# 0Setsuna0/SoftbodyUnity

Hardware: AMD Instinct MI355X
Metric: particle-substeps/sec (higher is better)
Workload: dtype f32

## Files before the change

include/softbody_debug.h:

```cpp
#ifndef SOFTBODY_MI355X_DEBUG_H
#define SOFTBODY_MI355X_DEBUG_H

#include "softbody.h"

#ifdef __cplusplus
extern "C" {
#endif

#define SB_DEBUG_NO_COMM  1u
#define SB_DEBUG_LOOPBACK 2u

#define SB_TUNE_NO_MASS_PALETTE   (1u << 0)
#define SB_TUNE_NO_UNIFORM_MASS   (1u << 1)
#define SB_TUNE_NO_PALETTE        (1u << 2)
#define SB_TUNE_NO_WAVE_ITEMS     (1u << 3)
#define SB_TUNE_NO_LANE_PACK      (1u << 4)
#define SB_TUNE_NO_COST_ORDER     (1u << 5)
#define SB_TUNE_NO_FUSED_UNPACK   (1u << 6)
#define SB_TUNE_PEER_COARSE       (1u << 7)
#define SB_TUNE_NO_LAZY_TICK      (1u << 8)
#define SB_TUNE_NO_PACK           (1u << 9)
#define SB_TUNE_NO_PEEK           (1u << 10)
#define SB_TUNE_NO_KIN_FUSE       (1u << 11)
#define SB_TUNE_NO_WIDE_SLOTS     (1u << 12)
#define SB_TUNE_AUTO_PREFER_OVERLAP (1u << 13)
#define SB_TUNE_NO_AUTO_CALIBRATION (1u << 14)
#define SB_TUNE_NO_SHARED_PROGRAMS (1u << 15)
typedef struct {
    uint32_t flags;
    int32_t tile_lanes;
    int32_t quad_lanes;
    int32_t narrow_min_tiles;
    int32_t store_through_max_tiles;
    int32_t store_through_large;
    int32_t peek_min_tiles;
    int32_t lds_pad_bytes;
    int32_t win_dwords;
    int32_t prev_offset_bytes;
    int32_t reserved[6];
} sb_tuning;
void sb_tuning_default(sb_tuning *t);
int sb_set_tuning(sb_solver *s, const sb_tuning *t);

int sb_profile_begin(sb_solver *s);
int sb_profile_end(sb_solver *s, float *elapsed_ms_out);
int sb_step_profiled(sb_solver *s, float dt, int32_t substeps, float *slot_ms_out, int32_t *slot_launches_out,
                     int32_t n_slots);
typedef struct {
    int64_t exchanges;
    double pack_ms, transport_ms, total_ms;
    double exposed_wait_ms;
} sb_exchange_timing;
int sb_debug_exchange_timing(sb_solver *s, int32_t enabled);
int sb_debug_exchange_timing_read(sb_solver *s, sb_exchange_timing *out);

int sb_debug_launch(sb_solver *s, float dt, int32_t substeps, int32_t it, int32_t gcolour);
int sb_debug_halo_pack(sb_solver *s, int32_t slot, float *host_out, int64_t capacity_floats, int64_t *count_floats_out);
int sb_debug_halo_unpack(sb_solver *s, int32_t slot, const float *host_in, int64_t count_floats);

typedef struct {
    int64_t tiles_checked, groups_checked, constraints_checked;
    int64_t errors[6];
    int32_t first_stage;
    int32_t first_tile, first_group, first_kind;
} sb_validate_report;
int sb_debug_validate(sb_solver *s, int32_t inject_fault, sb_validate_report *out);

int sb_debug_last_words(int32_t fd, const char *text, int64_t len, int32_t exit_code);

#ifdef __cplusplus
}
#endif
#endif
```

softbodyunity_amd/csrc/abi.hip:

```cpp
#include "solver_internal.hpp"

using namespace sbi;

extern "C" {

void sb_desc_default(sb_desc *d) {
    if (!d) return;
    std::memset(d, 0, sizeof(*d));
    d->world = 1;
    d->gravity[1] = -9.81f;
    d->tile_particles = 0;
    d->use_graph = 1;
}

int sb_create(const sb_desc *desc, sb_solver **out) {
    if (!desc || !out) return fail(SB_ERR_INVALID_ARG, "sb_create: null argument");
    *out = nullptr;
    return guarded([&]() -> int {
        sb_desc d = *desc;
        if (d.world <= 0) d.world = 1;
        if (d.rank < 0 || d.rank >= d.world) return fail(SB_ERR_INVALID_ARG, "sb_create: rank out of range");
        if (!(d.damping >= 0.0f)) return fail(SB_ERR_INVALID_ARG, "sb_create: damping must be >= 0");
        if (d.tile_particles > sbp::kMaxTileLocal) return fail(SB_ERR_INVALID_ARG, "sb_create: tile_particles too large");
        if (d.partition < SB_PARTITION_AUTO || d.partition > SB_PARTITION_RCB) return fail(SB_ERR_INVALID_ARG, "sb_create: partition must be SB_PARTITION_AUTO, _BLOCKS or _RCB");
        if (d.plan_flags & ~kPlanFlagsAll) return fail(SB_ERR_INVALID_ARG, "sb_create: unknown bit in plan_flags");
        if (d.halo_transport != SB_TRANSPORT_RCCL && d.halo_transport != SB_TRANSPORT_PEER) return fail(SB_ERR_INVALID_ARG, "sb_create: halo_transport must be SB_TRANSPORT_RCCL or _PEER");
        if (d.halo_schedule < SB_SCHEDULE_AUTO || d.halo_schedule > SB_SCHEDULE_OVERLAP_GRAPH) return fail(SB_ERR_INVALID_ARG, "sb_create: halo_schedule must be one of SB_SCHEDULE_*");
        if (d.debug_flags & ~(SB_DEBUG_NO_COMM | SB_DEBUG_LOOPBACK)) return fail(SB_ERR_INVALID_ARG, "sb_create: unknown bit in debug_flags");
        if (d.reserved[0] || d.reserved[1] || d.reserved[2]) return fail(SB_ERR_INVALID_ARG, "sb_create: reserved fields must be 0 (zero-initialise sb_desc or call sb_desc_default)");
        int ndev = 0;
        hipError_t e = hipGetDeviceCount(&ndev);
        if (e != hipSuccess || ndev <= 0)
            return fail(SB_ERR_NO_DEVICE, "sb_create: no HIP device (this plugin has no CPU path)");
        if (d.device < 0 || d.device >= ndev) return fail(SB_ERR_NO_DEVICE, "sb_create: device ordinal out of range");
        hipDeviceProp_t prop;
        HIP_CHECK(hipGetDeviceProperties(&prop, d.device));
        if (std::strncmp(prop.gcnArchName, "gfx950", 6) != 0)
            return fail(SB_ERR_NO_DEVICE, std::string("sb_create: device is ") + prop.gcnArchName + ", kernels are built for gfx950 only");
        HIP_CHECK(hipSetDevice(d.device));
        auto s = std::make_unique<sb_solver>();
        s->desc = d;
        s->peer.enabled = d.world > 1 && d.halo_transport == SB_TRANSPORT_PEER;
        s->loopback = d.world > 1 && (d.debug_flags & SB_DEBUG_LOOPBACK) != 0;
        HIP_CHECK(hipStreamCreateWithFlags(&s->stream, hipStreamNonBlocking));
        HIP_CHECK(hipEventCreate(&s->ev0));
        HIP_CHECK(hipEventCreate(&s->ev1));
        *out = s.release();
        return SB_OK;
    });
}

void sb_tuning_default(sb_tuning *t) {
    if (!t) return;
    std::memset(t, 0, sizeof(*t));
    t->store_through_max_tiles = -1;
    t->peek_min_tiles = -1;
}

int sb_set_tuning(sb_solver *s, const sb_tuning *t) {
    if (!s || !t) return fail(SB_ERR_INVALID_ARG, "sb_set_tuning: null argument");
    if (s->finalized) return fail(SB_ERR_STATE, "sb_set_tuning after sb_finalize");
    constexpr uint32_t kAll = (SB_TUNE_NO_SHARED_PROGRAMS << 1) - 1u;
    if (t->flags & ~kAll) return fail(SB_ERR_INVALID_ARG, "sb_set_tuning: unknown bit in flags");
    for (int32_t r : t->reserved) if (r) return fail(SB_ERR_INVALID_ARG, "sb_set_tuning: reserved fields must be 0 (sb_tuning_default)");
    if (t->tile_lanes != 0 && t->tile_lanes != 128 && t->tile_lanes != 256 && t->tile_lanes != 512) return fail(SB_ERR_INVALID_ARG, "sb_set_tuning: tile_lanes must be 0, 128, 256 or 512");
    if (t->quad_lanes != 0 && t->quad_lanes != 256 && t->quad_lanes != 512) return fail(SB_ERR_INVALID_ARG, "sb_set_tuning: quad_lanes must be 0, 256 or 512");
    if (t->prev_offset_bytes < 0 || (t->prev_offset_bytes & 15)) return fail(SB_ERR_INVALID_ARG, "sb_set_tuning: prev_offset_bytes must be a non-negative multiple of 16");
    if (t->narrow_min_tiles < 0 || t->store_through_max_tiles < -1 || t->peek_min_tiles < -1 || t->lds_pad_bytes < 0 || t->win_dwords < 0 || (t->store_through_large & ~3))
        return fail(SB_ERR_INVALID_ARG, "sb_set_tuning: value out of range");
    s->tune_flags = t->flags;
    s->lazy_tick = !(t->flags & SB_TUNE_NO_LAZY_TICK);
    s->pack_tiles = !(t->flags & SB_TUNE_NO_PACK);
    s->peek_enabled = !(t->flags & SB_TUNE_NO_PEEK);
    s->kin_fuse = !(t->flags & SB_TUNE_NO_KIN_FUSE);
    s->tile_lanes = t->tile_lanes;
    s->quad_lanes = t->quad_lanes ? t->quad_lanes : 512;
    if (t->narrow_min_tiles > 0) s->narrow_min_tiles = t->narrow_min_tiles;
    if (t->store_through_max_tiles >= 0) s->store_through_max_tiles = t->store_through_max_tiles;
    s->store_through_large = t->store_through_large;
    if (t->peek_min_tiles >= 0) s->peek_min_tiles = t->peek_min_tiles;
    s->lds_pad = (size_t)t->lds_pad_bytes;
    s->win_dwords_cap = t->win_dwords;
    s->prev_offset_bytes = t->prev_offset_bytes;
    return SB_OK;
}

int sb_destroy(sb_solver *s) {
    if (!s) return fail(SB_ERR_INVALID_ARG, "sb_destroy: null handle");
    (void)hipSetDevice(s->desc.device);
    delete s;
    return SB_OK;
}

int sb_set_particles(sb_solver *s, const float *pos, const float *vel, const float *inv_mass, int32_t n) {
    if (!s || !pos || !inv_mass || n <= 0) return fail(SB_ERR_INVALID_ARG, "sb_set_particles: bad argument");
    if (s->finalized) return fail(SB_ERR_STATE, "sb_set_particles after sb_finalize");
    return guarded([&]() -> int {
        for (int32_t p = 0; p < n; ++p) if (!(inv_mass[p] >= 0.0f)) return fail(SB_ERR_INVALID_ARG, "sb_set_particles: inverse mass must be >= 0");
        s->n = n;
        s->pos.assign(pos, pos + 3 * (size_t)n);
        if (vel) s->vel.assign(vel, vel + 3 * (size_t)n); else s->vel.assign(3 * (size_t)n, 0.0f);
        s->invm.assign(inv_mass, inv_mass + n);
        return SB_OK;
    });
}

int sb_set_rest_positions(sb_solver *s, const float *rest, int32_t n) {
    if (!s || !rest) return fail(SB_ERR_INVALID_ARG, "sb_set_rest_positions: bad argument");
    if (s->finalized) return fail(SB_ERR_STATE, "sb_set_rest_positions after sb_finalize");
    if (n != s->n) return fail(SB_ERR_INVALID_ARG, "sb_set_rest_positions: n differs from sb_set_particles");
    return guarded([&]() -> int { s->rest.assign(rest, rest + 3 * (size_t)n); return SB_OK; });
}

static int set_cons(sb_solver *s, const char *who, const int32_t *idx, const float *rest, int32_t m, float compliance,
                    int type, int nv, int nrest) {
    if (!s || m < 0 || (m > 0 && (!idx || !rest))) return fail(SB_ERR_INVALID_ARG, std::string(who) + ": bad argument");
    if (s->finalized) return fail(SB_ERR_STATE, std::string(who) + " after sb_finalize");
    if (s->n <= 0) return fail(SB_ERR_STATE, std::string(who) + " before sb_set_particles");
    if (!(compliance >= 0.0f)) return fail(SB_ERR_INVALID_ARG, std::string(who) + ": compliance must be >= 0");
    return guarded([&]() -> int {
        std::atomic<bool> bad{false};
        sbp::parallel_for_chunks((int64_t)m * nv, 1 << 22, [&](int64_t, int64_t kb, int64_t ke) {
            for (int64_t k = kb; k < ke; ++k) if (idx[k] < 0 || idx[k] >= s->n) { bad = true; return; }
        });
        if (bad) return fail(SB_ERR_INVALID_ARG, std::string(who) + ": particle index out of range");
        std::vector<int32_t> &I = type == 0 ? s->dist_ij : (type == 1 ? s->vol_ijkl : s->bend_ijkl);
        std::vector<float> &R = type == 0 ? s->dist_rest : (type == 1 ? s->vol_rest : s->bend_rest);
        I.assign(idx, idx + (size_t)m * nv);
        R.assign(rest, rest + (size_t)m * nrest);
        s->compliance[type] = compliance;
        return SB_OK;
    });
}

int sb_set_distance_constraints(sb_solver *s, const int32_t *ij, const float *rest_len, int32_t m, float compliance) {
    return set_cons(s, "sb_set_distance_constraints", ij, rest_len, m, compliance, 0, 2, 1);
}
int sb_set_volume_constraints(sb_solver *s, const int32_t *ijkl, const float *rest_vol, int32_t m, float compliance) {
    return set_cons(s, "sb_set_volume_constraints", ijkl, rest_vol, m, compliance, 1, 4, 1);
}
int sb_set_bending_constraints(sb_solver *s, const int32_t *ijkl, const float *rest_cs, int32_t m, float compliance) {
    return set_cons(s, "sb_set_bending_constraints", ijkl, rest_cs, m, compliance, 2, 4, 2);
}

int sb_set_ground_plane(sb_solver *s, float nx, float ny, float nz, float d, int32_t enabled) {
    if (!s) return fail(SB_ERR_INVALID_ARG, "sb_set_ground_plane: null handle");
    if (!(nx == nx) || !(ny == ny) || !(nz == nz) || !(d == d)) return fail(SB_ERR_INVALID_ARG, "sb_set_ground_plane: NaN");
    s->plane[0] = nx; s->plane[1] = ny; s->plane[2] = nz; s->plane[3] = d;
    s->plane_on = enabled ? 1 : 0;
    return SB_OK;
}

int sb_comm_unique_id(uint8_t out_id[SB_UNIQUE_ID_BYTES]) {
    if (!out_id) return fail(SB_ERR_INVALID_ARG, "sb_comm_unique_id: null");
    static_assert(sizeof(ncclUniqueId) <= SB_UNIQUE_ID_BYTES, "unique id size");
    return guarded([&]() -> int {
        ncclUniqueId id;
        NCCL_CHECK(rccl().GetUniqueId(&id));
        std::memset(out_id, 0, SB_UNIQUE_ID_BYTES);
        std::memcpy(out_id, &id, sizeof(id));
        return SB_OK;
    });
}

int sb_comm_init(sb_solver *s, const uint8_t id_bytes[SB_UNIQUE_ID_BYTES]) {
    if (!s || !id_bytes) return fail(SB_ERR_INVALID_ARG, "sb_comm_init: null");
    if (s->finalized) return fail(SB_ERR_STATE, "sb_comm_init after sb_finalize");
    if (s->comm) return fail(SB_ERR_STATE, "sb_comm_init called twice");
    return guarded([&]() -> int {
        int rc = set_device(s); if (rc) return rc;
        ncclUniqueId id;
        std::memcpy(&id, id_bytes, sizeof(id));
        if (s->loopback) {
            NCCL_CHECK(rccl().CommInitRank(&s->comm, 1, id, 0));
        } else {
            NCCL_CHECK(rccl().CommInitRank(&s->comm, s->desc.world, id, s->desc.rank));
        }
        return SB_OK;
    });
}

int sb_peer_mailbox_handle(sb_solver *s, uint8_t out_handle[SB_IPC_HANDLE_BYTES]) {
    if (!s || !out_handle) return fail(SB_ERR_INVALID_ARG, "sb_peer_mailbox_handle: null argument");
    if (!s->finalized || !s->peer.mailbox) return fail(SB_ERR_STATE, "sb_peer_mailbox_handle: needs a finalized world > 1 solver with SB_HALO_TRANSPORT=peer");
    static_assert(sizeof(hipIpcMemHandle_t) <= SB_IPC_HANDLE_BYTES, "ipc handle size");
    return guarded([&]() -> int {
        int rc = set_device(s); if (rc) return rc;
        hipIpcMemHandle_t h;
        HIP_CHECK(hipIpcGetMemHandle(&h, s->peer.mailbox));
        std::memset(out_handle, 0, SB_IPC_HANDLE_BYTES);
        std::memcpy(out_handle, &h, sizeof(h));
        return SB_OK;
    });
}

int sb_peer_connect(sb_solver *s, int32_t rank, const uint8_t handle[SB_IPC_HANDLE_BYTES], sb_solver *same_process_peer) {
    if (!s || (!handle && !same_process_peer)) return fail(SB_ERR_INVALID_ARG, "sb_peer_connect: null argument");
    if (!s->finalized || !s->peer.mailbox) return fail(SB_ERR_STATE, "sb_peer_connect: needs a finalized world > 1 solver with SB_HALO_TRANSPORT=peer");
    if (rank < 0 || rank >= s->desc.world || rank == s->desc.rank) return fail(SB_ERR_INVALID_ARG, "sb_peer_connect: bad rank");
    if (s->peer.remote[(size_t)rank]) return fail(SB_ERR_STATE, "sb_peer_connect: rank already connected");
    return guarded([&]() -> int {
        int rc = set_device(s); if (rc) return rc;
        if (same_process_peer) {
            if (!same_process_peer->peer.mailbox || same_process_peer->desc.rank != rank) return fail(SB_ERR_INVALID_ARG, "sb_peer_connect: the given solver is not that rank");
            s->peer.remote[(size_t)rank] = same_process_peer->peer.mailbox;
        } else {
            hipIpcMemHandle_t h;
            std::memcpy(&h, handle, sizeof(h));
            void *p = nullptr;
            HIP_CHECK(hipIpcOpenMemHandle(&p, h, hipIpcMemLazyEnablePeerAccess));
            s->peer.remote[(size_t)rank] = (uint32_t *)p; s->peer.opened[(size_t)rank] = 1;
        }
        s->peer.linked = false;
        return SB_OK;
    });
// ... 174 lines not shown
    return SB_OK;
}

int finalize_agree(sb_solver *s, int local_rc) {
    const int W = s->desc.world;
    const size_t rec = (size_t)W + 2;
    const std::string my_error = local_rc ? std::string(last_error_text()) : std::string();
    std::vector<uint64_t> mine = agreement_record(s, local_rc != SB_OK);
    std::vector<uint64_t> all((size_t)W * rec);
    const int rc = guarded([&]() -> int {
        int r0 = set_device(s); if (r0) return r0;
        DevBuf<uint64_t> d_all; int64_t acct = 0;
        d_all.alloc((size_t)W * rec, acct);
        HIP_CHECK(hipMemcpy(d_all.p + (size_t)s->desc.rank * rec, mine.data(), rec * sizeof(uint64_t), hipMemcpyHostToDevice));
        NCCL_CHECK(rccl().AllGather(d_all.p + (size_t)s->desc.rank * rec, d_all.p, rec * sizeof(uint64_t), ncclUint8, s->comm, s->stream));
        HIP_CHECK(hipStreamSynchronize(s->stream));
        HIP_CHECK(hipMemcpy(all.data(), d_all.p, all.size() * sizeof(uint64_t), hipMemcpyDeviceToHost));
        return SB_OK;
    });
    if (local_rc) return fail(local_rc, my_error);
    if (rc) return rc;
    return check_agreement(all, W, s->desc.rank);
}

int finalize_link(sb_solver *s) {
    return guarded([&]() -> int {
        int rc = set_device(s); if (rc) return rc;
        if (s->peer.enabled && s->desc.world > 1) {
            if (s->loopback) {
                peer_link(s);
            } else if (s->comm) {
                const int W = s->desc.world;
                hipIpcMemHandle_t mine;
                HIP_CHECK(hipIpcGetMemHandle(&mine, s->peer.mailbox));
                DevBuf<uint8_t> d_all; int64_t acct = 0;
                d_all.alloc((size_t)W * sizeof(mine), acct);
                HIP_CHECK(hipMemcpy(d_all.p + (size_t)s->desc.rank * sizeof(mine), &mine, sizeof(mine), hipMemcpyHostToDevice));
                NCCL_CHECK(rccl().AllGather(d_all.p + (size_t)s->desc.rank * sizeof(mine), d_all.p, sizeof(mine), ncclUint8, s->comm, s->stream));
                HIP_CHECK(hipStreamSynchronize(s->stream));
                std::vector<hipIpcMemHandle_t> all((size_t)W);
                HIP_CHECK(hipMemcpy(all.data(), d_all.p, (size_t)W * sizeof(mine), hipMemcpyDeviceToHost));
                for (int r = 0; r < W; ++r) {
                    if (r == s->desc.rank) continue;
                    bool needed = false;
                    for (const auto &H : s->halos) for (int pr : H->peers) needed |= pr == r;
                    if (!needed) continue;
                    void *p = nullptr;
                    HIP_CHECK(hipIpcOpenMemHandle(&p, all[(size_t)r], hipIpcMemLazyEnablePeerAccess));
                    s->peer.remote[(size_t)r] = (uint32_t *)p; s->peer.opened[(size_t)r] = 1;
                }
                peer_link(s);
            }
        }
        if (std::getenv("SB_PRINT_ALLOC")) {
            std::fprintf(stderr, "[alloc] pos3 %p prev %p vel %p wf %p w8 %p T0.stream %p T1.stream %p T0.tiles %p T1.tiles %p\n", (void *)s->d_pos3.p, (void *)s->d_prev.p,
                         (void *)s->d_vel.p, (void *)s->d_wf.p, (void *)s->d_w8.p, (void *)s->tiling[0].stream.p, (void *)s->tiling[1].stream.p,
                         (void *)s->tiling[0].tiles.p, (void *)s->tiling[1].tiles.p);
            for (int tl = 0; tl < 3; ++tl) {
                const DevTiling &D = s->tiling[tl];
                if (D.n_tiles)
                    std::fprintf(stderr, "[alloc] T%d: %d tiles, %lld distinct programs, stream %lld B read by the tiles, %lld B uploaded\n", tl, D.n_tiles,
                                 (long long)D.n_programs, (long long)D.stream_bytes, (long long)(D.stream.count * sizeof(uint32_t)));
            }
        }
        HIP_CHECK(hipDeviceSynchronize());
        std::vector<float>().swap(s->pos); std::vector<float>().swap(s->vel); std::vector<float>().swap(s->rest);
        std::vector<int32_t>().swap(s->dist_ij); std::vector<int32_t>().swap(s->vol_ijkl); std::vector<int32_t>().swap(s->bend_ijkl);
        std::vector<float>().swap(s->dist_rest); std::vector<float>().swap(s->vol_rest); std::vector<float>().swap(s->bend_rest);
        s->finalized = true;
        return SB_OK;
    });
}

}

extern "C" {

int sb_finalize(sb_solver *s) {
    if (!s) return fail(SB_ERR_INVALID_ARG, "sb_finalize: null handle");
    if (s->finalized) return fail(SB_ERR_STATE, "sb_finalize called twice");
    if (s->n <= 0) return fail(SB_ERR_STATE, "sb_finalize before sb_set_particles");
    const bool no_comm = (s->desc.debug_flags & SB_DEBUG_NO_COMM) != 0;
    if (s->desc.world > 1 && !s->comm && !s->peer.enabled && !no_comm)
        return fail(SB_ERR_STATE, "sb_finalize: world > 1 needs sb_comm_init first (or halo_transport = SB_TRANSPORT_PEER with sb_peer_connect)");
    int rc = guarded([&]() -> int { return finalize_local(s); });
    if (s->desc.world > 1 && s->comm && !s->loopback) rc = finalize_agree(s, rc);
    if (rc) return rc;
    return finalize_link(s);
}

int sb_synchronize(sb_solver *s) {
    if (!s) return fail(SB_ERR_INVALID_ARG, "sb_synchronize: null handle");
    return guarded([&]() -> int {
        int rc = set_device(s); if (rc) return rc;
        flush_deferred(s);
        HIP_CHECK(hipStreamSynchronize(s->stream));
        check_peer_error(s);
        return SB_OK;
    });
}

int sb_get_owner(sb_solver *s, int32_t *owner, int32_t n) {
    if (!s || !owner) return fail(SB_ERR_INVALID_ARG, "sb_get_owner: null argument");
    if (!s->finalized) return fail(SB_ERR_STATE, "sb_get_owner before sb_finalize");
    if (n != s->n) return fail(SB_ERR_INVALID_ARG, "sb_get_owner: n mismatch");
    std::memcpy(owner, s->plan->plan.owner_of_old.data(), (size_t)n * sizeof(int32_t));
    return SB_OK;
}

int sb_profile_begin(sb_solver *s) {
    if (!s) return fail(SB_ERR_INVALID_ARG, "sb_profile_begin: null handle");
    return guarded([&]() -> int {
        int rc = set_device(s); if (rc) return rc;
        HIP_CHECK(hipEventRecord(s->ev0, s->stream));
        return SB_OK;
    });
}
int sb_profile_end(sb_solver *s, float *ms) {
    if (!s || !ms) return fail(SB_ERR_INVALID_ARG, "sb_profile_end: null argument");
    return guarded([&]() -> int {
        int rc = set_device(s); if (rc) return rc;
        HIP_CHECK(hipEventRecord(s->ev1, s->stream));
        HIP_CHECK(hipEventSynchronize(s->ev1));
        HIP_CHECK(hipEventElapsedTime(ms, s->ev0, s->ev1));
        return SB_OK;
    });
}

int sb_get_stats(sb_solver *s, sb_stats *out) {
    if (!s || !out) return fail(SB_ERR_INVALID_ARG, "sb_get_stats: null argument");
    if (!s->finalized) return fail(SB_ERR_STATE, "sb_get_stats before sb_finalize");
    std::memset(out, 0, sizeof(*out));
    const sbp::Plan &P = s->plan->plan;
    const sbp::LocalPlan &L = s->plan->local;
    out->n_particles_owned = s->n_owned;
    out->n_particles_local = s->n_local;
    for (size_t k = 0; k < L.order_mask[0].size(); ++k) if (L.order_mask[0][k]) ++out->n_constraints_local[P.order_type[0][k]];
    out->n_tilings = P.tiling ? 2 : 1;
    out->n_global_colours = (int32_t)P.gcolours.size();
    for (int tl = 0; tl < 2; ++tl) { out->n_tiles[tl] = s->tiling[tl].n_tiles; out->tile_constraints[tl] = s->tiling[tl].n_slots; }
    out->n_t2_layers = (int64_t)s->t2_layer_range.size();
    out->n_t2_tiles = s->tiling[2].n_tiles;
    out->t2_constraints = s->tiling[2].n_slots;
    out->constraints_in_tiles = P.cons_in_tiles;
    out->constraints_in_global = P.cons_in_global;
    for (size_t slot = 0; slot < s->halos.size(); ++slot) {
        const int64_t cnt = s->halos[slot]->send_off.back();
        if (slot == 1) out->halo_particles_t1 = cnt; else out->halo_particles_global += cnt;
    }
    out->device_bytes = s->dev_bytes;
    {
        const int64_t mb = s->w_uniform ? 0 : (s->w_palette ? 1 : 4);
        auto tables = [&](const DevTiling &D) { return D.stream_bytes + (int64_t)D.n_tiles * (int64_t)sizeof(sbk::TileDesc) + (int64_t)D.runs_overflow.count * 8; };
        for (int tl = 0; tl < 2; ++tl) {
            const DevTiling &D = s->tiling[tl];
            if (!D.n_tiles) continue;
            out->launch_bytes[tl] = D.staged_particles * (12 + mb + 12 + 12 + 12) + tables(D);
        }
        const DevTiling &D0 = s->tiling[0];
        if (D0.n_tiles) {
            out->launch_bytes[2] = D0.staged_particles * (12 + mb + 12 + 12 + 12) + tables(D0);
            out->launch_bytes[3] = D0.staged_particles * (12 + mb + 12 + 12 + 12) + tables(D0);
        }
        const DevTiling &D2 = s->tiling[2];
        if (D2.n_tiles) out->launch_bytes[4] = D2.staged_particles * (4 + 12 + mb + 12) + tables(D2);
    }
    out->partition = P.partition;
    out->halo_schedule = s->schedule;
    out->halo_unpack_fused = s->fused_unpack ? 1 : 0;
    out->halo_auto_state = s->calib.state;
    out->halo_auto_ticks = s->calib.n[0] + s->calib.n[1];
    out->halo_auto_ms[0] = s->calib.decided_ms[0]; out->halo_auto_ms[1] = s->calib.decided_ms[1];
    out->readback_peeks = s->n_peeks;
    out->readback_peek_tiles = s->n_peek_tiles;
    out->ticks_fused = s->n_fused;
    out->ticks_fused_kinematic = s->n_kin_fused;
    for (int tl = 0; tl < 2; ++tl) out->lane_packed_tiles[tl] = s->tiling[tl].n_packed_tiles;
    out->plan_hash = s->plan_hash;
    if (!P.rank_cost.empty()) {
        out->partition_cost = P.rank_cost[(size_t)s->desc.rank];
        for (int64_t c : P.rank_cost) { out->partition_cost_total += c; out->partition_cost_max = std::max(out->partition_cost_max, c); }
    }
    {
        std::vector<uint8_t> is_peer((size_t)s->desc.world, 0);
        for (const auto &H : s->halos) {
            for (int pr : H->peers) is_peer[(size_t)pr] = 1;
            out->halo_particles_recv += H->recv_off.back();
        }
        for (uint8_t b : is_peer) out->halo_peers += b;
    }
    return SB_OK;
}

}
```

softbodyunity_amd/csrc/device_math.hip.hpp:

```cpp
#pragma once
#include "kernel_types.hpp"

namespace sbk {

__device__ __forceinline__ float4 pv_load(const PosView &P, int g) {
    const size_t o = 3 * (size_t)g;
    return make_float4(P.xyz[o], P.xyz[o + 1], P.xyz[o + 2], P.w[g]);
}
__device__ __forceinline__ void pv_store(const PosView &P, int g, const float4 &v) {
    const size_t o = 3 * (size_t)g;
    P.xyz[o] = v.x; P.xyz[o + 1] = v.y; P.xyz[o + 2] = v.z;
}

__device__ __forceinline__ void store3_through(float *p, float x, float y, float z) {
    f32x3_t v = {x, y, z};
    asm volatile("global_store_dwordx3 %0, %1, off sc0 sc1" ::"v"(p), "v"(v) : "memory");
}

struct V3 { float x, y, z; };
__device__ __forceinline__ V3 sub3(V3 a, V3 b) { return {a.x - b.x, a.y - b.y, a.z - b.z}; }
__device__ __forceinline__ V3 cross3(V3 a, V3 b) {
    float t0 = a.y * b.z, t1 = a.z * b.y, t2 = a.z * b.x, t3 = a.x * b.z, t4 = a.x * b.y, t5 = a.y * b.x;
    return {t0 - t1, t2 - t3, t4 - t5};
}
__device__ __forceinline__ float dot3(V3 a, V3 b) {
    float xx = a.x * b.x, yy = a.y * b.y, zz = a.z * b.z;
    return (xx + yy) + zz;
}
__device__ __forceinline__ V3 addscaled3(V3 x, float s, V3 g) {
    float a = s * g.x, b = s * g.y, c = s * g.z;
    return {x.x + a, x.y + b, x.z + c};
}
__device__ __forceinline__ V3 xyz(float4 p) { return {p.x, p.y, p.z}; }

__device__ __forceinline__ float sqrt_rn_normal(float x) {
#ifdef SB_LIBM_SQRT
    return sqrtf(x);
#endif
    float s = __builtin_amdgcn_sqrtf(x);
    float sd = __int_as_float(__float_as_int(s) - 1), su = __int_as_float(__float_as_int(s) + 1);
    float rd = __builtin_fmaf(-sd, s, x), ru = __builtin_fmaf(-su, s, x);
    s = rd <= 0.0f ? sd : s;
    return ru > 0.0f ? su : s;
}

__device__ __forceinline__ bool project_distance(float4 &a, float4 &b, float L0, float at) {
    float dx = a.x - b.x, dy = a.y - b.y, dz = a.z - b.z;
    float xx = dx * dx, yy = dy * dy, zz = dz * dz;
    float L2 = (xx + yy) + zz;
    float ws = (a.w + b.w) + at;
    if (!(L2 >= 0x1p-96f) || !(ws > 0.0f)) return false;
    float L = sqrt_rn_normal(L2);
    float C = L - L0;
    float wl = ws * L;
    float s = (-C) / wl;
    float si = a.w * s, sj = b.w * s;
    float ax = si * dx, ay = si * dy, az = si * dz;
    float bx = sj * dx, by = sj * dy, bz = sj * dz;
    a.x = a.x + ax; a.y = a.y + ay; a.z = a.z + az;
    b.x = b.x - bx; b.y = b.y - by; b.z = b.z - bz;
    return true;
}

__device__ __forceinline__ bool project_distance_nobranch(float4 &a, float4 &b, float L0, float at) {
    float dx = a.x - b.x, dy = a.y - b.y, dz = a.z - b.z;
    float xx = dx * dx, yy = dy * dy, zz = dz * dz;
    float L2 = (xx + yy) + zz;
    float ws = (a.w + b.w) + at;
    const bool ok = (L2 >= 0x1p-96f) && (ws > 0.0f);
    float L = sqrt_rn_normal(L2);
    float C = L - L0;
    float wl = ws * L;
    float s = (-C) / wl;
    float si = a.w * s, sj = b.w * s;
    float ax = si * dx, ay = si * dy, az = si * dz;
    float bx = sj * dx, by = sj * dy, bz = sj * dz;
    a.x = a.x + ax; a.y = a.y + ay; a.z = a.z + az;
    b.x = b.x - bx; b.y = b.y - by; b.z = b.z - bz;
    return ok;
}

__device__ __forceinline__ bool project_volume(float4 &p0, float4 &p1, float4 &p2, float4 &p3, float R6, float at_v) {
    V3 x0 = xyz(p0), x1 = xyz(p1), x2 = xyz(p2), x3 = xyz(p3);
    V3 e1 = sub3(x1, x0), e2 = sub3(x2, x0), e3 = sub3(x3, x0);
    V3 g1 = cross3(e2, e3), g2 = cross3(e3, e1), g3 = cross3(e1, e2);
    V3 g0;
    { float t = g1.x + g2.x; t = t + g3.x; g0.x = -t; }
    { float t = g1.y + g2.y; t = t + g3.y; g0.y = -t; }
    { float t = g1.z + g2.z; t = t + g3.z; g0.z = -t; }
    float C6 = dot3(e1, g1) - R6;
    float a0 = p0.w * dot3(g0, g0), a1 = p1.w * dot3(g1, g1), a2 = p2.w * dot3(g2, g2), a3 = p3.w * dot3(g3, g3);
    float den = (((a0 + a1) + a2) + a3) + at_v;
    if (!(den > 0.0f)) return false;
    float s = (-C6) / den;
    x0 = addscaled3(x0, p0.w * s, g0); x1 = addscaled3(x1, p1.w * s, g1);
    x2 = addscaled3(x2, p2.w * s, g2); x3 = addscaled3(x3, p3.w * s, g3);
    p0.x = x0.x; p0.y = x0.y; p0.z = x0.z; p1.x = x1.x; p1.y = x1.y; p1.z = x1.z;
    p2.x = x2.x; p2.y = x2.y; p2.z = x2.z; p3.x = x3.x; p3.y = x3.y; p3.z = x3.z;
    return true;
}

__device__ __forceinline__ bool project_bending(float4 &pa, float4 &pb, float4 &pc, float4 &pd, float2 rest, float at_b) {
    V3 xa = xyz(pa), xb = xyz(pb), xc = xyz(pc), xd = xyz(pd);
    V3 e = sub3(xb, xa);
    float el2 = dot3(e, e);
    float el = sqrtf(el2);
    V3 ac = sub3(xa, xc), bc = sub3(xb, xc), bd = sub3(xb, xd), ad = sub3(xa, xd);
    V3 n1 = cross3(ac, bc), n2 = cross3(bd, ad);
    float q1 = dot3(n1, n1), q2 = dot3(n2, n2);
    if (!(el > 0.0f) || !(q1 > 0.0f) || !(q2 > 0.0f)) return false;
    V3 m1 = {n1.x / q1, n1.y / q1, n1.z / q1}, m2 = {n2.x / q2, n2.y / q2, n2.z / q2};
    V3 gc = {el * m1.x, el * m1.y, el * m1.z}, gd = {el * m2.x, el * m2.y, el * m2.z};
    V3 cb = sub3(xc, xb), db = sub3(xd, xb);
    float ta1 = dot3(cb, e) / el, ta2 = dot3(db, e) / el;
    float tb1 = dot3(ac, e) / el, tb2 = dot3(ad, e) / el;
    V3 ga, gb;
    { float p = ta1 * m1.x, q = ta2 * m2.x; ga.x = p + q; float r = tb1 * m1.x, t = tb2 * m2.x; gb.x = r + t; }
    { float p = ta1 * m1.y, q = ta2 * m2.y; ga.y = p + q; float r = tb1 * m1.y, t = tb2 * m2.y; gb.y = r + t; }
    { float p = ta1 * m1.z, q = ta2 * m2.z; ga.z = p + q; float r = tb1 * m1.z, t = tb2 * m2.z; gb.z = r + t; }
    float s1 = sqrtf(q1), s2 = sqrtf(q2);
    V3 u1 = {n1.x / s1, n1.y / s1, n1.z / s1}, u2 = {n2.x / s2, n2.y / s2, n2.z / s2};
    float cs = dot3(u1, u2);
    V3 cr = cross3(u1, u2);
    float sn = -(dot3(cr, e) / el);
    float t0 = sn * rest.x, t1 = cs * rest.y;
    float C = t0 - t1;
    float a0 = pa.w * dot3(ga, ga), a1 = pb.w * dot3(gb, gb), a2 = pc.w * dot3(gc, gc), a3 = pd.w * dot3(gd, gd);
    float den = (((a0 + a1) + a2) + a3) + at_b;
    if (!(den > 0.0f)) return false;
    float s = (-C) / den;
    xa = addscaled3(xa, pa.w * s, ga); xb = addscaled3(xb, pb.w * s, gb);
    xc = addscaled3(xc, pc.w * s, gc); xd = addscaled3(xd, pd.w * s, gd);
    pa.x = xa.x; pa.y = xa.y; pa.z = xa.z; pb.x = xb.x; pb.y = xb.y; pb.z = xb.z;
    pc.x = xc.x; pc.y = xc.y; pc.z = xc.z; pd.x = xd.x; pd.y = xd.y; pd.z = xd.z;
    return true;
}

constexpr int qp_ctrl(int a, int b, int c, int d) { return a | (b << 2) | (c << 4) | (d << 6); }
template <int CTRL>
__device__ __forceinline__ float qperm(float v) {
    return __int_as_float(__builtin_amdgcn_mov_dpp(__float_as_int(v), CTRL, 0xf, 0xf, true));
}
__device__ __forceinline__ float qb0(float v) { return qperm<qp_ctrl(0, 0, 0, 0)>(v); }
__device__ __forceinline__ float qb1(float v) { return qperm<qp_ctrl(1, 1, 1, 1)>(v); }
__device__ __forceinline__ float qb2(float v) { return qperm<qp_ctrl(2, 2, 2, 2)>(v); }
__device__ __forceinline__ float qb3(float v) { return qperm<qp_ctrl(3, 3, 3, 3)>(v); }
__device__ __forceinline__ float qrot1(float v) { return qperm<qp_ctrl(1, 2, 0, 3)>(v); }
__device__ __forceinline__ float qrot2(float v) { return qperm<qp_ctrl(2, 0, 1, 3)>(v); }
__device__ __forceinline__ float qdot(float a, float b) {
    const float t = a * b;
    const float xx = qb0(t), yy = qb1(t), zz = qb2(t);
    return (xx + yy) + zz;
}
__device__ __forceinline__ float qcross(float a, float b) {
    const float t0 = qrot1(a) * qrot2(b), t1 = qrot2(a) * qrot1(b);
    return t0 - t1;
}

__device__ __forceinline__ bool project_volume_quad(float (&P)[4], float R6, float at_v) {
    const float W0 = qb3(P[0]), W1 = qb3(P[1]), W2 = qb3(P[2]), W3 = qb3(P[3]);
    const float e1 = P[1] - P[0], e2 = P[2] - P[0], e3 = P[3] - P[0];
    const float g1 = qcross(e2, e3), g2 = qcross(e3, e1), g3 = qcross(e1, e2);
    float t = g1 + g2; t = t + g3;
    const float g0 = -t;
    const float C6 = qdot(e1, g1) - R6;
    const float a0 = W0 * qdot(g0, g0), a1 = W1 * qdot(g1, g1), a2 = W2 * qdot(g2, g2), a3 = W3 * qdot(g3, g3);
    const float den = (((a0 + a1) + a2) + a3) + at_v;
    if (!(den > 0.0f)) return false;
    const float s = (-C6) / den;
// ... 100 lines not shown
```

softbodyunity_amd/csrc/kernel_types.hpp:

```cpp
#pragma once
#include <hip/hip_runtime.h>
#include <stdint.h>

namespace sbk {

struct TickParams {
    float h, inv_h, hgx, hgy, hgz, kd, at_d, at_v, at_b;
    float pnx, pny, pnz, pd;
    int32_t plane_on;
    float pad[2];
};

struct TileDesc {
    int32_t n_local, run_count, n_rounds;
    int32_t gather_begin;
    uint32_t s_begin;
    uint32_t s_hdr;
    uint32_t s_len;
    uint32_t packed_lanes;
    int32_t run_overflow;
    int32_t n_pal;
    int32_t n_steps;
    uint32_t s_items;
    int2 runs[10];
};
constexpr int kInlineRuns = 10;
constexpr int kLanePackLanes = 128, kLanePackRounds = 3, kLanePackFieldBits = 21, kLanePackMaxPalette = 8;
constexpr uint32_t kLanePackDwordsCompact = 4 * kLanePackLanes, kLanePackDwordsFull = 10 * kLanePackLanes;
constexpr int kWidePackLanes = 256;
constexpr uint32_t kWidePackDwords = 2 * kWidePackLanes;
constexpr int kWide8MaxTiles = 768;
#ifndef SB_REG_ROUNDS
#define SB_REG_ROUNDS 4
#endif
#ifndef SB_REG_ROUNDS_NARROW
#define SB_REG_ROUNDS_NARROW 3
#endif
constexpr int kRegRoundsWide = SB_REG_ROUNDS, kRegRoundsNarrow = SB_REG_ROUNDS_NARROW;
#ifdef SB_REG_COMPACT_ONLY
constexpr bool kRegFullSlots = false;
#else
constexpr bool kRegFullSlots = true;
#endif
constexpr bool kLanePackDecodable = kRegRoundsNarrow >= kLanePackRounds;
constexpr int kItemWaves = 4;
constexpr uint32_t kItemIdle = 0, kItemDistCompact = 1, kItemDistFull = 2, kItemVolume = 3, kItemBending = 4;
constexpr int kItemCountShift = 3, kItemBarrierBit = 10, kItemOffsetShift = 11;
constexpr int kMaxRoundsLds = 128;
constexpr int kMaxPalette = 256;

typedef float f32x3_t __attribute__((ext_vector_type(3)));
struct PosView {
    float *xyz;
    const float *w;
};

constexpr int kMaxMassPalette = 64;

struct TileArgs {
    PosView pos;
    const uint8_t *w8;
    const float *wpal;
    float *prev;
    float *vel;
    const TileDesc *tiles;
    const int2 *runs_overflow;
    const uint32_t *stream;
    const TickParams *tp;
    const int32_t *gather;
    int32_t max_local;
    int32_t rounds_dwords;
    int32_t pal_dwords;
    int32_t win_dwords;
    int32_t tile_base;
    int32_t w_uniform;
    int32_t item_waves;
    int32_t store_through;
    const float *ghost_src;
    int32_t n_owned;
    float *peek_out;
    const int32_t *kin_map;
    float *kin_target;
};
constexpr int kHaloNone = 0, kHaloGhosts = 1;

constexpr int kNarrowTileThreads = 128;
constexpr int kQuadTileThreads = 512;
constexpr int kWideTileThreads = 256;
constexpr int kRoundSlots = 256;
constexpr int kSmallTile = 512, kLargeTile = 1024;
typedef float f32x3 __attribute__((ext_vector_type(3)));

typedef float f32x4 __attribute__((ext_vector_type(4)));
typedef uint32_t u32x4 __attribute__((ext_vector_type(4)));

constexpr int kMaxPeers = 8;
struct PeerSlot {
    int32_t n_send, n_recv;
    int32_t send_off[kMaxPeers + 1];
    int32_t send_cap[kMaxPeers];
    float *remote_data[kMaxPeers];
    int32_t remote_stride[kMaxPeers];
    int32_t my_stride[kMaxPeers];
    int32_t recv_off[kMaxPeers + 1];
    int32_t recv_cnt[kMaxPeers];
    const float *my_data[kMaxPeers];
    uint32_t *remote_data_flag[kMaxPeers];
    uint32_t *my_ack_flag[kMaxPeers];
    uint32_t *my_data_flag[kMaxPeers];
    uint32_t *remote_ack_flag[kMaxPeers];
    uint32_t *local;
    uint32_t *error;
};
constexpr int kPeerSpinLimit = 1 << 24;

struct ValidateCounters {
    unsigned long long tiles, groups, constraints;
    unsigned int errors[6];
    int first[4];
};
constexpr int kValidateThreads = 256;

}
```

softbodyunity_amd/csrc/schedule.hip:

```cpp
#include "solver_internal.hpp"
#include "tile_kernel.hip.hpp"
#include "aux_kernels.hip.hpp"

namespace sbi {

sbk::TickParams tick_params(const sb_solver *s, float dt, int substeps) {
    sbk::TickParams t{};
    volatile float S = (float)substeps;
    volatile float h = dt / S;
    t.h = h;
    volatile float inv_h = 1.0f / h;
    t.inv_h = inv_h;
    volatile float hx = h * s->desc.gravity[0], hy = h * s->desc.gravity[1], hz = h * s->desc.gravity[2];
    t.hgx = hx; t.hgy = hy; t.hgz = hz;
    volatile float td = s->desc.damping * h;
    volatile float kd = 1.0f - td;
    t.kd = kd < 0.0f ? 0.0f : (float)kd;
    volatile float h2 = h * h;
    volatile float ad = s->compliance[0] / h2;
    volatile float av = s->compliance[1] / h2;
    volatile float av36 = 36.0f * av;
    volatile float ab = s->compliance[2] / h2;
    t.at_d = ad; t.at_v = av36; t.at_b = ab;
    t.pnx = s->plane[0]; t.pny = s->plane[1]; t.pnz = s->plane[2]; t.pd = s->plane[3]; t.plane_on = s->plane_on;
// ... 23 lines not shown
                const uint64_t their_plan = (uint64_t)hw[0] | ((uint64_t)hw[1] << 32);
                const uint64_t their_pair = (uint64_t)hw[4 + 2 * (size_t)me] | ((uint64_t)hw[5 + 2 * (size_t)me] << 32);
                const uint64_t my_pair = s->plan->local.pair_hash[(size_t)r];
                char msg[320];
                if (hw[3] != plan_shape(s)) {
                    std::snprintf(msg, sizeof msg, "peer transport: ranks %d and %d planned tick programs of different shape (leftover layers / global colours: %x vs %x): "
                                  "a window that does not reproduce the whole-mesh plan, or different meshes on the ranks", me, r, plan_shape(s), hw[3]);
                    throw HipError(SB_ERR_STATE, msg);
                }
                if (!s->sharded && !hw[2] && their_plan != s->plan_hash) {
                    std::snprintf(msg, sizeof msg, "peer transport: rank %d planned a different schedule than rank %d (plan hash %016llx vs %016llx): every rank "
                                  "must pass the same mesh, tile_particles, partition and plan_flags", r, me, (unsigned long long)their_plan, (unsigned long long)s->plan_hash);
                    throw HipError(SB_ERR_STATE, msg);
                }
                if (their_pair != my_pair) {
                    std::snprintf(msg, sizeof msg, "peer transport: ranks %d and %d disagree on what they share (ghost lists / programs of the tiles both run: pair hash "
                                  "%016llx vs %016llx)", me, r, (unsigned long long)my_pair, (unsigned long long)their_pair);
                    throw HipError(SB_ERR_STATE, msg);
                }
            }
            if (cs) {
                if (P.n_send >= sbk::kMaxPeers) throw std::runtime_error("peer transport: too many neighbours");
                uint32_t off = 0;
                if (s->loopback) off = PS.my_off[(size_t)slot][(size_t)D.peers[k]];
                else HIP_CHECK(hipMemcpy(&off, rm + PS.off_table + (size_t)slot * W + (size_t)me, 4, hipMemcpyDeviceToHost));
                if (off == 0) throw std::runtime_error("peer transport: a neighbour's mailbox has no segment for this rank");
                P.send_off[P.n_send] = D.send_off[k];
                P.send_cap[P.n_send] = s->loopback ? std::min(cs, cr) : cs;
                P.remote_data[P.n_send] = reinterpret_cast<float *>(rm + off);
                P.remote_stride[P.n_send] = (int32_t)((fl * (size_t)(s->loopback ? cr : cs) + 3) & ~(size_t)3);
                P.remote_data_flag[P.n_send] = rm + base + (size_t)(s->loopback ? D.peers[k] : me);
                P.my_ack_flag[P.n_send] = PS.mailbox + base + (size_t)W + (size_t)D.peers[k];
                ++P.n_send;
                P.send_off[P.n_send] = D.send_off[k + 1];
            }
            if (cr) {
                P.recv_off[P.n_recv] = D.recv_off[k];
                P.recv_off[P.n_recv + 1] = D.recv_off[k + 1];
                P.recv_cnt[P.n_recv] = cr;
                P.my_data[P.n_recv] = reinterpret_cast<const float *>(PS.mailbox + PS.my_off[(size_t)slot][(size_t)D.peers[k]]);
                P.my_stride[P.n_recv] = (int32_t)((fl * (size_t)cr + 3) & ~(size_t)3);
                P.my_data_flag[P.n_recv] = PS.mailbox + base + (size_t)D.peers[k];
                P.remote_ack_flag[P.n_recv] = rm + base + (size_t)W + (size_t)(s->loopback ? D.peers[k] : me);
                ++P.n_recv;
            }
        }
        for (int q = P.n_send + 1; q <= sbk::kMaxPeers; ++q) P.send_off[q] = INT32_MAX;
        for (int q = P.n_recv + 1; q <= sbk::kMaxPeers; ++q) P.recv_off[q] = INT32_MAX;
    }
    PS.linked = true;
}

bool halo_slot_active(const sb_solver *s, int slot) { return slot >= 0 && slot < (int)s->halos.size() && s->halos[(size_t)slot]->active(); }

void halo_exchange_pre(sb_solver *s, int slot, hipStream_t st) {
    if (!halo_slot_active(s, slot)) return;
    DevHalo &D = *s->halos[slot];
    const bool with_prev = slot == 1;
    const int ns = D.send_off.back(), nr = D.recv_off.back();
    if (s->peer.enabled) {
        if (!s->peer.linked) peer_link(s);
        const sbk::PeerSlot &P = s->peer.slots[(size_t)slot];
        const int push_chunks = ns, unpack_chunks = nr;
        constexpr int kPeerGrid = 128;
        if (with_prev) {
            hipLaunchKernelGGL(sbk::peer_push_kernel<true>, dim3(std::min(kPeerGrid, std::max(1, (push_chunks + 255) / 256))), dim3(256), 0, st, s->pos_view(), s->d_prev.p, D.send_idx.p, push_chunks, P);
            hipLaunchKernelGGL(sbk::peer_unpack_kernel<true>, dim3(std::min(kPeerGrid, std::max(1, (unpack_chunks + 255) / 256))), dim3(256), 0, st, s->pos_view(), s->d_prev.p, D.recv_idx.p, unpack_chunks, P);
        } else {
            hipLaunchKernelGGL(sbk::peer_push_kernel<false>, dim3(std::min(kPeerGrid, std::max(1, (push_chunks + 255) / 256))), dim3(256), 0, st, s->pos_view(), s->d_prev.p, D.send_idx.p, push_chunks, P);
            hipLaunchKernelGGL(sbk::peer_unpack_kernel<false>, dim3(std::min(kPeerGrid, std::max(1, (unpack_chunks + 255) / 256))), dim3(256), 0, st, s->pos_view(), s->d_prev.p, D.recv_idx.p, unpack_chunks, P);
        }
        return;
    }
    if (!s->comm) throw HipError(SB_ERR_STATE, "world > 1 needs sb_comm_init before sb_finalize");
    if (ns) {
        if (with_prev)
            hipLaunchKernelGGL(sbk::halo_pack_kernel<true>, dim3((ns + 255) / 256), dim3(256), 0, st, s->pos_view(),
                               s->d_prev.p, D.send_idx.p, s->d_sendbuf.p, ns);
        else
            hipLaunchKernelGGL(sbk::halo_pack_kernel<false>, dim3((ns + 255) / 256), dim3(256), 0, st, s->pos_view(),
                               s->d_prev.p, D.send_idx.p, s->d_sendbuf.p, ns);
    }
}

void halo_exchange_calls(sb_solver *s, int slot, hipStream_t st) {
    if (!halo_slot_active(s, slot) || s->peer.enabled) return;
    DevHalo &D = *s->halos[slot];
    const bool with_prev = slot == 1;
    for (size_t k = 0; k < D.peers.size(); ++k) {
        int cs = D.send_off[k + 1] - D.send_off[k], cr = D.recv_off[k + 1] - D.recv_off[k];
        if (s->loopback) cs = cr = std::min(cs, cr);
        const size_t fl = with_prev ? 6 : 3;
        if (cs) NCCL_CHECK(rccl().Send(s->d_sendbuf.p + fl * D.send_off[k], fl * (size_t)cs, ncclFloat, s->loopback ? 0 : D.peers[k], s->comm, st));
        if (cr) NCCL_CHECK(rccl().Recv(s->d_recvbuf.p + fl * D.recv_off[k], fl * (size_t)cr, ncclFloat, s->loopback ? 0 : D.peers[k], s->comm, st));
    }
}

void halo_exchange_post(sb_solver *s, int slot, hipStream_t st) {
    if (!halo_slot_active(s, slot) || s->peer.enabled) return;
    DevHalo &D = *s->halos[slot];
    const bool with_prev = slot == 1;
    const int nr = D.recv_off.back();
    if (nr && !(with_prev && s->fused_unpack)) {
        if (with_prev)
            hipLaunchKernelGGL(sbk::halo_unpack_kernel<true>, dim3((nr + 255) / 256), dim3(256), 0, st, s->pos_view(),
                               s->d_prev.p, D.recv_idx.p, s->d_recvbuf.p, nr);
        else
            hipLaunchKernelGGL(sbk::halo_unpack_kernel<false>, dim3((nr + 255) / 256), dim3(256), 0, st, s->pos_view(),
                               s->d_prev.p, D.recv_idx.p, s->d_recvbuf.p, nr);
    }
}

void ExchangeTimer::mark(hipStream_t st, bool join) {
    hipEvent_t e;
    if (free_list.empty()) HIP_CHECK(hipEventCreate(&e)); else { e = free_list.back(); free_list.pop_back(); }
    HIP_CHECK(hipEventRecord(e, st));
    (join ? join_pending : pending).push_back(e);
}
ExchangeTimer::~ExchangeTimer() {
    for (auto e : pending) (void)hipEventDestroy(e);
    for (auto e : join_pending) (void)hipEventDestroy(e);
    for (auto e : free_list) (void)hipEventDestroy(e);
}

void halo_exchange(sb_solver *s, int slot, hipStream_t st) {
    if (!st) st = s->stream;
    if (!halo_slot_active(s, slot)) return;
    const bool timed = s->xtimer.enabled && !s->capturing;
    if (timed) s->xtimer.mark(st);
    if (!s->peer.enabled) halo_exchange_pre(s, slot, st);
    if (timed) s->xtimer.mark(st);
    if (s->peer.enabled) halo_exchange_pre(s, slot, st);
    if (!s->peer.enabled) {
        NCCL_CHECK(rccl().GroupStart());
        try {
            halo_exchange_calls(s, slot, st);
        } catch (...) {
            (void)rccl().GroupEnd();
            throw;
        }
        NCCL_CHECK(rccl().GroupEnd());
    }
    halo_exchange_post(s, slot, st);
    if (timed) s->xtimer.mark(st);
}

template <int KIND>
void launch_tile(sb_solver *s, DevTiling &D, int tile_begin = 0, int tile_end = -1, int halo = sbk::kHaloNone, const sbk::TileDesc *table = nullptr) {
    const bool ghosts = halo == sbk::kHaloGhosts;
    if (tile_end < 0) tile_end = D.n_tiles;
    if (tile_end <= tile_begin) return;
    sbk::TileArgs A{};
    A.pos = s->pos_view(); A.w8 = s->d_w8.p; A.wpal = s->d_wpal.p; A.prev = s->d_prev.p; A.vel = s->d_vel.p;
    A.tiles = D.tiles.p; A.runs_overflow = D.runs_overflow.p; A.stream = D.stream.p;
    A.tp = s->d_tp.p;
    A.gather = D.gather.p;
    A.w_uniform = s->w_uniform ? 1 : 0;
    A.item_waves = D.item_waves;
    A.store_through = tile_end - tile_begin <= s->store_through_max_tiles ? 3 : s->store_through_large;
    A.ghost_src = ghosts ? s->d_recvbuf.p : nullptr; A.n_owned = (int32_t)s->n_owned;
    A.peek_out = KIND == 4 ? s->d_peek.p : nullptr;
    A.kin_map = KIND == 5 ? s->d_kin_map.p : nullptr; A.kin_target = KIND == 5 ? s->d_kin_target.p : nullptr;
    A.max_local = D.max_local; A.win_dwords = D.win_dwords; A.tile_base = tile_begin; A.pal_dwords = D.pal_dwords; A.rounds_dwords = D.rounds_dwords;
    const sbk::TileDesc *tiles_at_base = table ? table : D.tiles.p + tile_begin;
    const int n_wg = tile_end - tile_begin;
    const bool small = D.max_local <= sbk::kSmallTile;
    const bool narrow = small && (D.packed_lanes ? D.packed_lanes == sbk::kLanePackLanes : (s->tile_lanes ? s->tile_lanes == sbk::kNarrowTileThreads : tile_end - tile_begin >= s->narrow_min_tiles));
    const bool quad8 = D.has_quads && s->quad_lanes == sbk::kQuadTileThreads;
    constexpr int kWide8MaxTiles = sbk::kWide8MaxTiles;
    const bool wide8 = small && !D.has_quads && !D.packed_lanes && (s->tile_lanes ? s->tile_lanes == 512 : tile_end - tile_begin <= kWide8MaxTiles);
    const dim3 grid(tile_end - tile_begin), block(quad8 || wide8 ? sbk::kQuadTileThreads : (narrow ? sbk::kNarrowTileThreads : sbk::kWideTileThreads));
#define SB_LAUNCH_TILE(Q, W, G)                                                                                               \
    do {                                                                                                                      \
        if (Q && quad8) {                                                                                                     \
            if (small) hipLaunchKernelGGL((sbk::tile_kernel<KIND, true, sbk::kQuadTileThreads, sbk::kSmallTile / sbk::kQuadTileThreads, W, sbk::kHaloNone>), \
                                          grid, block, D.lds_bytes + s->lds_pad, s->stream, tiles_at_base, n_wg, A);                                           \
            else hipLaunchKernelGGL((sbk::tile_kernel<KIND, true, sbk::kQuadTileThreads, sbk::kLargeTile / sbk::kQuadTileThreads, W, sbk::kHaloNone>), \
                                    grid, block, D.lds_bytes + s->lds_pad, s->stream, tiles_at_base, n_wg, A);                                                 \
        } else if (wide8) hipLaunchKernelGGL((sbk::tile_kernel<KIND, false, sbk::kQuadTileThreads, sbk::kSmallTile / sbk::kQuadTileThreads, W, G>), \
                                       grid, block, D.lds_bytes + s->lds_pad, s->stream, tiles_at_base, n_wg, A);                                              \
        else if (narrow) hipLaunchKernelGGL((sbk::tile_kernel<KIND, Q, sbk::kNarrowTileThreads, sbk::kSmallTile / sbk::kNarrowTileThreads, W, G>), \
                                       grid, block, D.lds_bytes + s->lds_pad, s->stream, tiles_at_base, n_wg, A);                                              \
        else if (small) hipLaunchKernelGGL((sbk::tile_kernel<KIND, Q, sbk::kWideTileThreads, sbk::kSmallTile / sbk::kWideTileThreads, W, G>), \
                                           grid, block, D.lds_bytes + s->lds_pad, s->stream, tiles_at_base, n_wg, A);                                          \
        else hipLaunchKernelGGL((sbk::tile_kernel<KIND, Q, sbk::kWideTileThreads, sbk::kLargeTile / sbk::kWideTileThreads, W, G>), \
                                grid, block, D.lds_bytes + s->lds_pad, s->stream, tiles_at_base, n_wg, A);                                                     \
    } while (0)
    constexpr bool kCanGhost = KIND == 1 || KIND == 2;
    if (ghosts && !(kCanGhost && !D.has_quads)) throw std::runtime_error("internal: ghost-reading tile kernel requested for a launch that has none");
    if (kCanGhost && ghosts) {
        if (s->w_palette) SB_LAUNCH_TILE(false, true, (kCanGhost ? sbk::kHaloGhosts : sbk::kHaloNone)); else SB_LAUNCH_TILE(false, false, (kCanGhost ? sbk::kHaloGhosts : sbk::kHaloNone));
    } else
    if (s->w_palette) { if (D.has_quads) SB_LAUNCH_TILE(true, true, sbk::kHaloNone); else SB_LAUNCH_TILE(false, true, sbk::kHaloNone); }
    else { if (D.has_quads) SB_LAUNCH_TILE(true, false, sbk::kHaloNone); else SB_LAUNCH_TILE(false, false, sbk::kHaloNone); }
#undef SB_LAUNCH_TILE
}

struct LaunchTimer {
    std::vector<hipEvent_t> ev;
    std::vector<int> slot;
    hipStream_t stream;
    void begin(int which) {
        hipEvent_t a, b;
        HIP_CHECK(hipEventCreate(&a)); HIP_CHECK(hipEventCreate(&b));
        ev.push_back(a); ev.push_back(b); slot.push_back(which);
        HIP_CHECK(hipEventRecord(a, stream));
    }
    void end() { HIP_CHECK(hipEventRecord(ev.back(), stream)); }
    ~LaunchTimer() { for (auto e : ev) (void)hipEventDestroy(e); }
};

void launch_tick_kernel(sb_solver *s, int it, int substeps, LaunchTimer *lt, int tile_begin = 0, int tile_end = -1, bool kin = false) {
    const int tl = s->plan->plan.tiling ? (it & 1) : 0;
    DevTiling &D = s->tiling[tl];
    if (lt && D.n_tiles) lt->begin(it == 0 ? 2 + (int)s->gcolours.size() : (it == substeps ? 3 + (int)s->gcolours.size() : tl));
    const int halo_in = s->fused_unpack && tl == 1 ? sbk::kHaloGhosts : sbk::kHaloNone;
    if (it == 0) launch_tile<0>(s, D, tile_begin, tile_end);
    else if (it < substeps && kin) launch_tile<5>(s, D, tile_begin, tile_end);
    else if (it < substeps) launch_tile<1>(s, D, tile_begin, tile_end, halo_in);
    else launch_tile<2>(s, D, tile_begin, tile_end, halo_in);
    if (lt && D.n_tiles) lt->end();
}

void launch_t2_layer(sb_solver *s, int layer, LaunchTimer *lt, bool with_halo = true) {
    const auto rg = s->t2_layer_range[layer];
    if (with_halo) halo_exchange(s, 2 + (int)s->gcolours.size() + layer);
    if (rg.second <= rg.first) return;
    if (lt) lt->begin(4 + (int)s->gcolours.size());
    launch_tile<3>(s, s->tiling[2], rg.first, rg.second);
    if (lt) lt->end();
}

void launch_gcolour(sb_solver *s, int gc, LaunchTimer *lt) {
    DevGColour &G = *s->gcolours[gc];
    if (G.count == 0) return;
    if (lt) lt->begin(2 + gc);
    dim3 grid((G.count + 255) / 256);
    if (G.type == 0)
        hipLaunchKernelGGL(sbk::global_distance_kernel, grid, dim3(256), 0, s->stream, s->pos_view(), G.ij.p, G.rest.p, G.count,
                           s->d_tp.p);
    else
        hipLaunchKernelGGL(sbk::global_quad_kernel, grid, dim3(256), 0, s->stream, s->pos_view(), G.quad.p, G.rest2.p, G.count,
                           G.type, s->d_tp.p);
    if (lt) lt->end();
}

std::vector<TickStep> tick_program(const sb_solver *s, int substeps, bool fused_first, bool defer_last, bool kin) {
    std::vector<TickStep> P;
    const bool two = s->plan->plan.tiling;
    auto tile = [&](int it, TileRange rg, bool k = false) {
        const bool ff = it == 0 && fused_first;
        P.push_back(TickStep{StepKind::Tile, rg, k && ff, ff ? 2 : it, ff ? 4 : substeps, 0});
    };
    if (s->overlap_halo) {
        for (int it = 0; it <= substeps; ++it) {
            if (it == substeps && defer_last) break;
            if (it & 1) {
                tile(it, TileRange::T1Interior);
                P.push_back(TickStep{StepKind::JoinExchange, TileRange::All, false, it, substeps, 1});
                tile(it, TileRange::T1Boundary);
            } else {
                tile(it, TileRange::T0Boundary);
                if (it < substeps) P.push_back(TickStep{StepKind::ForkExchange, TileRange::All, false, it, substeps, 1});
                tile(it, TileRange::T0Interior);
            }
        }
        return P;
    }
    for (int it = 0; it <= substeps; ++it) {
        if (it == substeps && defer_last) break;
        if (two && (it & 1)) P.push_back(TickStep{StepKind::Exchange, TileRange::All, false, it, substeps, 1});
        tile(it, TileRange::All, kin);
        if (it == substeps) break;
        for (size_t ly = 0; ly < s->t2_layer_range.size(); ++ly) {
            P.push_back(TickStep{StepKind::Exchange, TileRange::All, false, it, substeps, 2 + (int)s->gcolours.size() + (int)ly});
            P.push_back(TickStep{StepKind::T2Layer, TileRange::All, false, it, substeps, (int)ly});
        }
        for (size_t gc = 0; gc < s->gcolours.size(); ++gc) {
            P.push_back(TickStep{StepKind::Exchange, TileRange::All, false, it, substeps, 2 + (int)gc});
            P.push_back(TickStep{StepKind::GColour, TileRange::All, false, it, substeps, (int)gc});
        }
    }
    return P;
}

void run_step(sb_solver *s, const TickStep &st, LaunchTimer *lt) {
    switch (st.kind) {
    case StepKind::Tile: {
        DevTiling &T0 = s->tiling[0], &T1 = s->tiling[1];
        int b = 0, e = -1;
        if (st.range == TileRange::T0Boundary) { b = 0; e = T0.n_boundary; }
        else if (st.range == TileRange::T0Interior) { b = T0.n_boundary; e = T0.n_tiles; }
        else if (st.range == TileRange::T1Interior) { b = 0; e = T1.n_tiles - T1.n_boundary; }
        else if (st.range == TileRange::T1Boundary) { b = T1.n_tiles - T1.n_boundary; e = T1.n_tiles; }
        launch_tick_kernel(s, st.it, st.substeps, lt, b, e, st.kin);
        break;
    }
    case StepKind::T2Layer: launch_t2_layer(s, st.index, lt, false); break;
    case StepKind::GColour: launch_gcolour(s, st.index, lt); break;
    case StepKind::Exchange: halo_exchange(s, st.index); break;
    case StepKind::ForkExchange:
        HIP_CHECK(hipEventRecord(s->ev_boundary, s->stream));
        HIP_CHECK(hipStreamWaitEvent(s->comm_stream, s->ev_boundary, 0));
        halo_exchange(s, st.index, s->comm_stream);
        HIP_CHECK(hipEventRecord(s->ev_halo, s->comm_stream));
        break;
    case StepKind::JoinExchange: {
        const bool timed = s->xtimer.enabled && !s->capturing;
        if (timed) s->xtimer.mark(s->stream, true);
        HIP_CHECK(hipStreamWaitEvent(s->stream, s->ev_halo, 0));
        if (timed) s->xtimer.mark(s->stream, true);
        break;
    }
    }
}

void enqueue_substeps(sb_solver *s, int substeps, LaunchTimer *lt = nullptr, bool fused_first = false, bool defer_last = false, bool kin = false) {
    for (const TickStep &st : tick_program(s, substeps, fused_first, defer_last, kin)) run_step(s, st, lt);
    HIP_CHECK(hipGetLastError());
}

void scatter_kinematic(sb_solver *s, float *dst) {
    const int q = s->kin_pending, count = s->kin_pending_count;
    hipLaunchKernelGGL(sbk::kinematic_scatter_kernel, dim3((unsigned)((count + 255) / 256)), dim3(256), 0, s->stream, dst, s->d_kin_idx[q], s->d_kin_pos[q], count);
    HIP_CHECK(hipGetLastError());
}
void retire_kinematic(sb_solver *s) {
    HIP_CHECK(hipEventRecord(s->ev_kin[s->kin_pending], s->stream));
    s->kin_pending = -1; s->kin_pending_count = 0;
}

void flush_deferred(sb_solver *s) {
    if (s->deferred) {
        const int S = s->deferred_substeps;
        s->deferred = false;
        if (s->plan->plan.tiling && (S & 1)) halo_exchange(s, 1);
        launch_tick_kernel(s, S, S, nullptr);
        HIP_CHECK(hipGetLastError());
    }
    if (s->kin_pending >= 0) {
        scatter_kinematic(s, s->d_pos3.p);
        retire_kinematic(s);
    }
}

void stage_kinematic_for_fusion(sb_solver *s) {
    if (!s->d_kin_map.p) {
// ... 341 lines not shown
```

softbodyunity_amd/csrc/solver_internal.hpp:

```cpp
#pragma once
#include <hip/hip_runtime.h>
#include <rccl/rccl.h>
#include <dlfcn.h>

#include <algorithm>
#include <array>
#include <atomic>
#include <chrono>
#include <climits>
#include <cmath>
#include <cstdio>
#include <cstdlib>
#include <cstring>
#include <limits>
#include <map>
#include <memory>
#include <mutex>
#include <type_traits>
#include <stdexcept>
#include <string>
#include <utility>
#include <vector>

#include "../../include/softbody.h"
// ... 8 lines not shown

int fail(int code, const std::string &msg);
const char *last_error_text();

struct HipError : std::runtime_error {
    int code;
    HipError(int c, const std::string &m) : std::runtime_error(m), code(c) {}
};
#define HIP_CHECK(expr)                                                                                   \
    do {                                                                                                  \
        hipError_t e_ = (expr);                                                                           \
        if (e_ != hipSuccess)                                                                             \
            throw HipError(SB_ERR_HIP, std::string(#expr) + ": " + hipGetErrorString(e_));                \
    } while (0)
struct RcclApi {
    void *handle = nullptr;
    bool was_resident = false;
    int version = 0;
    std::string path, error;
    decltype(&ncclGetVersion) GetVersion = nullptr;
    decltype(&ncclGetUniqueId) GetUniqueId = nullptr;
    decltype(&ncclCommInitRank) CommInitRank = nullptr;
    decltype(&ncclCommDestroy) CommDestroy = nullptr;
    decltype(&ncclGetErrorString) GetErrorString = nullptr;
    decltype(&ncclGroupStart) GroupStart = nullptr;
    decltype(&ncclGroupEnd) GroupEnd = nullptr;
    decltype(&ncclSend) Send = nullptr;
    decltype(&ncclRecv) Recv = nullptr;
    decltype(&ncclAllGather) AllGather = nullptr;
    bool ok() const { return handle != nullptr; }
};
RcclApi &rccl(bool required = true);
#define NCCL_CHECK(expr)                                                                                  \
    do {                                                                                                  \
        ncclResult_t r_ = (expr);                                                                         \
        if (r_ != ncclSuccess)                                                                            \
            throw HipError(SB_ERR_RCCL, std::string(#expr) + ": " + rccl().GetErrorString(r_));          \
    } while (0)

int hip_runtime_version();
bool capture_overlap_ok();

template <class T>
struct DevBuf {
    T *p = nullptr;
    T *base = nullptr;
    size_t count = 0;
    DevBuf() = default;
    DevBuf(const DevBuf &) = delete;
    DevBuf &operator=(const DevBuf &) = delete;
    DevBuf(DevBuf &&o) noexcept : p(o.p), base(o.base), count(o.count) { o.p = o.base = nullptr; o.count = 0; }
    DevBuf &operator=(DevBuf &&o) noexcept { if (this != &o) { free(); p = o.p; base = o.base; count = o.count; o.p = o.base = nullptr; o.count = 0; } return *this; }
    void alloc(size_t n, int64_t &acct, size_t lead_elems = 0) {
        free();
        count = n;
        if (n) { HIP_CHECK(hipMalloc((void **)&base, (n + lead_elems) * sizeof(T))); p = base + lead_elems; acct += (int64_t)((n + lead_elems) * sizeof(T)); }
    }
    void upload(const std::vector<T> &h, int64_t &acct) {
        alloc(h.size(), acct);
        if (!h.empty()) HIP_CHECK(hipMemcpy(p, h.data(), h.size() * sizeof(T), hipMemcpyHostToDevice));
    }
    void free() { if (base) { (void)hipFree(base); } base = nullptr; p = nullptr; count = 0; }
    ~DevBuf() { free(); }
};

struct DevHalo {
    std::vector<int> peers;
    std::vector<int32_t> send_off, recv_off;
    DevBuf<int32_t> send_idx, recv_idx;
    bool active() const { return !peers.empty(); }
};

struct DevTiling : sbt::TilingScalars {
    DevBuf<sbk::TileDesc> tiles;
    DevBuf<int2> runs_overflow;
    DevBuf<uint32_t> stream;
    DevBuf<int32_t> gather;
};

struct DevGColour {
    int type = 0;
    int32_t count = 0;
    DevBuf<int2> ij;
    DevBuf<int4> quad;
    DevBuf<float> rest;
    DevBuf<float2> rest2;
};

}

namespace sbi {

enum class StepKind : uint8_t { Tile, T2Layer, GColour, Exchange, ForkExchange, JoinExchange };
enum class TileRange : uint8_t { All, T0Boundary, T0Interior, T1Interior, T1Boundary };
struct TickStep {
    StepKind kind;
    TileRange range;
    bool kin;
    int it, substeps;
    int index;
};
struct TickShape { int substeps; bool fuse, defer_last, kin; };

struct ExchangeTimer {
    bool enabled = false;
    std::vector<hipEvent_t> pending, join_pending, free_list;
    void mark(hipStream_t st, bool join = false);
    ~ExchangeTimer();
};

}

using sbi::DevBuf; using sbi::DevGColour; using sbi::DevHalo; using sbi::DevTiling;

struct sb_plan {
    sbp::Plan plan;
    sbp::LocalPlan local;
    bool owns_local = true;
};

struct sb_solver {
    sb_desc desc;
    bool finalized = false;
    hipStream_t stream = nullptr;
    hipEvent_t ev0 = nullptr, ev1 = nullptr;
    ncclComm_t comm = nullptr;
    bool loopback = false;
    int schedule = SB_SCHEDULE_SERIAL_EAGER;
    uint64_t plan_hash = 0;
    hipStream_t comm_stream = nullptr;
    hipEvent_t ev_boundary = nullptr, ev_halo = nullptr;
    bool overlap_halo = false;
    int32_t n = 0;
    std::vector<float> pos, vel, invm, rest;
    bool sharded = false;
    sb_domain domain{};
    std::vector<int32_t> global_id;
    std::vector<int32_t> dist_ij, vol_ijkl, bend_ijkl;
    std::vector<float> dist_rest, vol_rest, bend_rest;
    float compliance[3] = {0, 0, 0};
    float plane[4] = {0, 1, 0, 0};
    int32_t plane_on = 0;
    std::unique_ptr<sb_plan> plan;
    int64_t dev_bytes = 0;
    int64_t n_owned = 0, n_local = 0;
    DevBuf<float> d_pos3;
    DevBuf<float> d_wf;
    DevBuf<uint8_t> d_w8;
    DevBuf<float> d_wpal;
    bool w_palette = false;
    bool w_uniform = false;
    sbk::PosView pos_view() const { return sbk::PosView{d_pos3.p, d_wf.p}; }
    DevBuf<float> d_prev, d_vel;
    DevBuf<sbk::TickParams> d_tp;
    DevBuf<float> d_sendbuf, d_recvbuf;
    DevTiling tiling[3];
    std::vector<std::pair<int32_t, int32_t>> t2_layer_range;
    std::vector<std::unique_ptr<DevGColour>> gcolours;
    std::vector<std::unique_ptr<DevHalo>> halos;
    sbk::TickParams tp_host{};
    bool tp_valid = false;
    struct CachedGraph { hipGraphExec_t exec; uint64_t last_use; };
    std::map<int, CachedGraph> graphs;
    uint64_t graph_clock = 0;
    static constexpr size_t kMaxGraphs = 8;
    bool deferred = false;
    int deferred_substeps = 0;
    uint32_t tune_flags = 0;
    int win_dwords_cap = 0;
    int prev_offset_bytes = 0;
    bool lazy_tick = true;
    int tile_lanes = 0;
    int quad_lanes = 512;
    int store_through_max_tiles = 6144;
    int store_through_large = 0;
    int narrow_min_tiles = 10240;
    size_t lds_pad = 0;
    bool pack_tiles = true;
    bool fused_unpack = false;
    bool graph_rccl = false;
    std::vector<float> h_stage;
    struct AutoSchedule {
        int state = 0;
        int tick = 0;
        hipEvent_t ev[8] = {nullptr, nullptr, nullptr, nullptr, nullptr, nullptr, nullptr, nullptr};
        int n[2] = {0, 0};
        double decided_ms[2] = {0, 0};
    } calib;
    bool group_walk = false;
    bool capturing = false;
    sbi::ExchangeTimer xtimer;
    struct PeerState {
        bool enabled = false, linked = false, fine_grained = false;
        uint32_t *mailbox = nullptr;
        size_t bytes = 0, data_off_words = 0, off_table = 0;
        int n_slots = 0;
        std::vector<uint32_t *> remote;
        std::vector<uint8_t> opened;
        std::vector<std::vector<uint32_t>> my_off;
        std::vector<sbk::PeerSlot> slots;
        uint32_t *local = nullptr;
        uint32_t *h_error = nullptr;
        size_t slot_base(int slot, int world) const { return sbt::mailbox_slot_base(slot, world); }
    } peer;
    hipStream_t copy_stream = nullptr;
    DevBuf<int32_t> d_local_to_old;
    DevBuf<float> d_get_scratch;
    static constexpr int kSnapSlots = 3;
    DevBuf<float> d_snap[kSnapSlots];
    float *h_snap[kSnapSlots] = {nullptr, nullptr, nullptr};
    hipEvent_t ev_snap[kSnapSlots] = {nullptr, nullptr, nullptr}, ev_copied[kSnapSlots] = {nullptr, nullptr, nullptr};
    int snap_head = 0, snap_pending = 0;
    std::vector<int32_t> render_tri;
    bool render_dirty = false;
    DevBuf<int32_t> d_tri, d_adj_off, d_adj_tri, d_render_set, d_render_local;
    std::vector<int32_t> render_set;
    bool render_set_only = false;
    DevBuf<float> d_cpos[kSnapSlots];
    float *h_cpos[kSnapSlots] = {nullptr, nullptr, nullptr};
    bool snap_compact[kSnapSlots] = {false, false, false};
    DevBuf<float> d_nrm[kSnapSlots];
    float *h_nrm[kSnapSlots] = {nullptr, nullptr, nullptr};
    bool snap_has_normals[kSnapSlots] = {false, false, false};
    bool snap_has_render_set[kSnapSlots] = {false, false, false};
    std::vector<int32_t> render_local;
    int snap_last_ended = -1;
    struct Embedding {
        int32_t m = 0;
        std::vector<int32_t> cage, tri;
        std::vector<float> w;
        bool dirty = false;
        std::vector<int32_t> wanted_local;
        DevBuf<int4> d_cage;
        DevBuf<float4> d_w;
        DevBuf<int32_t> d_tri, d_adj_off, d_adj_tri;
        DevBuf<float> d_pos[kSnapSlots], d_nrm[kSnapSlots];
        float *h_pos[kSnapSlots] = {nullptr, nullptr, nullptr}, *h_nrm[kSnapSlots] = {nullptr, nullptr, nullptr};
        void release() {
            d_cage.free(); d_w.free(); d_tri.free(); d_adj_off.free(); d_adj_tri.free();
            for (int k = 0; k < kSnapSlots; ++k) {
                d_pos[k].free(); d_nrm[k].free();
                if (h_pos[k]) (void)hipHostFree(h_pos[k]);
                if (h_nrm[k]) (void)hipHostFree(h_nrm[k]);
                h_pos[k] = h_nrm[k] = nullptr;
            }
        }
    } emb;
    bool snap_embedded[kSnapSlots] = {false, false, false};
    static constexpr int kKinSlots = 4;
    int32_t *h_kin_idx[kKinSlots] = {nullptr, nullptr, nullptr, nullptr};
    float *h_kin_pos[kKinSlots] = {nullptr, nullptr, nullptr, nullptr};
    int32_t *d_kin_idx[kKinSlots] = {nullptr, nullptr, nullptr, nullptr};
    float *d_kin_pos[kKinSlots] = {nullptr, nullptr, nullptr, nullptr};
    std::vector<uint32_t> kin_seen; uint32_t kin_stamp = 0;
    std::vector<int32_t> local_of_old;
    size_t kin_cap[kKinSlots] = {0, 0, 0, 0};
    hipEvent_t ev_kin[kKinSlots] = {nullptr, nullptr, nullptr, nullptr};
    int kin_next = 0;
    int kin_pending = -1, kin_pending_count = 0;
    DevBuf<int32_t> d_kin_map;
    DevBuf<float> d_kin_target;
    int64_t n_kin_fused = 0;
    bool kin_fuse = true;
    DevBuf<float> d_peek;
    DevBuf<sbk::TileDesc> peek_tiles;
    int32_t n_peek_tiles = -1;
    bool peek_enabled = true;
    int peek_min_tiles = 2048;
    int64_t n_peeks = 0;
    int64_t n_fused = 0;

    ~sb_solver() {
        if (stream) (void)hipStreamSynchronize(stream);
        if (comm_stream) (void)hipStreamSynchronize(comm_stream);
        if (copy_stream) (void)hipStreamSynchronize(copy_stream);
        for (auto &g : graphs) (void)hipGraphExecDestroy(g.second.exec);
        graphs.clear();
        if (comm) (void)sbi::rccl(false).CommDestroy(comm);
        for (size_t r = 0; r < peer.remote.size(); ++r) if (peer.opened[r] && peer.remote[r]) (void)hipIpcCloseMemHandle(peer.remote[r]);
        if (peer.mailbox) (void)hipFree(peer.mailbox);
        if (peer.local) (void)hipFree(peer.local);
        if (peer.h_error) (void)hipHostFree(peer.h_error);
        for (hipEvent_t e : calib.ev) if (e) (void)hipEventDestroy(e);
        if (ev_boundary) (void)hipEventDestroy(ev_boundary);
        if (ev_halo) (void)hipEventDestroy(ev_halo);
        if (comm_stream) (void)hipStreamDestroy(comm_stream);
        gcolours.clear(); halos.clear();
        for (int k = 0; k < kSnapSlots; ++k) {
            if (h_snap[k]) (void)hipHostFree(h_snap[k]);
            if (h_nrm[k]) (void)hipHostFree(h_nrm[k]);
            if (h_cpos[k]) (void)hipHostFree(h_cpos[k]);
            if (ev_snap[k]) (void)hipEventDestroy(ev_snap[k]);
            if (ev_copied[k]) (void)hipEventDestroy(ev_copied[k]);
        }
        emb.release();
        if (copy_stream) (void)hipStreamDestroy(copy_stream);
        for (int k = 0; k < kKinSlots; ++k) {
            if (h_kin_idx[k]) (void)hipHostFree(h_kin_idx[k]);
            if (h_kin_pos[k]) (void)hipHostFree(h_kin_pos[k]);
            if (ev_kin[k]) (void)hipEventDestroy(ev_kin[k]);
        }
        if (ev0) (void)hipEventDestroy(ev0);
        if (ev1) (void)hipEventDestroy(ev1);
        if (stream) (void)hipStreamDestroy(stream);
    }
};
// ... 70 lines not shown
```

softbodyunity_amd/csrc/tables.hip:

```cpp
#include "solver_internal.hpp"

namespace sbi {

sbp::Input make_input(const float *rest, int32_t n, const int32_t *d, int64_t md, const int32_t *v, int64_t mv,
                      const int32_t *b, int64_t mb) {
    sbp::Input in;
    in.rest = rest; in.n = n; in.dist_ij = d; in.m_d = md; in.vol = v; in.m_v = mv; in.bend = b; in.m_b = mb;
    return in;
}

sbp::Domain to_domain(const sb_domain &d) {
    sbp::Domain D;
    D.set = true; D.n_global = d.n_global; D.ell = d.spacing; D.fill = d.fill > 0 && d.fill <= 1 ? d.fill : 1.0;
    for (int a = 0; a < 3; ++a) { D.lo[a] = d.lo[a]; D.hi[a] = d.hi[a]; }
    return D;
}
sbp::Opts plan_opts(int rank, int world, const int32_t dims[3], int32_t tile_particles, int32_t partition, uint32_t plan_flags,
                    int64_t m_v, int64_t m_b, const sb_domain *domain) {
    sbp::Opts o;
    if (domain) {
        o.domain = to_domain(*domain);
        if (domain->four_vertex_constraints) m_v += 1;
    }
    o.rank = rank; o.world = world <= 0 ? 1 : world;
    for (int a = 0; a < 3; ++a) o.dims[a] = dims ? dims[a] : 0;
    o.tile_particles = tile_particles != 0 ? tile_particles : (m_v + m_b > 0 ? 256 : 512);
    o.partition = partition;
    o.third_tiling = !(plan_flags & SB_PLAN_NO_T2);
    o.third_list = !(plan_flags & SB_PLAN_NO_THIRD_LIST);
    o.cluster_layers = !(plan_flags & SB_PLAN_NO_CLUSTER_LAYERS);
    o.mixed_groups = !(plan_flags & SB_PLAN_NO_MIXED_GROUPS);
    o.bank_aware_lanes = !(plan_flags & SB_PLAN_NO_BANK_ORDER);
    o.merge_tiles = !(plan_flags & SB_PLAN_NO_TILE_MERGE);
    if ((plan_flags >> 8) & 3u) o.balanced_lists = (int)((plan_flags >> 8) & 3u);
    return o;
}

uint64_t hash_plan(const sbp::Plan &P) {
    uint64_t h = sbt::kFnvBasis;
    auto mix = [&](const void *p, size_t bytes) {
        const uint8_t *b = static_cast<const uint8_t *>(p);
        size_t k = 0;
        for (; k + 8 <= bytes; k += 8) { uint64_t w; std::memcpy(&w, b + k, 8); h = sbt::fnv1a(h, w); }
        for (; k < bytes; ++k) h = sbt::fnv1a(h, b[k]);
    };
    const int32_t head[8] = {P.n, P.opts.world, P.opts.tile_particles, P.partition,
                             (int32_t)((P.opts.third_tiling ? 0 : 1) | (P.opts.third_list ? 0 : 2) | (P.opts.cluster_layers ? 0 : 4) |
                                       (P.opts.mixed_groups ? 0 : 8) | (P.opts.bank_aware_lanes ? 0 : 16) | (P.opts.merge_tiles ? 0 : 32) | (P.opts.balanced_lists << 8)),
                             P.dims[0], P.dims[1], P.dims[2]};
    mix(head, sizeof(head));
    mix(P.m, sizeof(P.m));
    for (int p = 0; p < 2; ++p) {
        mix(P.order_type[p].data(), P.order_type[p].size());
        mix(P.order_id[p].data(), P.order_id[p].size() * sizeof(int32_t));
        for (const sbp::Phase &ph : P.phases[p]) {
            const int64_t rec[6] = {ph.kind, ph.tiling, ph.halo_slot, ph.layer, ph.order_begin, ph.order_end};
            mix(rec, sizeof(rec));
        }
    }
    mix(P.owner_of_old.data(), P.owner_of_old.size() * sizeof(int32_t));
    return h;
}

static void alloc_mailbox(sb_solver *s, sbt::HostMailbox &M) {
    auto &PS = s->peer;
    const int W = s->plan->local.world;
    PS.n_slots = M.n_slots; PS.off_table = M.off_table; PS.data_off_words = M.data_off_words; PS.bytes = M.bytes;
    PS.my_off = std::move(M.my_off);
    void *mb = nullptr;
    if (!(s->tune_flags & SB_TUNE_PEER_COARSE) && hipExtMallocWithFlags(&mb, PS.bytes, hipDeviceMallocFinegrained) == hipSuccess) PS.fine_grained = true;
    else { (void)hipGetLastError(); HIP_CHECK(hipMalloc(&mb, PS.bytes)); }
    PS.mailbox = (uint32_t *)mb;
    s->dev_bytes += (int64_t)PS.bytes;
    HIP_CHECK(hipMemset(PS.mailbox, 0, PS.bytes));
    HIP_CHECK(hipMemcpy(PS.mailbox, M.header.data(), M.header.size() * 4, hipMemcpyHostToDevice));
    HIP_CHECK(hipMalloc((void **)&PS.local, (size_t)PS.n_slots * 8 * sizeof(uint32_t)));
    HIP_CHECK(hipMemset(PS.local, 0, (size_t)PS.n_slots * 8 * sizeof(uint32_t)));
    HIP_CHECK(hipHostMalloc((void **)&PS.h_error, sizeof(uint32_t), hipHostMallocMapped));
    *PS.h_error = 0;
    PS.remote.assign((size_t)W, nullptr);
    PS.opened.assign((size_t)W, 0);
    PS.remote[(size_t)s->plan->local.rank] = PS.mailbox;
}

void build_device(sb_solver *s) {
    const sbp::LocalPlan &L = s->plan->local;
    const sbt::TableInput in{&s->plan->plan, &L, s->pos.data(), s->vel.data(), s->invm.data(), s->dist_rest.data(), s->vol_rest.data(),
                             s->bend_rest.data(), (int64_t)s->vol_rest.size(), (int64_t)s->bend_rest.size()};
    sbt::TableOptions opt;
    opt.tune_flags = s->tune_flags; opt.tile_lanes = s->tile_lanes; opt.quad_lanes = s->quad_lanes; opt.narrow_min_tiles = s->narrow_min_tiles;
    opt.pack_tiles = s->pack_tiles; opt.win_dwords_cap = s->win_dwords_cap;
    opt.split_launches = s->overlap_halo || s->calib.state == 1;
    opt.peer_enabled = s->peer.enabled; opt.sharded = s->sharded; opt.plan_hash = s->plan_hash;
    opt.plan_shape = opt.peer_enabled && L.world > 1 ? plan_shape(s) : 0u;
    sbt::HostTables H;
    sbt::build_state(in, opt, H);
    s->n_owned = H.n_owned; s->n_local = H.n_local;
    s->w_palette = H.w_palette; s->w_uniform = H.w_uniform;
    s->d_pos3.upload(H.pos3, s->dev_bytes);
    s->d_wf.upload(H.wf, s->dev_bytes);
    if (H.w_palette) s->d_w8.upload(H.w8, s->dev_bytes);
    s->d_wpal.upload(H.wpal, s->dev_bytes);
    s->d_vel.upload(H.vel, s->dev_bytes);
    for (std::vector<float> *v : {&H.pos3, &H.wf, &H.vel}) std::vector<float>().swap(*v);
    std::vector<uint8_t>().swap(H.w8);
    s->d_prev.alloc((size_t)s->n_local * 3, s->dev_bytes, (size_t)s->prev_offset_bytes / sizeof(float));
    HIP_CHECK(hipMemset(s->d_prev.p, 0, (size_t)s->n_local * 3 * sizeof(float)));
    s->d_tp.alloc(1, s->dev_bytes);
    for (int tl = 0; tl < 3; ++tl) {
        sbt::build_tiling(in, opt, tl, H);
        sbt::HostTiling &T = H.T[tl];
        DevTiling &D = s->tiling[tl];
        static_cast<sbt::TilingScalars &>(D) = T;
        D.tiles.upload(T.tiles, s->dev_bytes); D.runs_overflow.upload(T.runs_overflow, s->dev_bytes);
        D.stream.upload(T.stream, s->dev_bytes);
        D.gather.upload(T.gather, s->dev_bytes);
        T.release_arrays();
    }
    s->t2_layer_range = H.t2_layer_range;
    sbt::build_gcolours(in, H);
    for (const sbt::HostGColour &G : H.gcolours) {
        auto D = std::make_unique<DevGColour>();
        D->type = G.type; D->count = G.count;
        if (G.type == 0) { D->ij.upload(G.ij, s->dev_bytes); D->rest.upload(G.rest, s->dev_bytes); }
        else { D->quad.upload(G.quad, s->dev_bytes); D->rest2.upload(G.rest2, s->dev_bytes); }
        s->gcolours.push_back(std::move(D));
    }
    sbt::build_halos(in, opt, H);
    for (sbt::HostHalo &G : H.halos) {
        auto D = std::make_unique<DevHalo>();
        D->send_idx.upload(G.send_idx, s->dev_bytes); D->recv_idx.upload(G.recv_idx, s->dev_bytes);
        D->peers = std::move(G.peers); D->send_off = std::move(G.send_off); D->recv_off = std::move(G.recv_off);
        s->halos.push_back(std::move(D));
    }
    s->d_sendbuf.alloc(H.send_floats, s->dev_bytes);
    s->d_recvbuf.alloc(H.recv_floats, s->dev_bytes);
    if (H.recv_floats) HIP_CHECK(hipMemset(s->d_recvbuf.p, 0, H.recv_floats * sizeof(float)));
    s->fused_unpack = H.fused_unpack;
    if (s->peer.enabled && L.world > 1) alloc_mailbox(s, H.mailbox);
}

}
```

softbodyunity_amd/csrc/tile_kernel.hip.hpp:

```cpp
#pragma once
#include "device_math.hip.hpp"

namespace sbk {

__device__ __forceinline__ void lds_barrier() { asm volatile("s_waitcnt lgkmcnt(0)\n\ts_barrier" ::: "memory"); }

template <bool QUADS, int THREADS> constexpr int kWavesPerSimd = QUADS ? (THREADS == 64 ? 3 : (THREADS == 512 ? 2 : 4)) : (THREADS == 256 ? 8 : (THREADS == 128 ? 6 : 4));
template <int KIND_, bool QUADS, int THREADS, int PPT, bool WPAL, int HALO = kHaloNone>
__global__ __launch_bounds__(THREADS, (kWavesPerSimd<QUADS, THREADS> - (KIND_ == 5 && !QUADS ? 1 : 0))) void tile_kernel(const TileDesc *tiles_at_base, int n_workgroups, TileArgs A) {
    constexpr int KIND = KIND_ == 5 ? 1 : KIND_;
    constexpr bool KIN = KIND_ == 5;
    constexpr bool GHOSTS = HALO == kHaloGhosts;
    constexpr int kTileThreads = THREADS;
    constexpr int kCPL = THREADS >= kRoundSlots ? 1 : kRoundSlots / THREADS;
    extern __shared__ uint4 lds_raw[];
    float4 *lds_pos = reinterpret_cast<float4 *>(lds_raw);
    uint32_t *s_rounds = reinterpret_cast<uint32_t *>(lds_pos + A.max_local);
    float *s_pal = reinterpret_cast<float *>(s_rounds + A.rounds_dwords);
    uint32_t *cbuf = s_rounds + A.rounds_dwords + A.pal_dwords;
    f32x3 *lds_spare = reinterpret_cast<f32x3 *>(cbuf + A.win_dwords);
    typedef const TileDesc __attribute__((address_space(4))) *ConstTileDescPtr;
#ifndef SB_NO_XCD_REMAP
    const int nwg = n_workgroups, wg = (int)blockIdx.x;
    const int xq = nwg >> 3, xr = nwg & 7, xcd = wg & 7;
    const int tile_index = (xcd < xr ? xcd * (xq + 1) : xr * (xq + 1) + (xcd - xr) * xq) + (wg >> 3);
#else
    const int tile_index = (int)blockIdx.x;
#endif
    const TileDesc __attribute__((address_space(4))) &td = *((ConstTileDescPtr)(uintptr_t)tiles_at_base + tile_index);
    const int n_rounds_all = td.n_rounds;
    const int tid = threadIdx.x;
    const int n_local = td.n_local;
    const int run_count = td.run_count;
    const TickParams tp = *A.tp;
    const uint32_t *tstream = A.stream + td.s_begin;
#if defined(SB_ABLATE) && SB_ABLATE == 4
    if (n_local >= 0) { if (n_rounds_all == 0x7fffffff) A.vel[0] = tp.h; return; }
#endif

    int g[PPT];
    if (KIND == 3) {
#pragma unroll
        for (int m = 0; m < PPT; ++m) {
            const int l = tid + m * kTileThreads;
            g[m] = l < n_local ? A.gather[td.gather_begin + l] : -1;
        }
    } else {
        int run_d[kInlineRuns], run_y[kInlineRuns];
#pragma unroll
        for (int r = 0; r < kInlineRuns; ++r) { run_y[r] = td.runs[r].y; run_d[r] = td.runs[r].x - td.runs[r].y; }
#pragma unroll
        for (int m = 0; m < PPT; ++m) {
            const int l = tid + m * kTileThreads;
            int d = run_d[0];
#pragma unroll
            for (int r = 1; r < kInlineRuns; ++r) d = l >= run_y[r] ? run_d[r] : d;
            int gi = l + d;
            if (run_count > kInlineRuns)
                for (int r = kInlineRuns; r < run_count; ++r) {
                    const int2 rn = A.runs_overflow[td.run_overflow + r - kInlineRuns];
                    if (rn.y <= l) gi = rn.x + (l - rn.y);
                }
            g[m] = l < n_local ? gi : -1;
        }
    }
    const int R = n_rounds_all;
    const int v_begin = KIND == 0 ? R : 0;
    const int v_end = KIND == 3 ? R : (KIND == 2 || KIND == 4 ? R + 1 : 2 * R + 1);
    const uint32_t d_lo = td.s_hdr;
    const uint32_t d_hi = td.s_len;
    const uint32_t win = (uint32_t)A.win_dwords;
    uint32_t win_lo = d_lo;
    auto load_window = [&](uint32_t lo) {
        const uint32_t n4 = (min(lo + win, d_hi) - lo) >> 2;
        const uint4 *src = reinterpret_cast<const uint4 *>(tstream + lo);
        uint4 *dst = reinterpret_cast<uint4 *>(cbuf);
        uint32_t t0 = (uint32_t)tid;
        asm volatile("" : "+v"(t0));
        for (uint32_t i = t0; i < n4; i += 4 * kTileThreads) {
            uint4 v0 = src[i], v1, v2, v3;
            const bool b1 = i + kTileThreads < n4, b2 = i + 2 * kTileThreads < n4, b3 = i + 3 * kTileThreads < n4;
            if (b1) v1 = src[i + kTileThreads];
            if (b2) v2 = src[i + 2 * kTileThreads];
            if (b3) v3 = src[i + 3 * kTileThreads];
            dst[i] = v0;
            if (b1) dst[i + kTileThreads] = v1;
            if (b2) dst[i + 2 * kTileThreads] = v2;
            if (b3) dst[i + 3 * kTileThreads] = v3;
        }
    };
    f32x4 X[PPT];
    float pvx[PPT], pvy[PPT], pvz[PPT];
    uint32_t wi[PPT];
    const int mypal = WPAL ? __float_as_int(A.wpal[tid & (kMaxMassPalette - 1)]) : 0;
#pragma unroll
    for (int m = 0; m < PPT; ++m) {
        const int gc = max(g[m], 0);
        const bool ghost = GHOSTS && gc >= A.n_owned;
        const float *px = ghost ? A.ghost_src + 6 * (size_t)(gc - A.n_owned) : A.pos.xyz + 3 * (size_t)gc;
        X[m].x = px[0]; X[m].y = px[1]; X[m].z = px[2];
        if (WPAL) { wi[m] = A.w8[A.w_uniform ? 0 : gc]; X[m].w = 0.0f; } else { wi[m] = 0; X[m].w = A.pos.w[gc]; }
        pvx[m] = pvy[m] = pvz[m] = 0.0f;
        if (KIND != 0 && KIND != 3 && KIND != 4) {
            const float *pp = ghost ? px + 3 : A.prev + 3 * (size_t)gc;
            pvx[m] = pp[0]; pvy[m] = pp[1]; pvz[m] = pp[2];
        }
    }
    const bool rounds_in_lds = n_rounds_all <= A.rounds_dwords;
    const uint32_t rw = tstream[max(min(tid, n_rounds_all - 1), 0)];
    const bool rounds_in_lanes = n_rounds_all <= 64;
    const uint32_t rwl = tstream[max(min(tid & 63, n_rounds_all - 1), 0)];
    uint32_t itreg = 0;
    if (QUADS && kTileThreads == 64 * A.item_waves) {
        const int ns = td.n_steps;
        itreg = tstream[ns > 0 ? td.s_items + (uint32_t)((tid >> 6) * ns + min(tid & 63, ns - 1)) : 0u];
    }
    const int n_pal = td.n_pal;
    const uint32_t palw = tstream[tid < n_pal ? ((n_rounds_all + 3) & ~3) + tid : 0];
#ifndef SB_KW
#define SB_KW (QUADS ? 4 : 2)
#endif
    constexpr int kW = SB_KW;
    const bool lane_packed = !QUADS && kTileThreads == kLanePackLanes && td.packed_lanes == (uint32_t)kLanePackLanes;
    const bool lane_packed_full = !WPAL && lane_packed && td.n_pal == 0;
    const bool wide_packed = !QUADS && kTileThreads == kWidePackLanes && td.packed_lanes == (uint32_t)kWidePackLanes;
    const bool any_packed = lane_packed || wide_packed;
    const uint32_t n4_first = wide_packed ? 0u : lane_packed ? (lane_packed_full ? 2u * (uint32_t)kLanePackLanes : (uint32_t)kLanePackLanes)
                                          : (min(win_lo + win, d_hi) - win_lo) >> 2;
    const u32x4 *wsrc = reinterpret_cast<const u32x4 *>(tstream + win_lo);
    u32x4 wv[kW];
#pragma unroll
    for (int q = 0; q < kW; ++q) {
        const uint32_t i = tid + q * kTileThreads;
        wv[q] = i < n4_first ? wsrc[i] : *reinterpret_cast<const u32x4 *>(tstream);
    }
    typedef uint32_t u32x2 __attribute__((ext_vector_type(2)));
    u32x2 wc = {0u, 0u};
    u32x2 wp = {0u, 0u};
    if (!QUADS && kTileThreads == kWidePackLanes)
        wp = *reinterpret_cast<const u32x2 *>(wide_packed ? tstream + win_lo + 2u * (uint32_t)tid : tstream);
#pragma unroll
    for (int m = 0; m < PPT; ++m) asm volatile("" ::"v"(X[m].x), "v"(pvx[m]), "v"(wi[m]), "v"(X[m].w));
    asm volatile("" ::"v"(mypal));
    if (WPAL) {
#pragma unroll
        for (int m = 0; m < PPT; ++m) X[m].w = __int_as_float(__builtin_amdgcn_ds_bpermute((int)(wi[m] << 2), mypal));
    }
#pragma unroll
    for (int q = 0; q < kW; ++q) asm volatile("" ::"v"(wv[q].x));
    asm volatile("" ::"v"(rw), "v"(palw), "v"(rwl), "v"(itreg));
    if (!QUADS && kTileThreads == kWidePackLanes) asm volatile("" ::"v"(wp.x));
#pragma unroll
    for (int m = 0; m < PPT; ++m)
        if (g[m] >= 0) *reinterpret_cast<f32x4 *>(lds_pos + tid + m * kTileThreads) = X[m];
    if (rounds_in_lds && tid < n_rounds_all) s_rounds[tid] = rw;
    if (tid < n_pal) s_pal[tid] = __uint_as_float(palw);
    if (kTileThreads < kMaxRoundsLds && rounds_in_lds)
        for (int q = tid + kTileThreads; q < n_rounds_all; q += kTileThreads) s_rounds[q] = tstream[q];
    if (kTileThreads < kMaxPalette)
        for (int q = tid + kTileThreads; q < n_pal; q += kTileThreads) s_pal[q] = __uint_as_float(tstream[((n_rounds_all + 3) & ~3) + q]);
    {
        u32x4 *dst = reinterpret_cast<u32x4 *>(cbuf);
#pragma unroll
        for (int q = 0; q < kW; ++q) {
            const uint32_t i = tid + q * kTileThreads;
            if (i < n4_first && !any_packed) dst[i] = wv[q];
        }
        if (!any_packed)
            for (uint32_t i = tid + kW * kTileThreads; i < n4_first; i += kTileThreads) dst[i] = wsrc[i];
    }
    __syncthreads();
    if (!WPAL && !QUADS && kTileThreads == kLanePackLanes && lane_packed_full)
        wc = *reinterpret_cast<const u32x2 *>(tstream + win_lo + 8u * (uint32_t)kLanePackLanes + 2u * (uint32_t)tid);
#if defined(SB_ABLATE) && SB_ABLATE == 5
    if (n_local >= 0) { if (lds_pos[tid].x == 1.2345e-30f && cbuf[tid] == 0x12345678u) A.vel[0] = tp.h; return; }
#endif

    auto mark_step = [&]() {
#pragma unroll
        for (int m = 0; m < PPT; ++m)
            if (g[m] >= 0) {
                const int l = tid + m * kTileThreads;
                float4 P = lds_pos[l];
                if (KIND != 0 && tp.plane_on && P.w > 0.0f) {
                    float a = tp.pnx * P.x, b = tp.pny * P.y, c = tp.pnz * P.z;
                    float pen = ((a + b) + c) - tp.pd;
                    if (pen < 0.0f) {
                        float dx = pen * tp.pnx, dy = pen * tp.pny, dz = pen * tp.pnz;
                        P.x = P.x - dx; P.y = P.y - dy; P.z = P.z - dz;
                        if (KIND == 2 || KIND == 4) lds_pos[l] = P;
                    }
                }
                if (KIND == 4) continue;
                float vx, vy, vz;
                const size_t o = 3 * (size_t)g[m];
                if (KIND == 0) {
                    vx = A.vel[o + 0]; vy = A.vel[o + 1]; vz = A.vel[o + 2];
                } else {
                    float dx = P.x - pvx[m], dy = P.y - pvy[m], dz = P.z - pvz[m];
                    float qx = dx * tp.inv_h, qy = dy * tp.inv_h, qz = dz * tp.inv_h;
                    vx = qx * tp.kd; vy = qy * tp.kd; vz = qz * tp.kd;
                }
                bool moved = false;
                if (KIN && P.w == 0.0f) {
                    const int ks = A.kin_map[g[m]];
                    if (ks >= 0) {
                        float *t = A.kin_target + 3 * (size_t)ks;
                        const float tx = t[0], ty = t[1], tz = t[2];
                        if (tx == tx) { P.x = tx; P.y = ty; P.z = tz; moved = true; t[0] = __int_as_float(0x7fc00000); }
                    }
                }
                if (KIND == 2) {
                    A.vel[o + 0] = vx; A.vel[o + 1] = vy; A.vel[o + 2] = vz;
                } else {
                    if (A.store_through & 1) store3_through(A.prev + o, P.x, P.y, P.z);
                    else { A.prev[o + 0] = P.x; A.prev[o + 1] = P.y; A.prev[o + 2] = P.z; }
                    if (P.w > 0.0f) {
                        vx = vx + tp.hgx; vy = vy + tp.hgy; vz = vz + tp.hgz;
                        float hx = tp.h * vx, hy = tp.h * vy, hz = tp.h * vz;
                        P.x = P.x + hx; P.y = P.y + hy; P.z = P.z + hz;
                        lds_pos[l] = P;
                    } else if (KIN && moved) lds_pos[l] = P;
                }
            }
    };

    constexpr int kRegRounds = THREADS >= 256 ? kRegRoundsWide : kRegRoundsNarrow;
    if (kRegRounds > 0 && !QUADS && n_rounds_all <= kRegRounds && n_rounds_all > 0 && (kRegFullSlots || n_pal > 0) && (any_packed || d_hi - d_lo <= win)) {
        const bool tile_compact = n_pal > 0;
        uint32_t rs[kRegRounds > 0 ? kRegRounds : 1][kCPL];
        float rl[kRegRounds > 0 ? kRegRounds : 1][kCPL];
        int rcnt[kRegRounds > 0 ? kRegRounds : 1];
        {
            uint32_t o = 0;
#pragma unroll
            for (int r = 0; r < kRegRounds; ++r) {
                rcnt[r] = 0;
                if (r < n_rounds_all) {
                    rcnt[r] = (int)((uint32_t)__builtin_amdgcn_readlane((int)rwl, r) & 1023u);
                    if (kCPL == 2 && lane_packed) {
#pragma unroll
                        for (int u = 0; u < kCPL; ++u) {
                            const int bit = kLanePackFieldBits * (2 * r + u), w0 = bit >> 5, sh = bit & 31;
                            const uint32_t lo = wv[0][w0] >> sh;
                            const uint32_t hi = (sh + kLanePackFieldBits > 32) ? (wv[0][w0 + 1 < 4 ? w0 + 1 : 3] << ((32 - sh) & 31)) : 0u;
                            const uint32_t f = (lo | hi) & ((1u << kLanePackFieldBits) - 1u);
                            rs[r][u] = (f & 511u) | (((f >> 9) & 511u) << 12) | ((f >> 18) << 24);
                            if (!WPAL) {
                                const int fld = 2 * r + u;
                                rl[r][u] = __uint_as_float(fld < 4 ? wv[1][fld < 4 ? fld : 0] : wc[fld >= 4 ? fld - 4 : 0]);
                            }
                        }
                    } else if (kCPL == 1 && wide_packed) {
                        const uint64_t two = (uint64_t)wp.x | ((uint64_t)wp.y << 32);
                        const uint32_t f = (uint32_t)(two >> (kLanePackFieldBits * (r < kLanePackRounds ? r : 0))) & ((1u << kLanePackFieldBits) - 1u);
                        rs[r][0] = (f & 511u) | (((f >> 9) & 511u) << 12) | ((f >> 18) << 24);
                    } else if (tile_compact) {
#pragma unroll
                        for (int u = 0; u < kCPL; ++u) {
                            const int c = tid + u * kTileThreads;
                            rs[r][u] = cbuf[o + (c < rcnt[r] ? c : 0)];
                        }
                        o += ((uint32_t)rcnt[r] + 3u) & ~3u;
                    } else {
#pragma unroll
                        for (int u = 0; u < kCPL; ++u) {
                            const int c = tid + u * kTileThreads;
                            const uint2 e = *reinterpret_cast<const uint2 *>(cbuf + o + 2 * (c < rcnt[r] ? c : 0));
                            rs[r][u] = (e.x & 0xfffu) | ((e.x >> 16) << 12);
                            rl[r][u] = __uint_as_float(e.y);
                        }
                        o += (2u * (uint32_t)rcnt[r] + 3u) & ~3u;
                    }
                } else {
#pragma unroll
                    for (int u = 0; u < kCPL; ++u) { rs[r][u] = 0; rl[r][u] = 0.0f; }
                }
            }
            if (tile_compact) {
#pragma unroll
                for (int r = 0; r < kRegRounds; ++r)
#pragma unroll
                    for (int u = 0; u < kCPL; ++u) rl[r][u] = s_pal[rs[r][u] >> 24];
            }
        }
        auto reg_round = [&](const uint32_t (&e)[kCPL], const float (&L0)[kCPL], int cnt) {
            if (kCPL == 1) {
                if (tid < cnt) {
                    const int i = e[0] & 0xfffu, k = (e[0] >> 12) & 0xfffu;
                    float4 a = lds_pos[i], b = lds_pos[k];
                    if (project_distance(a, b, L0[0], tp.at_d)) { lds_pos[i] = a; lds_pos[k] = b; }
                }
            } else {
                int ci[kCPL], ck[kCPL];
                bool con[kCPL];
                f32x4 ca[kCPL], cb[kCPL];
#pragma unroll
                for (int u = 0; u < kCPL; ++u) {
                    con[u] = tid + u * kTileThreads < cnt;
                    ci[u] = e[u] & 0xfffu; ck[u] = (e[u] >> 12) & 0xfffu;
                    ca[u] = *reinterpret_cast<const f32x4 *>(lds_pos + ci[u]);
                    cb[u] = *reinterpret_cast<const f32x4 *>(lds_pos + ck[u]);
                }
#pragma unroll
                for (int u = 0; u < kCPL; ++u) {
                    float4 a = make_float4(ca[u].x, ca[u].y, ca[u].z, ca[u].w), b = make_float4(cb[u].x, cb[u].y, cb[u].z, cb[u].w);
                    con[u] = project_distance_nobranch(a, b, L0[u], tp.at_d) && con[u];
                    ca[u].x = a.x; ca[u].y = a.y; ca[u].z = a.z; cb[u].x = b.x; cb[u].y = b.y; cb[u].z = b.z;
                }
#pragma unroll
                for (int u = 0; u < kCPL; ++u) {
                    f32x3 *da = con[u] ? reinterpret_cast<f32x3 *>(lds_pos + ci[u]) : lds_spare;
                    f32x3 *db = con[u] ? reinterpret_cast<f32x3 *>(lds_pos + ck[u]) : lds_spare;
                    *da = (f32x3){ca[u].x, ca[u].y, ca[u].z};
                    *db = (f32x3){cb[u].x, cb[u].y, cb[u].z};
                }
            }
            lds_barrier();
        };
#if defined(SB_ABLATE) && SB_ABLATE == 1
        constexpr bool kRunRounds = false;
#else
        constexpr bool kRunRounds = true;
#endif
        if (KIND != 0 && kRunRounds) {
#pragma unroll
            for (int r = 0; r < kRegRounds; ++r) if (r < n_rounds_all) reg_round(rs[r], rl[r], rcnt[r]);
        }
        if (KIND != 3) { mark_step(); lds_barrier(); }
        if ((KIND == 0 || KIND == 1) && kRunRounds) {
#pragma unroll
            for (int r = 0; r < kRegRounds; ++r) if (r < n_rounds_all) reg_round(rs[r], rl[r], rcnt[r]);
        }
    } else if (QUADS && kTileThreads == 64 * A.item_waves && td.n_steps > 0 && d_hi - d_lo <= win) {
        const int n_steps = td.n_steps;
        const int wave = __builtin_amdgcn_readfirstlane(tid >> 6), lane = tid & 63;
        const uint32_t *items = tstream + td.s_items + (uint32_t)(wave * n_steps);
        float *lds_f = reinterpret_cast<float *>(lds_pos);
        const int q = tid & 3;
        auto run_pass = [&]() {
            if (n_steps > 64) itreg = items[min(lane, n_steps - 1)];
#if defined(SB_ABLATE) && SB_ABLATE == 1
            if (n_steps >= 0) return;
#endif
#pragma unroll 1
            for (int st = 0; st < n_steps; ++st) {
                if ((st & 63) == 0 && st > 0) itreg = items[min(st + lane, n_steps - 1)];
                const uint32_t it = (uint32_t)__builtin_amdgcn_readlane((int)itreg, st & 63);
                const uint32_t type = it & 7u;
                const int cnt = (int)((it >> kItemCountShift) & 127u);
                const uint32_t *slots = cbuf + (it >> kItemOffsetShift);
                if (type == kItemBending) {
                    const int c = lane >> 4;
                    if (c < cnt) {
                        const uint4 e = *reinterpret_cast<const uint4 *>(slots + 4 * c);
                        const int k = (lane >> 2) & 3;
                        const int o0 = 4 * (int)(e.x & 0xffffu) + q, o1 = 4 * (int)(e.x >> 16) + q;
                        const int o2 = 4 * (int)(e.y & 0xffffu) + q, o3 = 4 * (int)(e.y >> 16) + q;
                        const float P[4] = {lds_f[o0], lds_f[o1], lds_f[o2], lds_f[o3]};
                        float Xk = k == 0 ? P[0] : (k == 1 ? P[1] : (k == 2 ? P[2] : P[3]));
                        const int ok_off = k == 0 ? o0 : (k == 1 ? o1 : (k == 2 ? o2 : o3));
#if defined(SB_ABLATE) && SB_ABLATE == 2
                        const bool ok = true; Xk += __uint_as_float(e.z) * P[1];
#else
                        const bool ok = project_bending_row(P, __uint_as_float(e.z), __uint_as_float(e.w), tp.at_b, k, (lane & 48) << 2, Xk);
#endif
                        if (ok && q < 3) lds_f[ok_off] = Xk;
                    }
// ... 26 lines not shown
#if defined(SB_ABLATE) && SB_ABLATE == 2
                        a.x += L0; b.x -= tp.at_d; lds_pos[i] = a; lds_pos[k] = b;
#else
                        if (project_distance(a, b, L0, tp.at_d)) { lds_pos[i] = a; lds_pos[k] = b; }
#endif
                    }
                }
                if (it & (1u << kItemBarrierBit)) lds_barrier();
            }
        };
        if (KIND != 0) run_pass();
        if (KIND != 3) { mark_step(); lds_barrier(); }
        if (KIND == 0 || KIND == 1) run_pass();
    } else {
    uint32_t off = d_lo;
#if defined(SB_ABLATE) && SB_ABLATE == 1
    for (int v = v_begin; v < v_end; v += 100000) {
#else
    for (int v = v_begin; v < v_end; ++v) {
#endif
        if (v == R) { mark_step(); lds_barrier(); continue; }
        const int r = v < R ? v : v - R - 1;
        if (v == R + 1) off = d_lo;
        uint32_t w;
        if (rounds_in_lanes) w = (uint32_t)__builtin_amdgcn_readlane((int)rwl, __builtin_amdgcn_readfirstlane(r));
        else if (rounds_in_lds) w = (uint32_t)__builtin_amdgcn_readfirstlane((int)s_rounds[r]);
        else w = (uint32_t)__builtin_amdgcn_readfirstlane((int)tstream[r]);
        const int cnt = w & 1023u, n_vol = (w >> 10) & 1023u, n_bend = (w >> 20) & 1023u;
        const bool compact = (w >> 30) & 1u;
        const uint32_t dsize = compact ? ((cnt + 3u) & ~3u) : ((2u * cnt + 3u) & ~3u);
        const uint32_t size = dsize + 4u * (uint32_t)(n_vol + n_bend);
        if (off + size > win_lo + win || off < win_lo) {
            lds_barrier();
            win_lo = off;
            load_window(win_lo);
            __syncthreads();
        }
        const uint32_t *base = cbuf + (off - win_lo);
        if (QUADS) {
            const int wave = __builtin_amdgcn_readfirstlane(tid >> 6), lane = tid & 63;
            const int n_wb = (n_bend + 15) >> 4, n_wv = (n_vol + 15) >> 4, n_wd = (cnt + 63) >> 6;
            const uint32_t *qbase = base + dsize;
            float *lds_f = reinterpret_cast<float *>(lds_pos);
            const int q = tid & 3;
            constexpr int kWavesPerTile = kTileThreads / 64;
            const int n_slots = n_wb + n_wv + n_wd;
#pragma unroll 1
            for (int row = 0; row * kWavesPerTile < n_slots; ++row) {
                const int sw = row * kWavesPerTile + ((row & 1) ? kWavesPerTile - 1 - wave : wave);
                if (sw >= n_slots) continue;
                if (sw < n_wb + n_wv) {
                    const bool bend = sw < n_wb;
                    const int c = (bend ? sw : sw - n_wb) * 16 + (lane >> 2);
                    if (c < (bend ? n_bend : n_vol)) {
                        const uint4 e = *reinterpret_cast<const uint4 *>(qbase + 4 * (bend ? n_vol + c : c));
                        const int o0 = 4 * (int)(e.x & 0xffffu) + q, o1 = 4 * (int)(e.x >> 16) + q;
                        const int o2 = 4 * (int)(e.y & 0xffffu) + q, o3 = 4 * (int)(e.y >> 16) + q;
                        float P[4] = {lds_f[o0], lds_f[o1], lds_f[o2], lds_f[o3]};
                        const bool ok = bend ? project_bending_quad(P, __uint_as_float(e.z), __uint_as_float(e.w), tp.at_b, q)
                                             : project_volume_quad(P, __uint_as_float(e.z), tp.at_v);
                        if (ok && q < 3) { lds_f[o0] = P[0]; lds_f[o1] = P[1]; lds_f[o2] = P[2]; lds_f[o3] = P[3]; }
                    }
                } else {
                    const int c = (sw - n_wb - n_wv) * 64 + lane;
                    if (c < cnt) {
                        int i, k;
                        float L0;
                        if (compact) {
                            const uint32_t e = base[c];
                            i = e & 0xfffu; k = (e >> 12) & 0xfffu; L0 = s_pal[e >> 24];
                        } else {
                            const uint2 e = *reinterpret_cast<const uint2 *>(base + 2 * c);
                            i = e.x & 0xffffu; k = e.x >> 16; L0 = __uint_as_float(e.y);
                        }
                        float4 a = lds_pos[i], b = lds_pos[k];
                        if (project_distance(a, b, L0, tp.at_d)) { lds_pos[i] = a; lds_pos[k] = b; }
                    }
                }
            }
        } else if (kCPL == 1) {
            if (tid < cnt) {
                int i, k;
                float L0;
                if (compact) {
                    const uint32_t e = base[tid];
                    i = e & 0xfffu; k = (e >> 12) & 0xfffu; L0 = s_pal[e >> 24];
                } else {
                    const uint2 e = *reinterpret_cast<const uint2 *>(base + 2 * tid);
                    i = e.x & 0xffffu; k = e.x >> 16; L0 = __uint_as_float(e.y);
                }
                float4 a = lds_pos[i], b = lds_pos[k];
#if defined(SB_ABLATE) && SB_ABLATE == 2
                a.x += L0; b.x -= tp.at_d;
                lds_pos[i] = a; lds_pos[k] = b;
#else
                if (project_distance(a, b, L0, tp.at_d)) { lds_pos[i] = a; lds_pos[k] = b; }
#endif
            }
        } else {
            int ci[kCPL], ck[kCPL];
            float cL0[kCPL];
            bool con[kCPL];
            f32x4 ca[kCPL], cb[kCPL];
            if (!compact) {
#pragma unroll
                for (int u = 0; u < kCPL; ++u) {
                    const int c = tid + u * kTileThreads;
                    con[u] = c < cnt;
                    const uint2 e = *reinterpret_cast<const uint2 *>(base + 2 * (con[u] ? c : 0));
                    ci[u] = e.x & 0xffffu; ck[u] = e.x >> 16; cL0[u] = __uint_as_float(e.y);
                }
            } else {
                uint32_t ce[kCPL];
#pragma unroll
                for (int u = 0; u < kCPL; ++u) {
                    const int c = tid + u * kTileThreads;
                    con[u] = c < cnt;
                    ce[u] = base[con[u] ? c : 0];
                }
#pragma unroll
                for (int u = 0; u < kCPL; ++u) { ci[u] = ce[u] & 0xfffu; ck[u] = (ce[u] >> 12) & 0xfffu; cL0[u] = s_pal[ce[u] >> 24]; }
            }
#pragma unroll
            for (int u = 0; u < kCPL; ++u) {
                ca[u] = *reinterpret_cast<const f32x4 *>(lds_pos + ci[u]);
                cb[u] = *reinterpret_cast<const f32x4 *>(lds_pos + ck[u]);
            }
#pragma unroll
            for (int u = 0; u < kCPL; ++u) {
                float4 a = make_float4(ca[u].x, ca[u].y, ca[u].z, ca[u].w), b = make_float4(cb[u].x, cb[u].y, cb[u].z, cb[u].w);
                con[u] = project_distance_nobranch(a, b, cL0[u], tp.at_d) && con[u];
                ca[u].x = a.x; ca[u].y = a.y; ca[u].z = a.z; cb[u].x = b.x; cb[u].y = b.y; cb[u].z = b.z;
            }
#pragma unroll
            for (int u = 0; u < kCPL; ++u) {
                f32x3 *da = con[u] ? reinterpret_cast<f32x3 *>(lds_pos + ci[u]) : lds_spare;
                f32x3 *db = con[u] ? reinterpret_cast<f32x3 *>(lds_pos + ck[u]) : lds_spare;
                *da = (f32x3){ca[u].x, ca[u].y, ca[u].z};
                *db = (f32x3){cb[u].x, cb[u].y, cb[u].z};
            }
        }
        off += size;
#if defined(SB_ABLATE) && SB_ABLATE == 3
        asm volatile("s_waitcnt lgkmcnt(0)" ::: "memory");
#else
        lds_barrier();
#endif
    }
    }
#pragma unroll
    for (int m = 0; m < PPT; ++m)
        if (g[m] >= 0) {
            const float4 P = lds_pos[tid + m * kTileThreads];
            if (KIND == 4) { float *o = A.peek_out + 3 * (size_t)g[m]; o[0] = P.x; o[1] = P.y; o[2] = P.z; }
            else if (A.store_through & 2) store3_through(A.pos.xyz + 3 * (size_t)g[m], P.x, P.y, P.z);
            else pv_store(A.pos, g[m], P);
        }
}


}
```

softbodyunity_amd/csrc/validate.hip:

```cpp
#include "solver_internal.hpp"
#include "validate_kernels.hip.hpp"

using namespace sbi;

extern "C" {

int sb_debug_validate(sb_solver *s, int32_t inject_fault, sb_validate_report *out) {
    if (!s || !out) return fail(SB_ERR_INVALID_ARG, "sb_debug_validate: null argument");
    if (!s->finalized) return fail(SB_ERR_STATE, "sb_debug_validate before sb_finalize");
    if (inject_fault < 0 || inject_fault > 2) return fail(SB_ERR_INVALID_ARG, "sb_debug_validate: inject_fault must be 0, 1 or 2");
    std::memset(out, 0, sizeof(*out));
    out->first_stage = out->first_tile = out->first_group = out->first_kind = -1;
    return guarded([&]() -> int {
        int rc = set_device(s); if (rc) return rc;
        int64_t acct = 0;
        DevBuf<int32_t> owner; owner.alloc((size_t)std::max<int64_t>(s->n_local, 1), acct);
        DevBuf<sbk::ValidateCounters> d_cnt; d_cnt.alloc(1, acct);
        sbk::ValidateCounters zero{}; zero.first[0] = zero.first[1] = zero.first[2] = zero.first[3] = -1;
        auto stage = [&](int which, auto &&launch) {
            HIP_CHECK(hipMemcpyAsync(d_cnt.p, &zero, sizeof(zero), hipMemcpyHostToDevice, s->stream));
            HIP_CHECK(hipMemsetAsync(owner.p, 0xff, owner.count * sizeof(int32_t), s->stream));
            launch();
            HIP_CHECK(hipGetLastError());
            sbk::ValidateCounters c{};
            HIP_CHECK(hipMemcpyAsync(&c, d_cnt.p, sizeof(c), hipMemcpyDeviceToHost, s->stream));
            HIP_CHECK(hipStreamSynchronize(s->stream));
            out->tiles_checked += (int64_t)c.tiles; out->groups_checked += (int64_t)c.groups; out->constraints_checked += (int64_t)c.constraints;
            bool any = false;
            for (int k = 0; k < 6; ++k) { out->errors[k] += c.errors[k]; any |= c.errors[k] != 0; }
            if (any && out->first_stage < 0) { out->first_stage = which; out->first_tile = c.first[0]; out->first_group = c.first[1]; out->first_kind = c.first[2]; }
        };
        auto tiles_launch = [&](DevTiling &D, int tl, int begin, int end, const sbk::TileDesc *tiles, const uint32_t *stream) {
            if (end <= begin) return;
            hipLaunchKernelGGL(sbk::validate_tiles_kernel, dim3((unsigned)(end - begin)), dim3(sbk::kValidateThreads), 0, s->stream, tiles, begin,
                               D.runs_overflow.p, stream, D.gather.p, tl == 2 ? 1 : 0, (int)s->n_local, (int)D.item_waves, owner.p, d_cnt.p);
        };
        if (inject_fault) {
            DevTiling &D = s->tiling[0];
            if (D.n_tiles < 2) return fail(SB_ERR_STATE, "sb_debug_validate: fault injection needs a tiling of at least two tiles");
            std::vector<sbk::TileDesc> tiles((size_t)D.n_tiles);
            HIP_CHECK(hipMemcpy(tiles.data(), D.tiles.p, tiles.size() * sizeof(sbk::TileDesc), hipMemcpyDeviceToHost));
            DevBuf<sbk::TileDesc> t_copy; DevBuf<uint32_t> s_copy;
            s_copy.alloc(D.stream.count, acct);
            HIP_CHECK(hipMemcpy(s_copy.p, D.stream.p, D.stream.count * sizeof(uint32_t), hipMemcpyDeviceToDevice));
            if (inject_fault == 2) tiles[1] = tiles[0];
            else {
                bool planted = false;
                for (size_t t = 0; t < tiles.size() && !planted; ++t) {
                    const sbk::TileDesc &td = tiles[t];
                    std::vector<uint32_t> words((size_t)std::max(td.n_rounds, 1));
                    HIP_CHECK(hipMemcpy(words.data(), D.stream.p + td.s_begin, words.size() * sizeof(uint32_t), hipMemcpyDeviceToHost));
                    uint32_t off = td.s_hdr;
                    if (td.packed_lanes && td.n_rounds > 0 && (words[0] & 1023u) >= 2) {
                        uint32_t *base = s_copy.p + td.s_begin + off;
                        const size_t lane_dwords = td.packed_lanes == (uint32_t)sbk::kWidePackLanes ? 2 : 4;
                        HIP_CHECK(hipMemcpy(base + lane_dwords, base, lane_dwords * sizeof(uint32_t), hipMemcpyDeviceToDevice));
                        planted = true;
                    }
                    for (int r = 0; r < td.n_rounds && !planted && !td.packed_lanes; ++r) {
                        const uint32_t w = words[(size_t)r], cnt = w & 1023u, nq = ((w >> 10) & 1023u) + ((w >> 20) & 1023u);
                        const bool compact = (w >> 30) & 1u;
                        const uint32_t dsize = compact ? ((cnt + 3u) & ~3u) : ((2u * cnt + 3u) & ~3u);
                        uint32_t *base = s_copy.p + td.s_begin + off;
                        if (cnt >= 2) { HIP_CHECK(hipMemcpy(base + (compact ? 1 : 2), base, (compact ? 1 : 2) * sizeof(uint32_t), hipMemcpyDeviceToDevice)); planted = true; }
                        else if (nq >= 2) { HIP_CHECK(hipMemcpy(base + dsize + 4, base + dsize, 4 * sizeof(uint32_t), hipMemcpyDeviceToDevice)); planted = true; }
                        off += dsize + 4u * nq;
                    }
                }
                if (!planted) return fail(SB_ERR_STATE, "sb_debug_validate: no group with two constraints of one type to plant the fault in");
            }
            t_copy.upload(tiles, acct);
            stage(0, [&] { tiles_launch(D, 0, 0, D.n_tiles, t_copy.p, s_copy.p); });
            return SB_OK;
        }
        for (int tl = 0; tl < 2; ++tl) {
            DevTiling &D = s->tiling[tl];
            if (D.n_tiles) stage(tl, [&] { tiles_launch(D, tl, 0, D.n_tiles, D.tiles.p, D.stream.p); });
        }
        for (const auto &rg : s->t2_layer_range) {
            DevTiling &D = s->tiling[2];
            stage(2, [&] { tiles_launch(D, 2, rg.first, rg.second, D.tiles.p, D.stream.p); });
        }
        for (size_t gc = 0; gc < s->gcolours.size(); ++gc) {
            DevGColour &G = *s->gcolours[gc];
            if (!G.count) continue;
            stage(3, [&] {
                const int per = G.type == 0 ? 2 : 4;
                const int32_t *idx = G.type == 0 ? reinterpret_cast<const int32_t *>(G.ij.p) : reinterpret_cast<const int32_t *>(G.quad.p);
                hipLaunchKernelGGL(sbk::validate_gcolour_kernel, dim3((unsigned)((G.count + 255) / 256)), dim3(256), 0, s->stream, idx, per, (int)G.count,
                                   (int)s->n_local, (int)gc, owner.p, d_cnt.p);
            });
        }
        return SB_OK;
    });
}

}
```

softbodyunity_amd/native.py:

```python
import ctypes as C
import os

import numpy as np

_HERE = os.path.dirname(os.path.abspath(__file__))
_VARIANT = os.environ.get("SB_LIB_VARIANT", "")
LIB_PATH = os.path.join(_HERE, f"libsoftbody_mi355x{'_' + _VARIANT if _VARIANT else ''}.so")

SB_UNIQUE_ID_BYTES = 128
SB_IPC_HANDLE_BYTES = 64
SB_OK = 0
SB_PARTITION_AUTO, SB_PARTITION_BLOCKS, SB_PARTITION_RCB = 0, 1, 2
SB_PLAN_NO_T2, SB_PLAN_NO_THIRD_LIST, SB_PLAN_NO_CLUSTER_LAYERS, SB_PLAN_NO_MIXED_GROUPS, SB_PLAN_NO_BANK_ORDER, SB_PLAN_NO_TILE_MERGE = 1, 2, 4, 8, 16, 32
SB_TRANSPORT_RCCL, SB_TRANSPORT_PEER = 0, 1
SB_SCHEDULE_AUTO, SB_SCHEDULE_SERIAL_EAGER, SB_SCHEDULE_SERIAL_GRAPH, SB_SCHEDULE_OVERLAP_EAGER, SB_SCHEDULE_OVERLAP_GRAPH = 0, 1, 2, 3, 4
SB_DEBUG_NO_COMM, SB_DEBUG_LOOPBACK = 1, 2
SB_GROUP_WALK = 1
SB_GROUP_WHOLE_MESH = 2
(SB_TUNE_NO_MASS_PALETTE, SB_TUNE_NO_UNIFORM_MASS, SB_TUNE_NO_PALETTE, SB_TUNE_NO_WAVE_ITEMS, SB_TUNE_NO_LANE_PACK, SB_TUNE_NO_COST_ORDER,
 SB_TUNE_NO_FUSED_UNPACK, SB_TUNE_PEER_COARSE, SB_TUNE_NO_LAZY_TICK, SB_TUNE_NO_PACK, SB_TUNE_NO_PEEK, SB_TUNE_NO_KIN_FUSE,
 SB_TUNE_NO_WIDE_SLOTS, SB_TUNE_AUTO_PREFER_OVERLAP, SB_TUNE_NO_AUTO_CALIBRATION, SB_TUNE_NO_SHARED_PROGRAMS) = (1 << k for k in range(16))
SB_ERR_INVALID_ARG, SB_ERR_STATE, SB_ERR_NO_DEVICE, SB_ERR_HIP, SB_ERR_RCCL, SB_ERR_NOMEM, SB_ERR_UNSUPPORTED = \
    -1, -2, -3, -4, -5, -6, -7


class SbDesc(C.Structure):
    _fields_ = [("device", C.c_int32), ("rank", C.c_int32), ("world", C.c_int32), ("part_dims", C.c_int32 * 3),
                ("gravity", C.c_float * 3), ("damping", C.c_float), ("tile_particles", C.c_int32),
                ("use_graph", C.c_int32), ("partition", C.c_int32), ("plan_flags", C.c_uint32),
                ("halo_transport", C.c_int32), ("halo_schedule", C.c_int32), ("debug_flags", C.c_uint32),
                ("reserved", C.c_int32 * 3)]


class SbTuning(C.Structure):
    _fields_ = [("flags", C.c_uint32), ("tile_lanes", C.c_int32), ("quad_lanes", C.c_int32), ("narrow_min_tiles", C.c_int32),
                ("store_through_max_tiles", C.c_int32), ("store_through_large", C.c_int32), ("peek_min_tiles", C.c_int32),
                ("lds_pad_bytes", C.c_int32), ("win_dwords", C.c_int32), ("prev_offset_bytes", C.c_int32), ("reserved", C.c_int32 * 6)]


class SbExchangeTiming(C.Structure):
    _fields_ = [("exchanges", C.c_int64), ("pack_ms", C.c_double), ("transport_ms", C.c_double), ("total_ms", C.c_double), ("exposed_wait_ms", C.c_double)]


class SbStats(C.Structure):
    _fields_ = [("n_particles_owned", C.c_int64), ("n_particles_local", C.c_int64),
                ("n_constraints_local", C.c_int64 * 3), ("n_tilings", C.c_int32), ("n_global_colours", C.c_int32),
                ("n_tiles", C.c_int64 * 2), ("tile_constraints", C.c_int64 * 2), ("constraints_in_tiles", C.c_int64),
                ("constraints_in_global", C.c_int64), ("halo_particles_t1", C.c_int64),
                ("halo_particles_global", C.c_int64), ("device_bytes", C.c_int64),
                ("n_t2_layers", C.c_int64), ("n_t2_tiles", C.c_int64), ("t2_constraints", C.c_int64),
                ("launch_bytes", C.c_int64 * 5), ("partition", C.c_int32), ("halo_peers", C.c_int32),
                ("partition_cost", C.c_int64), ("partition_cost_max", C.c_int64), ("partition_cost_total", C.c_int64),
                ("halo_particles_recv", C.c_int64), ("plan_hash", C.c_uint64), ("halo_schedule", C.c_int32),
                ("halo_unpack_fused", C.c_int32), ("readback_peeks", C.c_int64), ("readback_peek_tiles", C.c_int64), ("ticks_fused", C.c_int64), ("ticks_fused_kinematic", C.c_int64), ("lane_packed_tiles", C.c_int64 * 2),
                ("halo_auto_state", C.c_int32), ("halo_auto_ticks", C.c_int32), ("halo_auto_ms", C.c_double * 2)]

    def as_dict(self):
        out = {}
        for name, _ in self._fields_:
            v = getattr(self, name)
            out[name] = list(v) if hasattr(v, "__len__") else v
        return out


class SbValidateReport(C.Structure):
    _fields_ = [("tiles_checked", C.c_int64), ("groups_checked", C.c_int64), ("constraints_checked", C.c_int64), ("errors", C.c_int64 * 6),
                ("first_stage", C.c_int32), ("first_tile", C.c_int32), ("first_group", C.c_int32), ("first_kind", C.c_int32)]


class SbDomain(C.Structure):
    _fields_ = [("n_global", C.c_int64), ("lo", C.c_double * 3), ("hi", C.c_double * 3), ("spacing", C.c_double), ("fill", C.c_double),
                ("four_vertex_constraints", C.c_int32), ("reserved", C.c_int32)]


class SbPlanOpts(C.Structure):
    _fields_ = [("rank", C.c_int32), ("world", C.c_int32), ("part_dims", C.c_int32 * 3), ("tile_particles", C.c_int32),
                ("partition", C.c_int32), ("plan_flags", C.c_uint32), ("domain", C.POINTER(SbDomain)), ("global_id", C.c_void_p)]


class SbRuntimeInfo(C.Structure):
    _fields_ = [("hip_runtime_version", C.c_int32), ("hip_driver_version", C.c_int32), ("rccl_version", C.c_int32),
                ("rccl_header_version", C.c_int32), ("rccl_was_resident", C.c_int32), ("capture_serial_ok", C.c_int32),
                ("capture_overlap_ok", C.c_int32), ("reserved", C.c_int32), ("hip_library", C.c_char * 256),
                ("rccl_library", C.c_char * 256)]


class SbPhaseInfo(C.Structure):
    _fields_ = [("kind", C.c_int32), ("type", C.c_int32), ("tiling", C.c_int32), ("halo_slot", C.c_int32),
                ("order_begin", C.c_int64), ("order_end", C.c_int64), ("task_begin", C.c_int64), ("task_end", C.c_int64)]


_P = C.c_void_p
SIGNATURES = {
    "sb_desc_default": (None, [C.POINTER(SbDesc)]),
    "sb_create": (C.c_int, [C.POINTER(SbDesc), C.POINTER(_P)]),
    "sb_destroy": (C.c_int, [_P]),
    "sb_set_particles": (C.c_int, [_P, _P, _P, _P, C.c_int32]),
    "sb_set_rest_positions": (C.c_int, [_P, _P, C.c_int32]),
    "sb_set_distance_constraints": (C.c_int, [_P, _P, _P, C.c_int32, C.c_float]),
    "sb_set_volume_constraints": (C.c_int, [_P, _P, _P, C.c_int32, C.c_float]),
    "sb_set_bending_constraints": (C.c_int, [_P, _P, _P, C.c_int32, C.c_float]),
    "sb_set_ground_plane": (C.c_int, [_P, C.c_float, C.c_float, C.c_float, C.c_float, C.c_int32]),
    "sb_set_domain": (C.c_int, [_P, C.POINTER(SbDomain), _P, C.c_int32]),
    "sb_domain_from_mesh": (C.c_int, [_P, C.c_int32, _P, C.c_int32, _P, C.c_int32, _P, C.c_int32, C.POINTER(SbDomain)]),
    "sb_domain_window": (C.c_int, [C.POINTER(SbDomain), C.POINTER(SbPlanOpts), C.POINTER(C.c_double), C.POINTER(C.c_double)]),
    "sb_finalize": (C.c_int, [_P]),
    "sb_comm_unique_id": (C.c_int, [_P]),
    "sb_comm_init": (C.c_int, [_P, _P]),
    "sb_peer_mailbox_handle": (C.c_int, [_P, _P]),
    "sb_peer_connect": (C.c_int, [_P, C.c_int32, _P, _P]),
    "sb_step": (C.c_int, [_P, C.c_float, C.c_int32]),
    "sb_get_positions": (C.c_int, [_P, _P, C.c_int32]),
    "sb_get_velocities": (C.c_int, [_P, _P, C.c_int32]),
    "sb_set_kinematic_positions": (C.c_int, [_P, _P, _P, C.c_int32]),
    "sb_set_state": (C.c_int, [_P, _P, _P, C.c_int32]),
    "sb_readback_begin": (C.c_int, [_P]),
    "sb_readback_end": (C.c_int, [_P, C.POINTER(C.POINTER(C.c_float))]),
    "sb_set_render_triangles": (C.c_int, [_P, C.POINTER(C.c_int32), C.c_int32]),
    "sb_set_render_embedding": (C.c_int, [_P, C.POINTER(C.c_int32), C.POINTER(C.c_float), C.c_int32, C.POINTER(C.c_int32), C.c_int32]),
    "sb_readback_get_normals": (C.c_int, [_P, C.POINTER(C.POINTER(C.c_float))]),
    "sb_set_readback_render_set_only": (C.c_int, [_P, C.c_int32]),
    "sb_readback_get_render_set": (C.c_int, [_P, C.POINTER(C.POINTER(C.c_int32)), C.POINTER(C.c_int32)]),
    "sb_get_owner": (C.c_int, [_P, _P, C.c_int32]),
    "sb_profile_begin": (C.c_int, [_P]),
    "sb_profile_end": (C.c_int, [_P, C.POINTER(C.c_float)]),
    "sb_synchronize": (C.c_int, [_P]),
    "sb_step_profiled": (C.c_int, [_P, C.c_float, C.c_int32, _P, _P, C.c_int32]),
    "sb_debug_launch": (C.c_int, [_P, C.c_float, C.c_int32, C.c_int32, C.c_int32]),
    "sb_debug_halo_pack": (C.c_int, [_P, C.c_int32, _P, C.c_int64, C.POINTER(C.c_int64)]),
    "sb_debug_halo_unpack": (C.c_int, [_P, C.c_int32, _P, C.c_int64]),
    "sb_debug_validate": (C.c_int, [_P, C.c_int32, C.POINTER(SbValidateReport)]),
    "sb_get_stats": (C.c_int, [_P, C.POINTER(SbStats)]),
    "sb_plan_build": (C.c_int, [_P, C.c_int32, _P, C.c_int32, _P, C.c_int32, _P, C.c_int32, C.POINTER(SbPlanOpts),
                                C.POINTER(_P)]),
    "sb_plan_destroy": (C.c_int, [_P]),
    "sb_get_plan": (C.c_int, [_P, C.POINTER(_P)]),
    "sb_plan_order_count": (C.c_int64, [_P]),
    "sb_plan_get_order": (C.c_int, [_P, C.c_int32, _P, _P]),
    "sb_plan_phase_count": (C.c_int32, [_P, C.c_int32]),
    "sb_plan_get_phases": (C.c_int, [_P, C.c_int32, C.POINTER(SbPhaseInfo)]),
    "sb_plan_task_count": (C.c_int64, [_P, C.c_int32]),
    "sb_plan_get_tasks": (C.c_int, [_P, C.c_int32, _P]),
    "sb_plan_group_count": (C.c_int64, [_P, C.c_int32]),
    "sb_plan_get_groups": (C.c_int, [_P, C.c_int32, _P]),
    "sb_plan_get_owner": (C.c_int, [_P, _P]),
    "sb_plan_local_count": (C.c_int64, [_P, C.POINTER(C.c_int64)]),
    "sb_plan_get_local_particles": (C.c_int, [_P, _P]),
    "sb_plan_halo_slot_count": (C.c_int32, [_P]),
    "sb_plan_halo_counts": (C.c_int, [_P, C.c_int32, _P, _P]),
    "sb_plan_get_halo": (C.c_int, [_P, C.c_int32, C.c_int32, _P, _P]),
    "sb_plan_get_pair_hashes": (C.c_int, [_P, _P]),
    "sb_plan_get_local_order_mask": (C.c_int, [_P, C.c_int32, _P]),
    "sb_runtime_info": (C.c_int, [C.POINTER(SbRuntimeInfo)]),
    "sb_tuning_default": (None, [C.POINTER(SbTuning)]),
    "sb_set_tuning": (C.c_int, [_P, C.POINTER(SbTuning)]),
    "sb_debug_exchange_timing": (C.c_int, [_P, C.c_int32]),
    "sb_debug_exchange_timing_read": (C.c_int, [_P, C.POINTER(SbExchangeTiming)]),
    "sb_debug_last_words": (C.c_int, [C.c_int32, C.c_char_p, C.c_int64, C.c_int32]),
    "sb_group_create": (C.c_int, [C.POINTER(SbDesc), _P, C.c_int32, C.c_uint32, C.POINTER(_P)]),
    "sb_group_destroy": (C.c_int, [_P]),
    "sb_group_set_particles": (C.c_int, [_P, _P, _P, _P, C.c_int32]),
    "sb_group_set_rest_positions": (C.c_int, [_P, _P, C.c_int32]),
    "sb_group_set_distance_constraints": (C.c_int, [_P, _P, _P, C.c_int32, C.c_float]),
    "sb_group_set_volume_constraints": (C.c_int, [_P, _P, _P, C.c_int32, C.c_float]),
    "sb_group_set_bending_constraints": (C.c_int, [_P, _P, _P, C.c_int32, C.c_float]),
    "sb_group_set_ground_plane": (C.c_int, [_P, C.c_float, C.c_float, C.c_float, C.c_float, C.c_int32]),
    "sb_group_finalize": (C.c_int, [_P]),
    "sb_group_step": (C.c_int, [_P, C.c_float, C.c_int32]),
    "sb_group_get_positions": (C.c_int, [_P, _P, C.c_int32]),
    "sb_group_get_velocities": (C.c_int, [_P, _P, C.c_int32]),
    "sb_group_set_state": (C.c_int, [_P, _P, _P, C.c_int32]),
    "sb_group_set_kinematic_positions": (C.c_int, [_P, _P, _P, C.c_int32]),
    "sb_group_set_render_triangles": (C.c_int, [_P, C.POINTER(C.c_int32), C.c_int32]),
    "sb_group_set_render_embedding": (C.c_int, [_P, C.POINTER(C.c_int32), C.POINTER(C.c_float), C.c_int32, C.POINTER(C.c_int32), C.c_int32]),
    "sb_group_set_readback_render_set_only": (C.c_int, [_P, C.c_int32]),
    "sb_group_readback_begin": (C.c_int, [_P]),
    "sb_group_readback_end": (C.c_int, [_P, C.POINTER(C.POINTER(C.c_float))]),
    "sb_group_readback_get_normals": (C.c_int, [_P, C.POINTER(C.POINTER(C.c_float))]),
    "sb_group_readback_get_render_set": (C.c_int, [_P, C.POINTER(C.POINTER(C.c_int32)), C.POINTER(C.c_int32)]),
    "sb_group_synchronize": (C.c_int, [_P]),
    "sb_group_rank_count": (C.c_int32, [_P]),
    "sb_group_get_rank": (C.c_int, [_P, C.c_int32, C.POINTER(_P)]),
    "sb_last_error": (C.c_char_p, []),
    "sb_abi_version": (C.c_int, []),
}

_lib = None


class SoftbodyError(RuntimeError):
    def __init__(self, code, msg):
        super().__init__(f"softbody_mi355x error {code}: {msg}")
        self.code = code


def lib():
    global _lib
    if _lib is None:
        if not os.path.exists(LIB_PATH):
            raise FileNotFoundError(
                f"{LIB_PATH} is missing: build it with `python -c 'import __graft_entry__ as g; g.build()'` "
                "(softbodyunity_amd has no CPU fallback)")
        L = C.CDLL(LIB_PATH)
        for name, (res, args) in SIGNATURES.items():
            fn = getattr(L, name)
            fn.restype = res
            fn.argtypes = args
        _lib = L
    return _lib


def check(rc):
    if rc != SB_OK:
        raise SoftbodyError(rc, lib().sb_last_error().decode("utf-8", "replace"))


def ptr(a):
    return None if a is None else a.ctypes.data_as(C.c_void_p)


def f32(a, shape=None):
    a = np.ascontiguousarray(a, dtype=np.float32)
    return a if shape is None else a.reshape(shape)


def i32(a, shape=None):
    a = np.ascontiguousarray(a, dtype=np.int32)
    return a if shape is None else a.reshape(shape)


_PLAN_FLAG_ENV = (("SB_NO_T2", SB_PLAN_NO_T2), ("SB_NO_THIRD_LIST", SB_PLAN_NO_THIRD_LIST),
                  ("SB_NO_CLUSTER_LAYERS", SB_PLAN_NO_CLUSTER_LAYERS), ("SB_NO_MIXED_GROUPS", SB_PLAN_NO_MIXED_GROUPS),
                  ("SB_NO_BANK_ORDER", SB_PLAN_NO_BANK_ORDER), ("SB_NO_TILE_MERGE", SB_PLAN_NO_TILE_MERGE))


def plan_flags_from_env():
    lists = int(os.environ.get("SB_BALANCED_LISTS", "0") or 0) & 3
    return sum(bit for name, bit in _PLAN_FLAG_ENV if os.environ.get(name)) | (lists << 8)


def halo_transport_from_env():
    return SB_TRANSPORT_PEER if os.environ.get("SB_HALO_TRANSPORT") == "peer" else SB_TRANSPORT_RCCL


def halo_schedule_from_env():
    overlap, graph = bool(os.environ.get("SB_HALO_OVERLAP")), bool(os.environ.get("SB_GRAPH_RCCL"))
    if not overlap and not graph:
        return SB_SCHEDULE_AUTO
    return (SB_SCHEDULE_OVERLAP_GRAPH if graph else SB_SCHEDULE_OVERLAP_EAGER) if overlap else SB_SCHEDULE_SERIAL_GRAPH


def debug_flags_from_env():
    return (SB_DEBUG_NO_COMM if os.environ.get("SB_TEST_NO_COMM") else 0) | (SB_DEBUG_LOOPBACK if os.environ.get("SB_TEST_LOOPBACK") else 0)


_TUNE_FLAG_ENV = (("SB_NO_MASS_PALETTE", SB_TUNE_NO_MASS_PALETTE), ("SB_NO_UNIFORM_MASS", SB_TUNE_NO_UNIFORM_MASS), ("SB_NO_PALETTE", SB_TUNE_NO_PALETTE),
                  ("SB_NO_WAVE_ITEMS", SB_TUNE_NO_WAVE_ITEMS), ("SB_NO_LANE_PACK", SB_TUNE_NO_LANE_PACK), ("SB_NO_COST_ORDER", SB_TUNE_NO_COST_ORDER),
                  ("SB_NO_FUSED_UNPACK", SB_TUNE_NO_FUSED_UNPACK), ("SB_PEER_COARSE", SB_TUNE_PEER_COARSE), ("SB_NO_LAZY_TICK", SB_TUNE_NO_LAZY_TICK),
                  ("SB_NO_PACK", SB_TUNE_NO_PACK), ("SB_NO_PEEK", SB_TUNE_NO_PEEK), ("SB_NO_KIN_FUSE", SB_TUNE_NO_KIN_FUSE),
                  ("SB_NO_WIDE_SLOTS", SB_TUNE_NO_WIDE_SLOTS), ("SB_AUTO_PREFER_OVERLAP", SB_TUNE_AUTO_PREFER_OVERLAP),
                  ("SB_NO_AUTO_CALIBRATION", SB_TUNE_NO_AUTO_CALIBRATION), ("SB_NO_SHARED_PROGRAMS", SB_TUNE_NO_SHARED_PROGRAMS))
_TUNE_INT_ENV = (("SB_TILE_LANES", "tile_lanes"), ("SB_QUAD_LANES", "quad_lanes"), ("SB_NARROW_MIN_TILES", "narrow_min_tiles"),
                 ("SB_STORE_THROUGH_MAX_TILES", "store_through_max_tiles"), ("SB_STORE_THROUGH_LARGE", "store_through_large"),
                 ("SB_PEEK_MIN_TILES", "peek_min_tiles"), ("SB_LDS_PAD", "lds_pad_bytes"), ("SB_WIN_DWORDS", "win_dwords"),
                 ("SB_PREV_OFFSET", "prev_offset_bytes"))


def tuning_from_env():
    t = SbTuning()
    lib().sb_tuning_default(C.byref(t))
    any_set = False
    for name, bit in _TUNE_FLAG_ENV:
        if os.environ.get(name):
            t.flags |= bit; any_set = True
    for name, field in _TUNE_INT_ENV:
        v = os.environ.get(name)
        if v not in (None, ""):
            setattr(t, field, int(v)); any_set = True
    return t if any_set else None


def runtime_info():
    ri = SbRuntimeInfo()
    check(lib().sb_runtime_info(C.byref(ri)))
    return {"hip_runtime_version": ri.hip_runtime_version, "hip_driver_version": ri.hip_driver_version,
            "rccl_version": ri.rccl_version, "rccl_header_version": ri.rccl_header_version,
            "rccl_was_resident": bool(ri.rccl_was_resident), "capture_serial_ok": bool(ri.capture_serial_ok),
            "capture_overlap_ok": bool(ri.capture_overlap_ok), "hip_library": ri.hip_library.decode(),
            "rccl_library": ri.rccl_library.decode()}


def domain_from_mesh(rest_pos, dist_ij=None, vol_ijkl=None, bend_ijkl=None):
    rest = f32(rest_pos, (-1, 3))
    d = i32(dist_ij if dist_ij is not None else np.zeros((0, 2)), (-1, 2))
    v = i32(vol_ijkl if vol_ijkl is not None else np.zeros((0, 4)), (-1, 4))
    b = i32(bend_ijkl if bend_ijkl is not None else np.zeros((0, 4)), (-1, 4))
    out = SbDomain()
    check(lib().sb_domain_from_mesh(ptr(rest), rest.shape[0], ptr(d), d.shape[0], ptr(v), v.shape[0], ptr(b), b.shape[0], C.byref(out)))
    return out


def make_domain(n_global, lo, hi, spacing, four_vertex_constraints=False):
    d = SbDomain()
    d.n_global = int(n_global); d.lo[:] = [float(c) for c in lo]; d.hi[:] = [float(c) for c in hi]
    d.spacing = float(spacing); d.fill = 1.0; d.four_vertex_constraints = 1 if four_vertex_constraints else 0
    return d


def domain_window(domain, rank, world, part_dims=(0, 0, 0), tile_particles=0):
    o = SbPlanOpts(rank, world, (C.c_int32 * 3)(*part_dims), tile_particles, SB_PARTITION_BLOCKS, 0, None, None)
    lo = (C.c_double * 3)(); hi = (C.c_double * 3)()
    check(lib().sb_domain_window(C.byref(domain), C.byref(o), lo, hi))
    return np.array(lo[:]), np.array(hi[:])


class Plan:

    def __init__(self, handle, owned):
        self._h = C.c_void_p(handle)
        self._owned = owned

    @classmethod
    def build(cls, rest_pos, dist_ij=None, vol_ijkl=None, bend_ijkl=None, rank=0, world=1, part_dims=(0, 0, 0),
              tile_particles=0, partition=SB_PARTITION_AUTO, plan_flags=None, domain=None, global_id=None):
        L = lib()
        rest = f32(rest_pos, (-1, 3))
        d = i32(dist_ij if dist_ij is not None else np.zeros((0, 2)), (-1, 2))
        v = i32(vol_ijkl if vol_ijkl is not None else np.zeros((0, 4)), (-1, 4))
        b = i32(bend_ijkl if bend_ijkl is not None else np.zeros((0, 4)), (-1, 4))
        gid = None if global_id is None else i32(global_id, (-1,))
        o = SbPlanOpts(rank, world, (C.c_int32 * 3)(*part_dims), tile_particles, partition,
                       plan_flags_from_env() if plan_flags is None else plan_flags,
                       C.pointer(domain) if domain is not None else None, ptr(gid))
        h = C.c_void_p()
        check(L.sb_plan_build(ptr(rest), rest.shape[0], ptr(d), d.shape[0], ptr(v), v.shape[0], ptr(b), b.shape[0],
                              C.byref(o), C.byref(h)))
        p = cls(h.value, True)
        p.n = rest.shape[0]
        p.world = world
        return p

    def close(self):
        if self._owned and self._h:
            lib().sb_plan_destroy(self._h)
        self._h = None

    def __del__(self):
        try:
            self.close()
        except Exception:
            pass

    def order(self, parity=0):
        L = lib()
        m = L.sb_plan_order_count(self._h)
        t = np.zeros(m, np.uint8); ids = np.zeros(m, np.int32)
        check(L.sb_plan_get_order(self._h, parity, ptr(t), ptr(ids)))
        return t, ids

    def phases(self, parity=0):
        L = lib()
        k = L.sb_plan_phase_count(self._h, parity)
        arr = (SbPhaseInfo * k)()
        check(L.sb_plan_get_phases(self._h, parity, arr))
        return [dict(kind=a.kind, type=a.type, tiling=a.tiling, halo_slot=a.halo_slot, order_begin=a.order_begin,
                     order_end=a.order_end, task_begin=a.task_begin, task_end=a.task_end) for a in arr]

    def tasks(self, parity=0):
        L = lib()
        k = L.sb_plan_task_count(self._h, parity)
        out = np.zeros(k + 1, np.int64)
        check(L.sb_plan_get_tasks(self._h, parity, ptr(out)))
        return out

    def groups(self, parity=0):
        L = lib()
        k = L.sb_plan_group_count(self._h, parity)
        out = np.zeros(k + 1, np.int64)
        check(L.sb_plan_get_groups(self._h, parity, ptr(out)))
        return out

    def phase_task_offsets(self, parity=0):
        ph = self.phases(parity)
        if not ph:
            return np.zeros(1, np.int64)
        return np.array([p["task_begin"] for p in ph] + [ph[-1]["task_end"]], np.int64)

    def owner(self, n):
        out = np.zeros(n, np.int32)
        check(lib().sb_plan_get_owner(self._h, ptr(out)))
        return out

    def local_particles(self):
        L = lib()
        owned = C.c_int64()
        k = L.sb_plan_local_count(self._h, C.byref(owned))
        out = np.zeros(k, np.int32)
        check(L.sb_plan_get_local_particles(self._h, ptr(out)))
        return out, owned.value

    def halo_slot_count(self):
        return lib().sb_plan_halo_slot_count(self._h)

    def halo(self, slot, world):
        L = lib()
        sc = np.zeros(world, np.int32); rc = np.zeros(world, np.int32)
        check(L.sb_plan_halo_counts(self._h, slot, ptr(sc), ptr(rc)))
        out = {}
        for peer in range(world):
            if sc[peer] == 0 and rc[peer] == 0:
                continue
            s = np.zeros(sc[peer], np.int32); r = np.zeros(rc[peer], np.int32)
            check(L.sb_plan_get_halo(self._h, slot, peer, ptr(s), ptr(r)))
            out[peer] = (s, r)
# ... 14 lines not shown
```

softbodyunity_amd/softbody.py:

```python
import ctypes as C
import os

import numpy as np

from . import native
from .native import check, f32, i32, ptr


class Softbody:
    def __init__(self, mesh, substeps=20, fixed_delta_time=0.02, gravity=(0.0, -9.81, 0.0), damping=0.0,
                 distance_compliance=0.0, volume_compliance=0.0, bending_compliance=0.0, device=0, rank=0, world=1,
                 part_dims=(0, 0, 0), tile_particles=0, use_graph=True, unique_id=None, ground_plane=None, use_gpu=True,
                 partition=native.SB_PARTITION_AUTO, plan_flags=None, halo_transport=None, halo_schedule=None, debug_flags=None, tuning=None):
        self.mesh = mesh
        self.substeps = int(substeps)
        self.fixed_delta_time = float(fixed_delta_time)
        self.gravity = tuple(float(g) for g in gravity)
        self.damping = float(damping)
        self.compliance = (float(distance_compliance), float(volume_compliance), float(bending_compliance))
        self.device, self.rank, self.world = int(device), int(rank), int(world)
        self.part_dims = tuple(int(d) for d in part_dims)
        self.tile_particles = int(tile_particles)
        self.use_graph = bool(use_graph)
        self.partition = int(partition)
# ... 35 lines not shown
        check(L.sb_create(C.byref(d), C.byref(h)))
        self._h = h
        try:
            tune = native.tuning_from_env() if self.tuning is None else self.tuning
            if tune is not None:
                check(L.sb_set_tuning(h, C.byref(tune)))
            self._author(L, h)
        except Exception:
            self.OnDestroy()
            raise
        return self

    def _author(self, L, h):
        m = self.mesh
        pos = f32(m.pos, (-1, 3)); vel = f32(m.vel, (-1, 3)); w = f32(m.inv_mass, (-1,))
        self.n = pos.shape[0]
        check(L.sb_set_particles(h, ptr(pos), ptr(vel), ptr(w), self.n))
        if m.rest_pos is not None:
            rest = f32(m.rest_pos, (-1, 3))
            check(L.sb_set_rest_positions(h, ptr(rest), self.n))
        if len(m.dist_rest):
            ij = i32(m.dist_ij, (-1, 2)); r = f32(m.dist_rest, (-1,))
            check(L.sb_set_distance_constraints(h, ptr(ij), ptr(r), r.shape[0], self.compliance[0]))
        if len(m.vol_rest):
            q = i32(m.vol_ijkl, (-1, 4)); r = f32(m.vol_rest, (-1,))
            check(L.sb_set_volume_constraints(h, ptr(q), ptr(r), r.shape[0], self.compliance[1]))
        if len(m.bend_rest):
            q = i32(m.bend_ijkl, (-1, 4)); r = f32(m.bend_rest, (-1, 2))
            check(L.sb_set_bending_constraints(h, ptr(q), ptr(r), r.shape[0], self.compliance[2]))
        peer_only = self.halo_transport == native.SB_TRANSPORT_PEER and self.unique_id is None
        if self.world > 1 and not (self.debug_flags & native.SB_DEBUG_NO_COMM) and not peer_only:
            assert self.unique_id is not None and len(self.unique_id) == native.SB_UNIQUE_ID_BYTES
            buf = (C.c_uint8 * native.SB_UNIQUE_ID_BYTES)(*self.unique_id)
            check(L.sb_comm_init(h, buf))
        if self.ground_plane is not None:
            check(L.sb_set_ground_plane(h, *[float(c) for c in self.ground_plane], 1))
        if getattr(m, "domain", None) is not None:
            gid = i32(m.global_id, (-1,))
            check(L.sb_set_domain(h, C.byref(m.domain), ptr(gid), self.n))
        check(L.sb_finalize(h))
        self.vertices = pos.copy()

    def cpu_schedule(self):
        if self._cpu_plan is None:
            raise RuntimeError("cpu_schedule() needs use_gpu=False and Start()")
        return [self._cpu_plan.order(parity) for parity in (0, 1)]

    def FixedUpdate(self, readback=True):
        if not self.use_gpu:
            raise RuntimeError("softbodyunity_amd has no CPU execution path: the CPU tick is csharp/SoftbodyCpuSolver.cs "
                               "(tests drive the oracle with cpu_schedule())")
        check(native.lib().sb_step(self._h, self.fixed_delta_time, self.substeps))
        if readback:
            self.get_positions(self.vertices)
        return self.vertices

    def OnDestroy(self):
        if self._cpu_plan is not None:
            self._cpu_plan.close()
            self._cpu_plan = None
        if self._h is not None:
            native.lib().sb_destroy(self._h)
            self._h = None

    def __enter__(self):
        return self.Start()

    def __exit__(self, *a):
        self.OnDestroy()

    def step(self, dt=None, substeps=None):
        check(native.lib().sb_step(self._h, self.fixed_delta_time if dt is None else dt,
                                   self.substeps if substeps is None else substeps))

    def synchronize(self):
        check(native.lib().sb_synchronize(self._h))

    def peer_mailbox_handle(self):
        out = np.zeros(native.SB_IPC_HANDLE_BYTES, np.uint8)
        check(native.lib().sb_peer_mailbox_handle(self._h, ptr(out)))
        return out

    def peer_connect(self, rank, handle):
        h = np.ascontiguousarray(handle, np.uint8)
        assert h.shape == (native.SB_IPC_HANDLE_BYTES,)
        check(native.lib().sb_peer_connect(self._h, int(rank), ptr(h), None))

    def get_positions(self, out=None):
        out = np.zeros((self.n, 3), np.float32) if out is None else out
        check(native.lib().sb_get_positions(self._h, ptr(out), self.n))
        return out

    def get_velocities(self, out=None):
        out = np.zeros((self.n, 3), np.float32) if out is None else out
        check(native.lib().sb_get_velocities(self._h, ptr(out), self.n))
        return out

    def readback_begin(self):
        check(native.lib().sb_readback_begin(self._h))

    def readback_end(self, normals=False):
        p = C.POINTER(C.c_float)()
        check(native.lib().sb_readback_end(self._h, C.byref(p)))
        rows = self.n
        if self._embedded:
            rows = self._embedded
        elif self._render_set_only:
            rows = len(self.render_set())
        pos = np.ctypeslib.as_array(p, shape=(rows, 3))
        if not normals:
            return pos
        q = C.POINTER(C.c_float)()
        check(native.lib().sb_readback_get_normals(self._h, C.byref(q)))
        return pos, np.ctypeslib.as_array(q, shape=(rows, 3))

    def set_readback_render_set_only(self, on=True):
        check(native.lib().sb_set_readback_render_set_only(self._h, 1 if on else 0))
        self._render_set_only = bool(on)

    def render_set(self):
        ids = C.POINTER(C.c_int32)(); cnt = C.c_int32()
        check(native.lib().sb_readback_get_render_set(self._h, C.byref(ids), C.byref(cnt)))
        return np.ctypeslib.as_array(ids, shape=(cnt.value,)) if cnt.value else np.zeros(0, np.int32)

    def set_render_triangles(self, tri):
        tri = np.ascontiguousarray(tri, dtype=np.int32).reshape(-1, 3)
        check(native.lib().sb_set_render_triangles(self._h, tri.ctypes.data_as(C.POINTER(C.c_int32)), tri.shape[0]))

    def set_render_embedding(self, cage, weights, tri=None):
        cage, weights, tri, m = _embedding_args(cage, weights, tri)
        check(native.lib().sb_set_render_embedding(self._h, _ip(cage), _fp(weights), m, _ip(tri), 0 if tri is None else tri.shape[0]))
        self._embedded = m

    def set_kinematic_positions(self, ids, pos):
        ids = i32(ids); pos = f32(pos, (-1, 3))
        assert pos.shape[0] == ids.shape[0]
        check(native.lib().sb_set_kinematic_positions(self._h, ptr(ids), ptr(pos), int(ids.shape[0])))

    def set_state(self, pos, vel):
        pos = f32(pos, (-1, 3)); vel = f32(vel, (-1, 3))
        check(native.lib().sb_set_state(self._h, ptr(pos), ptr(vel), self.n))

    def owner(self):
        out = np.zeros(self.n, np.int32)
        check(native.lib().sb_get_owner(self._h, ptr(out), self.n))
        return out

    def validate(self, inject_fault=0):
        rep = native.SbValidateReport()
        check(native.lib().sb_debug_validate(self._h, int(inject_fault), C.byref(rep)))
        return {"tiles_checked": rep.tiles_checked, "groups_checked": rep.groups_checked, "constraints_checked": rep.constraints_checked,
                "errors": list(rep.errors), "first_stage": rep.first_stage, "first_tile": rep.first_tile, "first_group": rep.first_group,
                "first_kind": rep.first_kind}

    def stats(self):
        st = native.SbStats()
        check(native.lib().sb_get_stats(self._h, C.byref(st)))
        return st.as_dict()

    def plan(self):
        h = C.c_void_p()
        check(native.lib().sb_get_plan(self._h, C.byref(h)))
        p = native.Plan(h.value, False)
        p.n = self.n
        p.world = self.world
        return p

    def step_profiled(self, dt=None, substeps=None):
        k = self.stats()["n_global_colours"] + 5
        ms = np.zeros(k, np.float32); cnt = np.zeros(k, np.int32)
        check(native.lib().sb_step_profiled(self._h, self.fixed_delta_time if dt is None else dt,
                                            self.substeps if substeps is None else substeps, ptr(ms), ptr(cnt), k))
        return ms, cnt

    def profile_begin(self):
        check(native.lib().sb_profile_begin(self._h))

    def exchange_timing(self, enabled):
        check(native.lib().sb_debug_exchange_timing(self._h, 1 if enabled else 0))

    def exchange_timing_read(self):
        t = native.SbExchangeTiming()
        check(native.lib().sb_debug_exchange_timing_read(self._h, C.byref(t)))
        return {"exchanges": t.exchanges, "pack_ms": t.pack_ms, "transport_ms": t.transport_ms, "total_ms": t.total_ms, "exposed_wait_ms": t.exposed_wait_ms}

    def profile_end(self):
        ms = C.c_float()
        check(native.lib().sb_profile_end(self._h, C.byref(ms)))
        return ms.value


def _embedding_args(cage, weights, tri):
    if cage is None:
        return None, None, None, 0
    cage = np.ascontiguousarray(cage, dtype=np.int32).reshape(-1, 4)
    weights = np.ascontiguousarray(weights, dtype=np.float32).reshape(-1, 4)
    assert cage.shape == weights.shape, "one row of four weights per row of four cage particles"
    if tri is not None:
        tri = np.ascontiguousarray(tri, dtype=np.int32).reshape(-1, 3)
    return cage, weights, tri, cage.shape[0]


def _ip(a):
    return None if a is None else a.ctypes.data_as(C.POINTER(C.c_int32))


def _fp(a):
    return None if a is None else a.ctypes.data_as(C.POINTER(C.c_float))


def comm_unique_id():
    buf = (C.c_uint8 * native.SB_UNIQUE_ID_BYTES)()
    check(native.lib().sb_comm_unique_id(buf))
    return bytes(buf)


class SoftbodyGroup:

    def __init__(self, mesh, devices, substeps=20, fixed_delta_time=0.02, gravity=(0.0, -9.81, 0.0), damping=0.0,
                 distance_compliance=0.0, volume_compliance=0.0, bending_compliance=0.0, part_dims=(0, 0, 0), tile_particles=0,
                 use_graph=True, ground_plane=None, partition=native.SB_PARTITION_AUTO, plan_flags=None,
                 halo_transport=native.SB_TRANSPORT_RCCL, halo_schedule=native.SB_SCHEDULE_AUTO, debug_flags=0, walk=False, tuning=None, whole_mesh=False):
        self.mesh = mesh
        self.whole_mesh = bool(whole_mesh)
        self.devices = [int(d) for d in devices]
        self.substeps, self.fixed_delta_time = int(substeps), float(fixed_delta_time)
        self.gravity, self.damping = tuple(float(g) for g in gravity), float(damping)
        self.compliance = (float(distance_compliance), float(volume_compliance), float(bending_compliance))
        self.part_dims, self.tile_particles, self.use_graph = tuple(int(d) for d in part_dims), int(tile_particles), bool(use_graph)
        self.ground_plane = ground_plane
        self.partition = int(partition)
        self.plan_flags = native.plan_flags_from_env() if plan_flags is None else int(plan_flags)
        self.halo_transport, self.halo_schedule, self.debug_flags = int(halo_transport), int(halo_schedule), int(debug_flags)
        self.walk = bool(walk)
        self.tuning = tuning
        self._g = None
        self._render_set_only = False
        self._embedded = 0
        self.vertices = None

    def Start(self):
        L = native.lib()
        d = native.SbDesc()
        L.sb_desc_default(C.byref(d))
        d.part_dims[:] = self.part_dims
        d.gravity[:] = self.gravity
        d.damping, d.tile_particles, d.use_graph = self.damping, self.tile_particles, 1 if self.use_graph else 0
        d.partition, d.plan_flags = self.partition, self.plan_flags
        d.halo_transport, d.halo_schedule, d.debug_flags = self.halo_transport, self.halo_schedule, self.debug_flags
        devs = (C.c_int32 * len(self.devices))(*self.devices)
        g = C.c_void_p()
        check(L.sb_group_create(C.byref(d), devs, len(self.devices), (native.SB_GROUP_WALK if self.walk else 0) | (native.SB_GROUP_WHOLE_MESH if self.whole_mesh else 0), C.byref(g)))
        self._g = g
        try:
            tune = native.tuning_from_env() if self.tuning is None else self.tuning
            if tune is not None:
                for r in range(len(self.devices)):
                    check(L.sb_set_tuning(self._rank_handle(r), C.byref(tune)))
            m = self.mesh
            pos = f32(m.pos, (-1, 3)); vel = f32(m.vel, (-1, 3)); w = f32(m.inv_mass, (-1,))
            self.n = pos.shape[0]
            check(L.sb_group_set_particles(g, ptr(pos), ptr(vel), ptr(w), self.n))
            if m.rest_pos is not None:
                rest = f32(m.rest_pos, (-1, 3))
                check(L.sb_group_set_rest_positions(g, ptr(rest), self.n))
            if len(m.dist_rest):
                ij = i32(m.dist_ij, (-1, 2)); r = f32(m.dist_rest, (-1,))
                check(L.sb_group_set_distance_constraints(g, ptr(ij), ptr(r), r.shape[0], self.compliance[0]))
            if len(m.vol_rest):
                q = i32(m.vol_ijkl, (-1, 4)); r = f32(m.vol_rest, (-1,))
                check(L.sb_group_set_volume_constraints(g, ptr(q), ptr(r), r.shape[0], self.compliance[1]))
            if len(m.bend_rest):
                q = i32(m.bend_ijkl, (-1, 4)); r = f32(m.bend_rest, (-1, 2))
                check(L.sb_group_set_bending_constraints(g, ptr(q), ptr(r), r.shape[0], self.compliance[2]))
            if self.ground_plane is not None:
                check(L.sb_group_set_ground_plane(g, *[float(c) for c in self.ground_plane], 1))
            check(L.sb_group_finalize(g))
            self.vertices = pos.copy()
        except Exception:
            self.OnDestroy()
            raise
        return self

    def FixedUpdate(self, readback=True):
        check(native.lib().sb_group_step(self._g, self.fixed_delta_time, self.substeps))
        if readback:
            self.get_positions(self.vertices)
        return self.vertices

    def OnDestroy(self):
        if self._g is not None:
            native.lib().sb_group_destroy(self._g)
            self._g = None

    def __enter__(self):
        return self.Start()

    def __exit__(self, *a):
        self.OnDestroy()

    def step(self, dt=None, substeps=None):
        check(native.lib().sb_group_step(self._g, self.fixed_delta_time if dt is None else dt, self.substeps if substeps is None else substeps))

    def synchronize(self):
        check(native.lib().sb_group_synchronize(self._g))

# ... 66 lines not shown
```

Before: 115.2 billion.

## Store previous positions as lossless 64-bit deltas against current positions

Previous positions are now written as one 8-byte word per particle, holding three 21-bit integer deltas scaled to the ulp of the current position, in place of 12 bytes of floats. The codec checks that decoding reproduces the exact bits. Particles whose delta does not fit are marked as escaped and fall back to the float prev array. The aim is to cut memory traffic in the bandwidth-bound tile kernels, at the cost of extra encode/decode ALU work, escape-path loads and a new kernel template variant. It is enabled only for single-rank runs with no global colours, no third tiling and no tets or hinges.

```diff
diff --git a/include/softbody_debug.h b/include/softbody_debug.h
--- a/include/softbody_debug.h
+++ b/include/softbody_debug.h
@@ -26,6 +26,7 @@
 #define SB_TUNE_AUTO_PREFER_OVERLAP (1u << 13)
 #define SB_TUNE_NO_AUTO_CALIBRATION (1u << 14)
 #define SB_TUNE_NO_SHARED_PROGRAMS (1u << 15)
+#define SB_TUNE_NO_PACKED_PREV     (1u << 16)
 typedef struct {
     uint32_t flags;
     int32_t tile_lanes;
@@ -66,6 +67,8 @@
 } sb_validate_report;
 int sb_debug_validate(sb_solver *s, int32_t inject_fault, sb_validate_report *out);
 
+int sb_debug_prev_escapes(sb_solver *s, uint64_t *escaped, uint64_t *total);
+
 int sb_debug_last_words(int32_t fd, const char *text, int64_t len, int32_t exit_code);
 
 #ifdef __cplusplus
diff --git a/softbodyunity_amd/csrc/abi.hip b/softbodyunity_amd/csrc/abi.hip
--- a/softbodyunity_amd/csrc/abi.hip
+++ b/softbodyunity_amd/csrc/abi.hip
@@ -60,7 +60,7 @@
 int sb_set_tuning(sb_solver *s, const sb_tuning *t) {
     if (!s || !t) return fail(SB_ERR_INVALID_ARG, "sb_set_tuning: null argument");
     if (s->finalized) return fail(SB_ERR_STATE, "sb_set_tuning after sb_finalize");
-    constexpr uint32_t kAll = (SB_TUNE_NO_SHARED_PROGRAMS << 1) - 1u;
+    constexpr uint32_t kAll = (SB_TUNE_NO_PACKED_PREV << 1) - 1u;
     if (t->flags & ~kAll) return fail(SB_ERR_INVALID_ARG, "sb_set_tuning: unknown bit in flags");
     for (int32_t r : t->reserved) if (r) return fail(SB_ERR_INVALID_ARG, "sb_set_tuning: reserved fields must be 0 (sb_tuning_default)");
     if (t->tile_lanes != 0 && t->tile_lanes != 128 && t->tile_lanes != 256 && t->tile_lanes != 512) return fail(SB_ERR_INVALID_ARG, "sb_set_tuning: tile_lanes must be 0, 128, 256 or 512");
@@ -541,15 +541,16 @@
     {
         const int64_t mb = s->w_uniform ? 0 : (s->w_palette ? 1 : 4);
         auto tables = [&](const DevTiling &D) { return D.stream_bytes + (int64_t)D.n_tiles * (int64_t)sizeof(sbk::TileDesc) + (int64_t)D.runs_overflow.count * 8; };
+        const int64_t pb = s->packed_prev ? 8 : 12;
         for (int tl = 0; tl < 2; ++tl) {
             const DevTiling &D = s->tiling[tl];
             if (!D.n_tiles) continue;
-            out->launch_bytes[tl] = D.staged_particles * (12 + mb + 12 + 12 + 12) + tables(D);
+            out->launch_bytes[tl] = D.staged_particles * (12 + mb + pb + 12 + pb) + tables(D);
         }
         const DevTiling &D0 = s->tiling[0];
         if (D0.n_tiles) {
-            out->launch_bytes[2] = D0.staged_particles * (12 + mb + 12 + 12 + 12) + tables(D0);
-            out->launch_bytes[3] = D0.staged_particles * (12 + mb + 12 + 12 + 12) + tables(D0);
+            out->launch_bytes[2] = D0.staged_particles * (12 + mb + 12 + 12 + pb) + tables(D0);
+            out->launch_bytes[3] = D0.staged_particles * (12 + mb + pb + 12 + 12) + tables(D0);
         }
         const DevTiling &D2 = s->tiling[2];
         if (D2.n_tiles) out->launch_bytes[4] = D2.staged_particles * (4 + 12 + mb + 12) + tables(D2);
diff --git a/softbodyunity_amd/csrc/device_math.hip.hpp b/softbodyunity_amd/csrc/device_math.hip.hpp
--- a/softbodyunity_amd/csrc/device_math.hip.hpp
+++ b/softbodyunity_amd/csrc/device_math.hip.hpp
@@ -15,6 +15,11 @@
 __device__ __forceinline__ void store3_through(float *p, float x, float y, float z) {
     f32x3_t v = {x, y, z};
     asm volatile("global_store_dwordx3 %0, %1, off sc0 sc1" ::"v"(p), "v"(v) : "memory");
+}
+
+typedef uint32_t u32x2_t __attribute__((ext_vector_type(2)));
+__device__ __forceinline__ void store2_through(void *p, u32x2_t v) {
+    asm volatile("global_store_dwordx2 %0, %1, off sc0 sc1" ::"v"(p), "v"(v) : "memory");
 }
 
 struct V3 { float x, y, z; };
diff --git a/softbodyunity_amd/csrc/kernel_types.hpp b/softbodyunity_amd/csrc/kernel_types.hpp
--- a/softbodyunity_amd/csrc/kernel_types.hpp
+++ b/softbodyunity_amd/csrc/kernel_types.hpp
@@ -81,6 +81,7 @@
     float *peek_out;
     const int32_t *kin_map;
     float *kin_target;
+    uint64_t *prev_pk;
 };
 constexpr int kHaloNone = 0, kHaloGhosts = 1;
 
diff --git a/softbodyunity_amd/csrc/prev_codec.hpp b/softbodyunity_amd/csrc/prev_codec.hpp
--- /dev/null
+++ b/softbodyunity_amd/csrc/prev_codec.hpp
@@ -0,0 +1,62 @@
+#pragma once
+#include <stdint.h>
+#include <string.h>
+
+#if defined(__HIPCC__) || defined(__CUDACC__)
+#define SB_PREV_HD __host__ __device__ __forceinline__
+#else
+#define SB_PREV_HD inline
+#endif
+
+namespace sbk {
+
+#ifndef SB_PREV_UNIT_SHIFT
+#define SB_PREV_UNIT_SHIFT 0
+#endif
+constexpr int kPrevUnitShift = SB_PREV_UNIT_SHIFT;
+constexpr int kPrevFieldBits = 21;
+constexpr uint32_t kPrevEscapeHi = 0x80000000u;
+
+SB_PREV_HD uint32_t prev_f2u(float f) { uint32_t u; memcpy(&u, &f, 4); return u; }
+SB_PREV_HD float prev_u2f(uint32_t u) { float f; memcpy(&f, &u, 4); return f; }
+
+SB_PREV_HD float prev_unit(float x) { return prev_u2f((prev_f2u(x) & 0x7f800000u) - ((23u + (uint32_t)kPrevUnitShift) << 23)); }
+SB_PREV_HD float prev_inv_unit(float x) { return prev_u2f(((277u + (uint32_t)kPrevUnitShift) << 23) - (prev_f2u(x) & 0x7f800000u)); }
+
+SB_PREV_HD float prev_decode_c(float x, int32_t q) {
+    const float t = (float)q * prev_unit(x);
+    return x - t;
+}
+
+SB_PREV_HD bool prev_encode_c(float x, float p, int32_t &q) {
+    const float d = x - p;
+    const float qf = d * prev_inv_unit(x);
+    const bool fits = (qf < 1048576.0f) && (qf > -1048576.0f);
+    q = fits ? (int32_t)qf : 0;
+    return fits && prev_f2u(prev_decode_c(x, q)) == prev_f2u(p);
+}
+
+struct PrevWord { uint32_t lo, hi; };
+
+SB_PREV_HD PrevWord prev_encode(float x0, float x1, float x2, float p0, float p1, float p2) {
+    int32_t q0, q1, q2;
+    const bool ok0 = prev_encode_c(x0, p0, q0), ok1 = prev_encode_c(x1, p1, q1), ok2 = prev_encode_c(x2, p2, q2);
+    const uint32_t m = (1u << kPrevFieldBits) - 1u;
+    const uint32_t a = (uint32_t)q0 & m, b = (uint32_t)q1 & m, c = (uint32_t)q2 & m;
+    PrevWord w;
+    w.lo = a | (b << 21);
+    w.hi = (b >> 11) | (c << 10);
+    if (!(ok0 && ok1 && ok2)) { w.lo = 0u; w.hi = kPrevEscapeHi; }
+    return w;
+}
+
+SB_PREV_HD bool prev_escaped(PrevWord w) { return (w.hi & kPrevEscapeHi) != 0u; }
+
+SB_PREV_HD void prev_decode(PrevWord w, float x0, float x1, float x2, float &p0, float &p1, float &p2) {
+    const int32_t q0 = (int32_t)(w.lo << 11) >> 11;
+    const int32_t q1 = (int32_t)(((w.lo >> 21) | (w.hi << 11)) << 11) >> 11;
+    const int32_t q2 = (int32_t)(w.hi << 1) >> 11;
+    p0 = prev_decode_c(x0, q0); p1 = prev_decode_c(x1, q1); p2 = prev_decode_c(x2, q2);
+}
+
+}
diff --git a/softbodyunity_amd/csrc/schedule.hip b/softbodyunity_amd/csrc/schedule.hip
--- a/softbodyunity_amd/csrc/schedule.hip
+++ b/softbodyunity_amd/csrc/schedule.hip
@@ -199,6 +199,7 @@
     if (tile_end <= tile_begin) return;
     sbk::TileArgs A{};
     A.pos = s->pos_view(); A.w8 = s->d_w8.p; A.wpal = s->d_wpal.p; A.prev = s->d_prev.p; A.vel = s->d_vel.p;
+    A.prev_pk = s->d_prev_pk.p;
     A.tiles = D.tiles.p; A.runs_overflow = D.runs_overflow.p; A.stream = D.stream.p;
     A.tp = s->d_tp.p;
     A.gather = D.gather.p;
@@ -217,29 +218,33 @@
     constexpr int kWide8MaxTiles = sbk::kWide8MaxTiles;
     const bool wide8 = small && !D.has_quads && !D.packed_lanes && (s->tile_lanes ? s->tile_lanes == 512 : tile_end - tile_begin <= kWide8MaxTiles);
     const dim3 grid(tile_end - tile_begin), block(quad8 || wide8 ? sbk::kQuadTileThreads : (narrow ? sbk::kNarrowTileThreads : sbk::kWideTileThreads));
-#define SB_LAUNCH_TILE(Q, W, G)                                                                                               \
+#define SB_LAUNCH_TILE(Q, W, G, P)                                                                                              \
     do {                                                                                                                      \
         if (Q && quad8) {                                                                                                     \
-            if (small) hipLaunchKernelGGL((sbk::tile_kernel<KIND, true, sbk::kQuadTileThreads, sbk::kSmallTile / sbk::kQuadTileThreads, W, sbk::kHaloNone>), \
+            if (small) hipLaunchKernelGGL((sbk::tile_kernel<KIND, true, sbk::kQuadTileThreads, sbk::kSmallTile / sbk::kQuadTileThreads, W, sbk::kHaloNone, P>), \
                                           grid, block, D.lds_bytes + s->lds_pad, s->stream, tiles_at_base, n_wg, A);                                           \
-            else hipLaunchKernelGGL((sbk::tile_kernel<KIND, true, sbk::kQuadTileThreads, sbk::kLargeTile / sbk::kQuadTileThreads, W, sbk::kHaloNone>), \
+            else hipLaunchKernelGGL((sbk::tile_kernel<KIND, true, sbk::kQuadTileThreads, sbk::kLargeTile / sbk::kQuadTileThreads, W, sbk::kHaloNone, P>), \
                                     grid, block, D.lds_bytes + s->lds_pad, s->stream, tiles_at_base, n_wg, A);                                                 \
-        } else if (wide8) hipLaunchKernelGGL((sbk::tile_kernel<KIND, false, sbk::kQuadTileThreads, sbk::kSmallTile / sbk::kQuadTileThreads, W, G>), \
+        } else if (wide8) hipLaunchKernelGGL((sbk::tile_kernel<KIND, false, sbk::kQuadTileThreads, sbk::kSmallTile / sbk::kQuadTileThreads, W, G, P>), \
                                        grid, block, D.lds_bytes + s->lds_pad, s->stream, tiles_at_base, n_wg, A);                                              \
-        else if (narrow) hipLaunchKernelGGL((sbk::tile_kernel<KIND, Q, sbk::kNarrowTileThreads, sbk::kSmallTile / sbk::kNarrowTileThreads, W, G>), \
+        else if (narrow) hipLaunchKernelGGL((sbk::tile_kernel<KIND, Q, sbk::kNarrowTileThreads, sbk::kSmallTile / sbk::kNarrowTileThreads, W, G, P>), \
                                        grid, block, D.lds_bytes + s->lds_pad, s->stream, tiles_at_base, n_wg, A);                                              \
-        else if (small) hipLaunchKernelGGL((sbk::tile_kernel<KIND, Q, sbk::kWideTileThreads, sbk::kSmallTile / sbk::kWideTileThreads, W, G>), \
+        else if (small) hipLaunchKernelGGL((sbk::tile_kernel<KIND, Q, sbk::kWideTileThreads, sbk::kSmallTile / sbk::kWideTileThreads, W, G, P>), \
                                            grid, block, D.lds_bytes + s->lds_pad, s->stream, tiles_at_base, n_wg, A);                                          \
-        else hipLaunchKernelGGL((sbk::tile_kernel<KIND, Q, sbk::kWideTileThreads, sbk::kLargeTile / sbk::kWideTileThreads, W, G>), \
+        else hipLaunchKernelGGL((sbk::tile_kernel<KIND, Q, sbk::kWideTileThreads, sbk::kLargeTile / sbk::kWideTileThreads, W, G, P>), \
                                 grid, block, D.lds_bytes + s->lds_pad, s->stream, tiles_at_base, n_wg, A);                                                     \
     } while (0)
     constexpr bool kCanGhost = KIND == 1 || KIND == 2;
+    constexpr bool kCanPack = KIND == 0 || KIND == 1 || KIND == 2 || KIND == 5;
     if (ghosts && !(kCanGhost && !D.has_quads)) throw std::runtime_error("internal: ghost-reading tile kernel requested for a launch that has none");
     if (kCanGhost && ghosts) {
-        if (s->w_palette) SB_LAUNCH_TILE(false, true, (kCanGhost ? sbk::kHaloGhosts : sbk::kHaloNone)); else SB_LAUNCH_TILE(false, false, (kCanGhost ? sbk::kHaloGhosts : sbk::kHaloNone));
+        if (s->w_palette) SB_LAUNCH_TILE(false, true, (kCanGhost ? sbk::kHaloGhosts : sbk::kHaloNone), false); else SB_LAUNCH_TILE(false, false, (kCanGhost ? sbk::kHaloGhosts : sbk::kHaloNone), false);
+    } else if (kCanPack && s->packed_prev) {
+        if (D.has_quads) throw std::runtime_error("internal: packed previous positions on a tiling with tets / hinges");
+        if (s->w_palette) SB_LAUNCH_TILE(false, true, sbk::kHaloNone, kCanPack); else SB_LAUNCH_TILE(false, false, sbk::kHaloNone, kCanPack);
     } else
-    if (s->w_palette) { if (D.has_quads) SB_LAUNCH_TILE(true, true, sbk::kHaloNone); else SB_LAUNCH_TILE(false, true, sbk::kHaloNone); }
-    else { if (D.has_quads) SB_LAUNCH_TILE(true, false, sbk::kHaloNone); else SB_LAUNCH_TILE(false, false, sbk::kHaloNone); }
+    if (s->w_palette) { if (D.has_quads) SB_LAUNCH_TILE(true, true, sbk::kHaloNone, false); else SB_LAUNCH_TILE(false, true, sbk::kHaloNone, false); }
+    else { if (D.has_quads) SB_LAUNCH_TILE(true, false, sbk::kHaloNone, false); else SB_LAUNCH_TILE(false, false, sbk::kHaloNone, false); }
 #undef SB_LAUNCH_TILE
 }
 
diff --git a/softbodyunity_amd/csrc/solver_internal.hpp b/softbodyunity_amd/csrc/solver_internal.hpp
--- a/softbodyunity_amd/csrc/solver_internal.hpp
+++ b/softbodyunity_amd/csrc/solver_internal.hpp
@@ -184,6 +184,8 @@
     bool w_uniform = false;
     sbk::PosView pos_view() const { return sbk::PosView{d_pos3.p, d_wf.p}; }
     DevBuf<float> d_prev, d_vel;
+    DevBuf<uint64_t> d_prev_pk;
+    bool packed_prev = false;
     DevBuf<sbk::TickParams> d_tp;
     DevBuf<float> d_sendbuf, d_recvbuf;
     DevTiling tiling[3];
diff --git a/softbodyunity_amd/csrc/tables.hip b/softbodyunity_amd/csrc/tables.hip
--- a/softbodyunity_amd/csrc/tables.hip
+++ b/softbodyunity_amd/csrc/tables.hip
@@ -126,6 +126,12 @@
         else { D->quad.upload(G.quad, s->dev_bytes); D->rest2.upload(G.rest2, s->dev_bytes); }
         s->gcolours.push_back(std::move(D));
     }
+    s->packed_prev = !(s->tune_flags & SB_TUNE_NO_PACKED_PREV) && L.world == 1 && s->gcolours.empty() && s->tiling[2].n_tiles == 0 &&
+                     !s->tiling[0].has_quads && !s->tiling[1].has_quads;
+    if (s->packed_prev) {
+        s->d_prev_pk.alloc((size_t)s->n_local, s->dev_bytes);
+        HIP_CHECK(hipMemset(s->d_prev_pk.p, 0, (size_t)s->n_local * sizeof(uint64_t)));
+    }
     sbt::build_halos(in, opt, H);
     for (sbt::HostHalo &G : H.halos) {
         auto D = std::make_unique<DevHalo>();
diff --git a/softbodyunity_amd/csrc/tile_kernel.hip.hpp b/softbodyunity_amd/csrc/tile_kernel.hip.hpp
--- a/softbodyunity_amd/csrc/tile_kernel.hip.hpp
+++ b/softbodyunity_amd/csrc/tile_kernel.hip.hpp
@@ -1,16 +1,19 @@
 #pragma once
 #include "device_math.hip.hpp"
+#include "prev_codec.hpp"
 
 namespace sbk {
 
 __device__ __forceinline__ void lds_barrier() { asm volatile("s_waitcnt lgkmcnt(0)\n\ts_barrier" ::: "memory"); }
 
 template <bool QUADS, int THREADS> constexpr int kWavesPerSimd = QUADS ? (THREADS == 64 ? 3 : (THREADS == 512 ? 2 : 4)) : (THREADS == 256 ? 8 : (THREADS == 128 ? 6 : 4));
-template <int KIND_, bool QUADS, int THREADS, int PPT, bool WPAL, int HALO = kHaloNone>
+template <int KIND_, bool QUADS, int THREADS, int PPT, bool WPAL, int HALO = kHaloNone, bool PACKED = false>
 __global__ __launch_bounds__(THREADS, (kWavesPerSimd<QUADS, THREADS> - (KIND_ == 5 && !QUADS ? 1 : 0))) void tile_kernel(const TileDesc *tiles_at_base, int n_workgroups, TileArgs A) {
     constexpr int KIND = KIND_ == 5 ? 1 : KIND_;
     constexpr bool KIN = KIND_ == 5;
     constexpr bool GHOSTS = HALO == kHaloGhosts;
+    static_assert(!(PACKED && GHOSTS), "ghosts carry previous positions as floats");
+    constexpr bool PK_READ = PACKED && (KIND == 1 || KIND == 2), PK_WRITE = PACKED && (KIND == 0 || KIND == 1);
     constexpr int kTileThreads = THREADS;
     constexpr int kCPL = THREADS >= kRoundSlots ? 1 : kRoundSlots / THREADS;
     extern __shared__ uint4 lds_raw[];
@@ -92,6 +95,8 @@
     f32x4 X[PPT];
     float pvx[PPT], pvy[PPT], pvz[PPT];
     uint32_t wi[PPT];
+    typedef uint32_t u32x2 __attribute__((ext_vector_type(2)));
+    u32x2 pk[PK_READ ? PPT : 1];
     const int mypal = WPAL ? __float_as_int(A.wpal[tid & (kMaxMassPalette - 1)]) : 0;
 #pragma unroll
     for (int m = 0; m < PPT; ++m) {
@@ -101,7 +106,8 @@
         X[m].x = px[0]; X[m].y = px[1]; X[m].z = px[2];
         if (WPAL) { wi[m] = A.w8[A.w_uniform ? 0 : gc]; X[m].w = 0.0f; } else { wi[m] = 0; X[m].w = A.pos.w[gc]; }
         pvx[m] = pvy[m] = pvz[m] = 0.0f;
-        if (KIND != 0 && KIND != 3 && KIND != 4) {
+        if (PK_READ) pk[m] = *(reinterpret_cast<const u32x2 *>(A.prev_pk) + gc);
+        else if (KIND != 0 && KIND != 3 && KIND != 4) {
             const float *pp = ghost ? px + 3 : A.prev + 3 * (size_t)gc;
             pvx[m] = pp[0]; pvy[m] = pp[1]; pvz[m] = pp[2];
         }
@@ -134,13 +140,15 @@
         const uint32_t i = tid + q * kTileThreads;
         wv[q] = i < n4_first ? wsrc[i] : *reinterpret_cast<const u32x4 *>(tstream);
     }
-    typedef uint32_t u32x2 __attribute__((ext_vector_type(2)));
     u32x2 wc = {0u, 0u};
     u32x2 wp = {0u, 0u};
     if (!QUADS && kTileThreads == kWidePackLanes)
         wp = *reinterpret_cast<const u32x2 *>(wide_packed ? tstream + win_lo + 2u * (uint32_t)tid : tstream);
 #pragma unroll
-    for (int m = 0; m < PPT; ++m) asm volatile("" ::"v"(X[m].x), "v"(pvx[m]), "v"(wi[m]), "v"(X[m].w));
+    for (int m = 0; m < PPT; ++m) {
+        if (PK_READ) asm volatile("" ::"v"(X[m].x), "v"(pk[m].x), "v"(wi[m]), "v"(X[m].w));
+        else asm volatile("" ::"v"(X[m].x), "v"(pvx[m]), "v"(wi[m]), "v"(X[m].w));
+    }
     asm volatile("" ::"v"(mypal));
     if (WPAL) {
 #pragma unroll
@@ -168,6 +176,28 @@
         }
         if (!any_packed)
             for (uint32_t i = tid + kW * kTileThreads; i < n4_first; i += kTileThreads) dst[i] = wsrc[i];
+    }
+    if (PK_READ) {
+        uint32_t esc = 0u;
+#pragma unroll
+        for (int m = 0; m < PPT; ++m) {
+            const PrevWord w = {pk[m].x, pk[m].y};
+            prev_decode(w, X[m].x, X[m].y, X[m].z, pvx[m], pvy[m], pvz[m]);
+            esc |= (prev_escaped(w) && g[m] >= 0) ? (1u << m) : 0u;
+        }
+        if (__builtin_amdgcn_ballot_w64(esc != 0u) != 0ull) {
+            float ex[PPT], ey[PPT], ez[PPT];
+#pragma unroll
+            for (int m = 0; m < PPT; ++m) {
+                int gm = max(g[m], 0);
+                asm volatile("" : "+v"(gm));
+                const float *pp = A.prev + 3 * (size_t)gm;
+                ex[m] = pp[0]; ey[m] = pp[1]; ez[m] = pp[2];
+            }
+#pragma unroll
+            for (int m = 0; m < PPT; ++m)
+                if (esc & (1u << m)) { pvx[m] = ex[m]; pvy[m] = ey[m]; pvz[m] = ez[m]; }
+        }
     }
     __syncthreads();
     if (!WPAL && !QUADS && kTileThreads == kLanePackLanes && lane_packed_full)
@@ -193,7 +223,9 @@
                 }
                 if (KIND == 4) continue;
                 float vx, vy, vz;
-                const size_t o = 3 * (size_t)g[m];
+                int gm = g[m];
+                if (PACKED) asm volatile("" : "+v"(gm));
+                const size_t o = 3 * (size_t)gm;
                 if (KIND == 0) {
                     vx = A.vel[o + 0]; vy = A.vel[o + 1]; vz = A.vel[o + 2];
                 } else {
@@ -203,7 +235,7 @@
                 }
                 bool moved = false;
                 if (KIN && P.w == 0.0f) {
-                    const int ks = A.kin_map[g[m]];
+                    const int ks = A.kin_map[gm];
                     if (ks >= 0) {
                         float *t = A.kin_target + 3 * (size_t)ks;
                         const float tx = t[0], ty = t[1], tz = t[2];
@@ -213,7 +245,8 @@
                 if (KIND == 2) {
                     A.vel[o + 0] = vx; A.vel[o + 1] = vy; A.vel[o + 2] = vz;
                 } else {
-                    if (A.store_through & 1) store3_through(A.prev + o, P.x, P.y, P.z);
+                    if (PK_WRITE) { pvx[m] = P.x; pvy[m] = P.y; pvz[m] = P.z; }
+                    else if (A.store_through & 1) store3_through(A.prev + o, P.x, P.y, P.z);
                     else { A.prev[o + 0] = P.x; A.prev[o + 1] = P.y; A.prev[o + 2] = P.z; }
                     if (P.w > 0.0f) {
                         vx = vx + tp.hgx; vy = vy + tp.hgy; vz = vz + tp.hgz;
@@ -546,9 +579,22 @@
     for (int m = 0; m < PPT; ++m)
         if (g[m] >= 0) {
             const float4 P = lds_pos[tid + m * kTileThreads];
-            if (KIND == 4) { float *o = A.peek_out + 3 * (size_t)g[m]; o[0] = P.x; o[1] = P.y; o[2] = P.z; }
-            else if (A.store_through & 2) store3_through(A.pos.xyz + 3 * (size_t)g[m], P.x, P.y, P.z);
-            else pv_store(A.pos, g[m], P);
+            int gm = g[m];
+            if (PACKED) asm volatile("" : "+v"(gm));
+            if (KIND == 4) { float *o = A.peek_out + 3 * (size_t)gm; o[0] = P.x; o[1] = P.y; o[2] = P.z; }
+            else if (A.store_through & 2) store3_through(A.pos.xyz + 3 * (size_t)gm, P.x, P.y, P.z);
+            else pv_store(A.pos, gm, P);
+            if (PK_WRITE) {
+                const PrevWord w = prev_encode(P.x, P.y, P.z, pvx[m], pvy[m], pvz[m]);
+                u32x2 *dst = reinterpret_cast<u32x2 *>(A.prev_pk) + gm;
+                const u32x2 wv2 = {w.lo, w.hi};
+                if (A.store_through & 1) store2_through(dst, wv2); else *dst = wv2;
+                if (prev_escaped(w)) {
+                    float *o = A.prev + 3 * (size_t)gm;
+                    if (A.store_through & 1) store3_through(o, pvx[m], pvy[m], pvz[m]);
+                    else { o[0] = pvx[m]; o[1] = pvy[m]; o[2] = pvz[m]; }
+                }
+            }
         }
 }
 
diff --git a/softbodyunity_amd/csrc/validate.hip b/softbodyunity_amd/csrc/validate.hip
--- a/softbodyunity_amd/csrc/validate.hip
+++ b/softbodyunity_amd/csrc/validate.hip
@@ -3,7 +3,36 @@
 
 using namespace sbi;
 
+namespace sbk {
+__global__ __launch_bounds__(256) void prev_escape_count_kernel(const uint64_t *words, long long n, unsigned long long *count) {
+    unsigned long long mine = 0;
+    for (long long i = (long long)blockIdx.x * blockDim.x + threadIdx.x; i < n; i += (long long)gridDim.x * blockDim.x) mine += words[i] >> 63;
+    if (mine) atomicAdd(count, mine);
+}
+}
+
 extern "C" {
+
+int sb_debug_prev_escapes(sb_solver *s, uint64_t *escaped, uint64_t *total) {
+    if (!s || !escaped || !total) return fail(SB_ERR_INVALID_ARG, "sb_debug_prev_escapes: null argument");
+    if (!s->finalized) return fail(SB_ERR_STATE, "sb_debug_prev_escapes before sb_finalize");
+    *escaped = 0; *total = 0;
+    if (!s->packed_prev || s->n_local == 0) return SB_OK;
+    return guarded([&]() -> int {
+        int rc = set_device(s); if (rc) return rc;
+        int64_t acct = 0;
+        DevBuf<unsigned long long> d_cnt; d_cnt.alloc(1, acct);
+        HIP_CHECK(hipMemsetAsync(d_cnt.p, 0, sizeof(unsigned long long), s->stream));
+        const unsigned grid = (unsigned)std::min<int64_t>((s->n_local + 255) / 256, 4096);
+        hipLaunchKernelGGL(sbk::prev_escape_count_kernel, dim3(grid), dim3(256), 0, s->stream, s->d_prev_pk.p, (long long)s->n_local, d_cnt.p);
+        HIP_CHECK(hipGetLastError());
+        unsigned long long c = 0;
+        HIP_CHECK(hipMemcpyAsync(&c, d_cnt.p, sizeof(c), hipMemcpyDeviceToHost, s->stream));
+        HIP_CHECK(hipStreamSynchronize(s->stream));
+        *escaped = (uint64_t)c; *total = (uint64_t)s->n_local;
+        return SB_OK;
+    });
+}
 
 int sb_debug_validate(sb_solver *s, int32_t inject_fault, sb_validate_report *out) {
     if (!s || !out) return fail(SB_ERR_INVALID_ARG, "sb_debug_validate: null argument");
diff --git a/softbodyunity_amd/native.py b/softbodyunity_amd/native.py
--- a/softbodyunity_amd/native.py
+++ b/softbodyunity_amd/native.py
@@ -19,7 +19,7 @@
 SB_GROUP_WHOLE_MESH = 2
 (SB_TUNE_NO_MASS_PALETTE, SB_TUNE_NO_UNIFORM_MASS, SB_TUNE_NO_PALETTE, SB_TUNE_NO_WAVE_ITEMS, SB_TUNE_NO_LANE_PACK, SB_TUNE_NO_COST_ORDER,
  SB_TUNE_NO_FUSED_UNPACK, SB_TUNE_PEER_COARSE, SB_TUNE_NO_LAZY_TICK, SB_TUNE_NO_PACK, SB_TUNE_NO_PEEK, SB_TUNE_NO_KIN_FUSE,
- SB_TUNE_NO_WIDE_SLOTS, SB_TUNE_AUTO_PREFER_OVERLAP, SB_TUNE_NO_AUTO_CALIBRATION, SB_TUNE_NO_SHARED_PROGRAMS) = (1 << k for k in range(16))
+ SB_TUNE_NO_WIDE_SLOTS, SB_TUNE_AUTO_PREFER_OVERLAP, SB_TUNE_NO_AUTO_CALIBRATION, SB_TUNE_NO_SHARED_PROGRAMS, SB_TUNE_NO_PACKED_PREV) = (1 << k for k in range(17))
 SB_ERR_INVALID_ARG, SB_ERR_STATE, SB_ERR_NO_DEVICE, SB_ERR_HIP, SB_ERR_RCCL, SB_ERR_NOMEM, SB_ERR_UNSUPPORTED = \
     -1, -2, -3, -4, -5, -6, -7
 
@@ -130,6 +130,7 @@
     "sb_debug_halo_pack": (C.c_int, [_P, C.c_int32, _P, C.c_int64, C.POINTER(C.c_int64)]),
     "sb_debug_halo_unpack": (C.c_int, [_P, C.c_int32, _P, C.c_int64]),
     "sb_debug_validate": (C.c_int, [_P, C.c_int32, C.POINTER(SbValidateReport)]),
+    "sb_debug_prev_escapes": (C.c_int, [_P, C.POINTER(C.c_uint64), C.POINTER(C.c_uint64)]),
     "sb_get_stats": (C.c_int, [_P, C.POINTER(SbStats)]),
     "sb_plan_build": (C.c_int, [_P, C.c_int32, _P, C.c_int32, _P, C.c_int32, _P, C.c_int32, C.POINTER(SbPlanOpts),
                                 C.POINTER(_P)]),
@@ -259,7 +260,8 @@
                   ("SB_NO_FUSED_UNPACK", SB_TUNE_NO_FUSED_UNPACK), ("SB_PEER_COARSE", SB_TUNE_PEER_COARSE), ("SB_NO_LAZY_TICK", SB_TUNE_NO_LAZY_TICK),
                   ("SB_NO_PACK", SB_TUNE_NO_PACK), ("SB_NO_PEEK", SB_TUNE_NO_PEEK), ("SB_NO_KIN_FUSE", SB_TUNE_NO_KIN_FUSE),
                   ("SB_NO_WIDE_SLOTS", SB_TUNE_NO_WIDE_SLOTS), ("SB_AUTO_PREFER_OVERLAP", SB_TUNE_AUTO_PREFER_OVERLAP),
-                  ("SB_NO_AUTO_CALIBRATION", SB_TUNE_NO_AUTO_CALIBRATION), ("SB_NO_SHARED_PROGRAMS", SB_TUNE_NO_SHARED_PROGRAMS))
+                  ("SB_NO_AUTO_CALIBRATION", SB_TUNE_NO_AUTO_CALIBRATION), ("SB_NO_SHARED_PROGRAMS", SB_TUNE_NO_SHARED_PROGRAMS),
+                  ("SB_NO_PACKED_PREV", SB_TUNE_NO_PACKED_PREV))
 _TUNE_INT_ENV = (("SB_TILE_LANES", "tile_lanes"), ("SB_QUAD_LANES", "quad_lanes"), ("SB_NARROW_MIN_TILES", "narrow_min_tiles"),
                  ("SB_STORE_THROUGH_MAX_TILES", "store_through_max_tiles"), ("SB_STORE_THROUGH_LARGE", "store_through_large"),
                  ("SB_PEEK_MIN_TILES", "peek_min_tiles"), ("SB_LDS_PAD", "lds_pad_bytes"), ("SB_WIN_DWORDS", "win_dwords"),
diff --git a/softbodyunity_amd/softbody.py b/softbodyunity_amd/softbody.py
--- a/softbodyunity_amd/softbody.py
+++ b/softbodyunity_amd/softbody.py
@@ -211,6 +211,11 @@
         return {"tiles_checked": rep.tiles_checked, "groups_checked": rep.groups_checked, "constraints_checked": rep.constraints_checked,
                 "errors": list(rep.errors), "first_stage": rep.first_stage, "first_tile": rep.first_tile, "first_group": rep.first_group,
                 "first_kind": rep.first_kind}
+
+    def prev_escapes(self):
+        e, t = C.c_uint64(0), C.c_uint64(0)
+        check(native.lib().sb_debug_prev_escapes(self._h, C.byref(e), C.byref(t)))
+        return int(e.value), int(t.value)
 
     def stats(self):
         st = native.SbStats()
```

Result: slower. 113.5 billion (-1.4%).
